# XiandaGuo/OpenStereo

Measured on AMD Instinct MI355X. Metric: stereo-pairs/s at 540x960 D=192 (GwcNet fwd), higher is better.
Workload: dtype f32 via f16x3 split-MFMA (hi/lo fp16 operands, f32 accumulate; HBM tensors f32); 1 GPU; GwcNet-gc inference, SceneFlow-shaped 540x960 padded to 544x960, D=192, G=40 + 12ch concat (BASELINE configs[1]); weights=deterministic synthetic (sharpened), random-init architecture, sub_batch_streams=3, parallelism=independent pairs x1, precision=f16x3, launch=hipGraph replay

## Files before the change

### include/openstereo_amd.h

```cpp
#ifndef OPENSTEREO_AMD_H
#define OPENSTEREO_AMD_H

#include <stddef.h>

#ifdef __cplusplus
extern "C" {
#endif

#define OSA_ABI_VERSION 17
#define OSA_META_FLOATS 128

enum { OSA_NCDHW = 0, OSA_NDHWC = 1 };
enum { OSA_ACT_NONE = 0, OSA_ACT_RELU = 1, OSA_ACT_LEAKY = 2, OSA_ACT_RELU6 = 3, OSA_ACT_SIGMOID = 4, OSA_ACT_TANH = 5 };
enum { OSA_GATE_RAW = 16 };
#define OSA_GATE_CHANNELS(n) ((int)((unsigned)(n) << 16))
enum { OSA_IN_SPLIT = 32, OSA_OUT_SPLIT = 64, OSA_RES_SPLIT = 128, OSA_REDIR_SPLIT = 256 };
enum { OSA_RES_AFTER_ACT = 512 };

int         osa_abi_version(void);
const char* osa_last_error(void);
const char* osa_target_arch(void);

int osa_build_volume_f32(const float* left_gwc, const float* right_gwc, int C, int num_groups,
                         const float* left_cat, const float* right_cat, int Cc,
                         float* vol, int layout, int vol_channels, int c_off,
                         int B, int H, int W, int maxdisp, int mask_left_concat,
                         float* vol_meta, void* stream);

int osa_build_volume_nhwc_f32(const float* left_gwc, const float* right_gwc, int C, int num_groups, int gwc_stride,
                              const float* left_cat, const float* right_cat, int Cc, int cat_stride,
                              float* vol, int vol_channels, int c_off,
                              int B, int H, int W, int maxdisp, int mask_left_concat, float* vol_meta, void* stream);
int osa_cat_fms_f32(const float* reference_fm, const float* target_fm, float* out, const int* disp_index,
                    int B, int C, int H, int W, int n_samples, void* stream);
int osa_pair_volume_f32(const float* left, const float* right, float* out,
                        int B, int C, int groups, int H, int W, int planes, int mode, void* stream);

int osa_corr_volume_f32(const float* left, const float* right, float* vol,
                        int B, int C, int H, int W, int maxdisp, void* stream);

int osa_ncdhw_to_ndhwc_f32(const float* x, float* y, int B, int C, long long S,
                           int yCs, int c_off, void* stream);
int osa_ndhwc_to_ncdhw_f32(const float* x, float* y, int B, int C, long long S,
                           int xCs, int c_off, void* stream);

size_t osa_conv3d_packed_floats(int Ci, int Co, int kd, int kh, int kw);
int    osa_conv3d_pack_f32(const float* w_ref, float* w_packed,
                           int Ci, int Co, int kd, int kh, int kw, void* stream);
size_t osa_deconv3d_packed_floats(int Ci, int Co, int k);
int    osa_deconv3d_pack_f32(const float* w_ref, float* w_packed,
                             int Ci, int Co, int k, int pad, void* stream);

int osa_conv3d_ndhwc_f32(const float* x, const float* w_packed,
                         const float* scale, const float* shift, const float* residual,
                         float* y,
                         int B, int Di, int Hi, int Wi, int Ci, int xCs,
                         int Co, int yCs, int rCs,
                         int kd, int kh, int kw, int stride,
                         int pad_d, int pad_h, int pad_w,
                         int dil_d, int dil_h, int dil_w,
                         const float* gate_logits, int gCs,
                         int act, float slope, void* stream);

int osa_conv3d_supported(int B, int Di, int Hi, int Wi, int Ci, int Co, int kd, int kh, int kw, int stride,
                         int pad_d, int pad_h, int pad_w, int dil_d, int dil_h, int dil_w, int precision);

int osa_deconv3d_ndhwc_f32(const float* x, const float* w_packed,
                           const float* scale, const float* shift, const float* residual,
                           float* y,
                           int B, int Di, int Hi, int Wi, int Ci, int xCs,
                           int Co, int yCs, int rCs,
                           int k, int pad, int opad,
                           const float* gate_logits, int gCs,
                           int act, float slope, void* stream);

typedef struct osa_f16x3_ranges {
    const float* x_meta;
    const float* residual_meta;
    const float* redir_meta;
    float*       y_meta;
    const float* bound_coef;
    const float* redir_bound_coef;
    const float* weight_scale;
} osa_f16x3_ranges;

int osa_conv3d_pack_ex_auto(const float* w_ref, float* w_packed, int Ci, int Co, int kd, int kh, int kw,
                            int src_transposed, int flip, const float* w_amax, float* scale_out, void* stream);
int osa_deconv3d_pack_f16x3_auto(const float* w_ref, float* w_packed, int Ci, int Co, int k, int pad,
                                 const float* w_amax, float* scale_out, void* stream);
int osa_deconv2d_pack_f16x3_auto(const float* w_ref, float* w_packed, int Ci, int Co, int k, int pad,
                                 const float* w_amax, float* scale_out, void* stream);

int osa_conv3d_pack_f16x3(const float* w_ref, float* w_packed,
                          int Ci, int Co, int kd, int kh, int kw, float wscale, void* stream);
int osa_deconv3d_pack_f16x3(const float* w_ref, float* w_packed,
                            int Ci, int Co, int k, int pad, float wscale, void* stream);
int osa_conv3d_ndhwc_f16x3(const float* x, const float* w_packed,
                           const float* scale, const float* shift, const float* residual,
                           float* y,
                           int B, int Di, int Hi, int Wi, int Ci, int xCs,
                           int Co, int yCs, int rCs,
                           int kd, int kh, int kw, int stride,
                           int pad_d, int pad_h, int pad_w,
                           int dil_d, int dil_h, int dil_w,
                           const float* gate_logits, int gCs,
                           int act, float slope, float out_scale, const osa_f16x3_ranges* ranges, void* stream);
int osa_deconv3d_ndhwc_f16x3(const float* x, const float* w_packed,
                             const float* scale, const float* shift, const float* residual,
                             float* y,
                             int B, int Di, int Hi, int Wi, int Ci, int xCs,
                             int Co, int yCs, int rCs,
                             int k, int pad, int opad,
                             const float* gate_logits, int gCs,
                             int act, float slope, float out_scale, const osa_f16x3_ranges* ranges, void* stream);

int osa_deconv3d_redir_ndhwc_f32(const float* x, const float* w_packed, const float* scale, const float* shift, float* y,
                                 int B, int Di, int Hi, int Wi, int Ci, int xCs, int Co, int yCs,
                                 int k, int pad, int opad,
                                 const float* rx, int rxCs, int rCi, const float* rw_packed,
                                 const float* rscale, const float* rshift,
                                 int act, float slope, void* stream);
int osa_deconv3d_redir_ndhwc_f16x3(const float* x, const float* w_packed, const float* scale, const float* shift, float* y,
                                   int B, int Di, int Hi, int Wi, int Ci, int xCs, int Co, int yCs,
                                   int k, int pad, int opad,
                                   const float* rx, int rxCs, int rCi, const float* rw_packed,
                                   const float* rscale, const float* rshift, float r_out_scale,
                                   int act, float slope, float out_scale, const osa_f16x3_ranges* ranges, void* stream);

size_t osa_deconv2d_packed_floats(int Ci, int Co, int k);
int    osa_deconv2d_pack_f32(const float* w_ref, float* w_packed, int Ci, int Co, int k, int pad, void* stream);
int    osa_deconv2d_pack_f16x3(const float* w_ref, float* w_packed, int Ci, int Co, int k, int pad,
                               float wscale, void* stream);
int osa_deconv2d_nhwc_f32(const float* x, const float* w_packed,
                          const float* scale, const float* shift, const float* residual,
                          float* y,
                          int B, int Hi, int Wi, int Ci, int xCs,
                          int Co, int yCs, int rCs,
                          int k, int pad, int opad,
                          const float* gate_logits, int gCs,
                          int act, float slope, void* stream);
int osa_deconv2d_nhwc_f16x3(const float* x, const float* w_packed,
                            const float* scale, const float* shift, const float* residual,
                            float* y,
                            int B, int Hi, int Wi, int Ci, int xCs,
                            int Co, int yCs, int rCs,
                            int k, int pad, int opad,
                            const float* gate_logits, int gCs,
                            int act, float slope, float out_scale, const osa_f16x3_ranges* ranges, void* stream);

int osa_dwconv2d_pack_f32(const float* w_ref, float* w_packed, int C, int kh, int kw, void* stream);
int osa_dwconv2d_nhwc_f32(const float* x, const float* w_packed,
                          const float* scale, const float* shift, const float* add, float* y,
                          int B, int Hi, int Wi, int C, int xCs, int yCs, int aCs,
                          int kh, int kw, int stride, int pad_h, int pad_w, int dil_h, int dil_w,
                          int act, float* y_meta, void* stream);
int osa_dwconv2d_nhwc_f16io(const void* x, int x_f16, const float* w_packed,
                            const float* scale, const float* shift, void* y, int y_f16,
                            int B, int Hi, int Wi, int C, int xCs, int yCs,
                            int kh, int kw, int stride, int pad_h, int pad_w,
                            int act, float* y_meta, void* stream);

int osa_gru_combine_f32(const float* z, const float* q, const float* h, float* out,
                        long long npix, int C, int zCs, int qCs, int hCs, int oCs, float* out_meta, void* stream);

typedef struct osa_nhwc_ref { void* ptr; int cs; int f16; } osa_nhwc_ref;
int osa_gru_gates_rz_fwd(const osa_nhwc_ref* pre, const float* bias_z, const float* bias_r, const osa_nhwc_ref* cz, const osa_nhwc_ref* cr,
                         const osa_nhwc_ref* h, const osa_nhwc_ref* z_out, const osa_nhwc_ref* rh_out, long long npix, int C, void* stream);
int osa_gru_gates_rz_bwd(const osa_nhwc_ref* pre, const float* bias_z, const float* bias_r, const osa_nhwc_ref* cz, const osa_nhwc_ref* cr,
                         const osa_nhwc_ref* h, const osa_nhwc_ref* dz, const osa_nhwc_ref* drh, const osa_nhwc_ref* dpre_out,
                         const osa_nhwc_ref* dh_out, long long npix, int C, void* stream);
int osa_gru_gates_q_fwd(const osa_nhwc_ref* z, const osa_nhwc_ref* qpre, const float* bias_q, const osa_nhwc_ref* cq, const osa_nhwc_ref* h,
                        const osa_nhwc_ref* out, long long npix, int C, void* stream);
int osa_gru_gates_q_bwd(const osa_nhwc_ref* z, const osa_nhwc_ref* qpre, const float* bias_q, const osa_nhwc_ref* cq, const osa_nhwc_ref* h,
                        const osa_nhwc_ref* dout, const osa_nhwc_ref* dz_out, const osa_nhwc_ref* dqpre_out, const osa_nhwc_ref* dh_out,
                        long long npix, int C, void* stream);

int osa_disp_update_f32(float* disp, const float* delta, int delta_cs, float* disp_nhwc4, float* slot, int slot_cs,
                        long long npix, float* disp4_meta, float* slot_meta, void* stream);

int osa_pool2x_nhwc_f32(const float* x, float* y, int B, int H, int W, int C, int xCs, int yCs,
                        const float* x_meta, float* y_meta, void* stream);
int osa_resize_bilinear_nhwc_f32(const float* x, float* y, int B, int Hi, int Wi, int Ho, int Wo, int C, int xCs, int yCs,
                                 const float* x_meta, float* y_meta, void* stream);

int osa_conv3d_pack_ex(const float* w_ref, float* w_packed, int Ci, int Co,
                       int kd, int kh, int kw, int src_transposed, int flip,
                       int f16x3, float wscale, void* stream);
int osa_conv3d_wgrad_f32(const float* x, const float* dy, float* dw,
                         int B, int Di, int Hi, int Wi, int Ci, int xCs,
                         int Do, int Ho, int Wo, int Co, int dyCs,
                         int kd, int kh, int kw, int stride,
                         int pad_d, int pad_h, int pad_w, int dil_d, int dil_h, int dil_w,
                         int transposed, void* stream);
size_t osa_conv3d_wgrad_workspace_bytes(int B, int Di, int Hi, int Wi, int Ci, int Do, int Ho, int Wo, int Co,
                                        int kd, int kh, int kw, int stride, int pad_d, int pad_h, int pad_w,
                                        int dil_d, int dil_h, int dil_w, int transposed);
int osa_conv3d_wgrad_ws_f32(const float* x, const float* dy, float* dw,
                            int B, int Di, int Hi, int Wi, int Ci, int xCs,
                            int Do, int Ho, int Wo, int Co, int dyCs,
                            int kd, int kh, int kw, int stride,
                            int pad_d, int pad_h, int pad_w, int dil_d, int dil_h, int dil_w,
                            int transposed, float* workspace, size_t workspace_bytes, void* stream);
size_t osa_conv3d_wgrad_f16x3_workspace_bytes(int B, int Di, int Hi, int Wi, int Ci, int Do, int Ho, int Wo, int Co,
                                              int kd, int kh, int kw, int stride, int pad_d, int pad_h, int pad_w,
                                              int dil_d, int dil_h, int dil_w, int transposed);
int osa_conv3d_wgrad_ws_f16x3(const float* x, const float* dy, float* dw,
                              int B, int Di, int Hi, int Wi, int Ci, int xCs,
                              int Do, int Ho, int Wo, int Co, int dyCs,
                              int kd, int kh, int kw, int stride,
                              int pad_d, int pad_h, int pad_w, int dil_d, int dil_h, int dil_w,
                              int transposed, const float* x_meta, const float* dy_meta,
                              float* workspace, size_t workspace_bytes, void* stream);
int osa_conv3d_wgrad_ws_f16(const void* x, const void* dy, float* dw,
                            int B, int Di, int Hi, int Wi, int Ci, int xCs,
                            int Do, int Ho, int Wo, int Co, int dyCs,
                            int kd, int kh, int kw, int stride,
                            int pad_d, int pad_h, int pad_w, int dil_d, int dil_h, int dil_w,
                            int transposed, const float* x_meta, const float* dy_meta, int x_f16, int dy_f16,
                            float* workspace, size_t workspace_bytes, void* stream);

int osa_conv3d_wgrad_ws_multi(int form, const void* const* xs, const void* const* dys, int n_items, float* dw,
                              int B, int Di, int Hi, int Wi, int Ci, int xCs,
                              int Do, int Ho, int Wo, int Co, int dyCs,
                              int kd, int kh, int kw, int stride,
                              int pad_d, int pad_h, int pad_w, int dil_d, int dil_h, int dil_w,
                              int transposed, const float* x_meta, const float* dy_meta, int x_f16, int dy_f16,
                              float* workspace, size_t workspace_bytes, void* stream);


int osa_conv3d_small_co_ndhwc_f32(const float* x, const float* w_ref, const float* bias,
                                  const float* residual, float* y,
                                  int B, int D, int H, int W, int Ci, int xCs, int Co, int yCs,
                                  int kd, int kh, int kw, int pad_d, int pad_h, int pad_w,
                                  void* stream);

size_t osa_conv3d_small_co_packed_floats(int Ci, int Co, int kd, int kh, int kw);
int    osa_conv3d_small_co_pack_f32(const float* w_ref, float* w_packed, int Ci, int Co,
                                    int kd, int kh, int kw, void* stream);
int    osa_conv3d_small_co_packed_ndhwc_f32(const float* x, const float* w_packed, const float* bias,
                                            const float* residual, float* y,
                                            int B, int D, int H, int W, int Ci, int xCs, int Co, int yCs,
                                            int kd, int kh, int kw, int pad_d, int pad_h, int pad_w,
                                            void* stream);

int osa_softargmin_f32(const float* prob, float* out, int B, int D, int H, int W, void* stream);
int osa_softmax_softargmin_f32(const float* cost, float* prob, float* out,
                               int B, int D, int H, int W, void* stream);
int osa_upsample_softargmin_f32(const float* cost_lowres, float* out,
                                int B, int Dl, int Hl, int Wl, int D, int H, int W,
                                int align_corners, void* stream);

int osa_softargmin_var_f32(const float* prob, const float* disparity, float* out, float* var,
                           int B, int D, int H, int W, void* stream);
int osa_softmax_softargmin_var_f32(const float* cost, float* out, float* var,
                                   int B, int D, int H, int W, void* stream);
int osa_upsample_softargmin_var_f32(const float* cost_lowres, float* out, float* var,
                                    int B, int Dl, int Hl, int Wl, int D, int H, int W,
                                    int align_corners, void* stream);

int osa_build_volume_bwd_f32(const float* dvol, const float* left, const float* right,
                             float* dleft, float* dright,
                             int B, int C, int H, int W, int maxdisp, int num_groups,
                             int concat, int mask_left_concat, int vol_channels, int c_off,
                             void* stream);
int osa_mr_volume_f32(const float* left, const float* right, const float* patch0, const float* patch1,
                      float* v0, float* v1, float* v2, int layout,
                      int B, int C, int H, int W, int num_groups, int out_channels, int maxdisp, int s_range, int m_range, int k0, int k1,
                      void* stream);
size_t osa_mr_volume_bwd_workspace_bytes(int B, int H, int W, int maxdisp);
int osa_mr_volume_bwd_ws_f32(const float* dv0, const float* dv1, const float* dv2, int layout,
                             const float* left, const float* right, const float* patch0, const float* patch1,
                             float* dleft, float* dright, float* dpatch0, float* dpatch1,
                             int B, int C, int H, int W, int num_groups, int out_channels, int maxdisp, int s_range, int m_range, int k0, int k1,
                             void* workspace, size_t workspace_bytes, void* stream);
int osa_softargmin_bwd_f32(const float* dout, float* dprob, int B, int D, int H, int W, void* stream);
int osa_softmax_softargmin_bwd_f32(const float* cost, const float* dout, float* dcost,
                                   int B, int D, int H, int W, void* stream);
int osa_upsample_softargmin_bwd_f32(const float* cost_lowres, const float* dout, float* dcost_lowres,
                                    int B, int Dl, int Hl, int Wl, int D, int H, int W,
                                    int align_corners, void* stream);
size_t osa_upsample_softargmin_bwd_workspace_bytes(int B, int Dl, int H, int W);
int osa_upsample_softargmin_bwd_ws_f32(const float* cost_lowres, const float* dout, float* dcost_lowres,
                                       int B, int Dl, int Hl, int Wl, int D, int H, int W,
                                       int align_corners, void* workspace, size_t workspace_bytes, void* stream);
int osa_softargmin_var_bwd_f32(const float* prob, const float* disparity, const float* dout, const float* dvar,
                               float* dprob, float* ddisparity, int B, int D, int H, int W, void* stream);
int osa_softmax_softargmin_var_bwd_f32(const float* cost, const float* dout, const float* dvar, float* dcost,
                                       int B, int D, int H, int W, void* stream);
int osa_upsample_softargmin_var_bwd_ws_f32(const float* cost_lowres, const float* dout, const float* dvar, float* dcost_lowres,
                                           int B, int Dl, int Hl, int Wl, int D, int H, int W,
                                           int align_corners, void* workspace, size_t workspace_bytes, void* stream);

int osa_amax_f32(const float* x, long long n, float* meta, void* stream);

int osa_context_upsample_f32(const float* disp_low, const float* weights, float* out,
                             int B, int h, int w, int scale, int softmax_weights, float gain,
                             void* stream);
int osa_context_upsample_logits_f32(const float* disp_low, const void* logits, int logits_f16, const long long* logits_strides,
                                    float* out, int B, int h, int w, int scale, float gain, void* stream);
int osa_context_upsample_logits_bwd_f32(const float* disp_low, const void* logits, int logits_f16, const long long* logits_strides,
                                        const float* dout, float* ddisp_low, void* dlogits, const long long* dlogits_strides, float* scratch,
                                        int B, int h, int w, int scale, float gain, void* stream);

int osa_allpairs_corr_f32(const float* fmap1, const float* fmap2, float* corr,
                          int B, int C, int H, int W1, int W2, void* stream);
int osa_geo_rows_f32(const float* vol_ndhwc, float* rows, int B, int D, int H, int W, int C, int Cs, void* stream);
int osa_avgpool_rows_f32(const float* x, float* y, long long rows, int n, void* stream);
int osa_geo_lookup_f32(const float* const* geo_levels, const float* const* corr_levels,
                       const int* geo_len, const int* corr_len, int levels,
                       const float* disp, const float* coords_x, float* out,
                       int B, int H, int W, int C, int radius, void* stream);
int osa_geo_lookup_nhwc_f32(const float* const* geo_levels, const float* const* corr_levels,
                            const int* geo_len, const int* corr_len, int levels,
                            const float* disp, const float* coords_x, float* out, int out_cs,
                            int B, int H, int W, int C, int radius, void* stream);
int osa_geo_lookup_bwd_f32(float* const* dgeo_levels, float* const* dcorr_levels,
                           const int* geo_len, const int* corr_len, int levels,
                           const float* disp, const float* coords_x, const float* dout,
                           int B, int H, int W, int C, int radius, void* stream);
int osa_geo_lookup_bwd_acc_f32(float* const* dgeo_levels, float* const* dcorr_levels,
                               const int* geo_len, const int* corr_len, int levels,
                               const float* disp, const float* coords_x, const float* dout,
                               int B, int H, int W, int C, int radius, void* stream);

int osa_geo_lookup_mr_f32(const float* const* geo0_levels, const float* const* corr_levels,
                          const int* geo0_len, const int* corr_len, int levels,
                          const float* geo1, int geo1_len, const float* geo2, int geo2_len,
                          const float* disp, const float* coords_x,
                          float* geo_feat0, float* geo_feat1, float* geo_feat2, float* init_corr,
                          int B, int H, int W, int C, int radius, void* stream);
int osa_geo_lookup_mr_nhwc_f32(const float* const* geo0_levels, const float* const* corr_levels,
                               const int* geo0_len, const int* corr_len, int levels,
                               const float* geo1, int geo1_len, const float* geo2, int geo2_len,
                               const float* disp, const float* coords_x,
                               float* geo_feat0, float* geo_feat1, float* geo_feat2, float* init_corr,
                               int cs0, int cs1, int cs2, int cs_corr,
                               int B, int H, int W, int C, int radius, void* stream);
int osa_geo_lookup_mr_bwd_acc_f32(float* const* dgeo0_levels, float* const* dcorr_levels,
                                  const int* geo0_len, const int* corr_len, int levels,
                                  float* dgeo1, int geo1_len, float* dgeo2, int geo2_len,
                                  const float* disp, const float* coords_x,
                                  const float* dfeat0, const float* dfeat1, const float* dfeat2, const float* dcorr_out,
                                  int B, int H, int W, int C, int radius, void* stream);

size_t osa_mv2_block3d_packed_floats(int Ci, int Ch, int Co);
int osa_mv2_block3d_pack_f32(const float* w_expand, const float* w_dw, const float* w_project, const float* scale1, const float* shift1,
                             const float* scale2, const float* shift2, const float* scale3, const float* shift3, float* packed,
                             int Ci, int Ch, int Co, void* stream);
int osa_mv2_block3d_f32(const float* x, const float* packed, float* y, int B, int D, int H, int W, int Ci, int Ch, int Co, int stride, int residual,
                        void* stream);

size_t osa_mv2_block2d_packed_floats(int Ci, int Ch, int Co);
int osa_mv2_block2d_pack_f32(const float* w_expand, const float* w_dw, const float* w_project, const float* scale1, const float* shift1,
                             const float* scale2, const float* shift2, const float* scale3, const float* shift3, float* packed,
                             int Ci, int Ch, int Co, void* stream);
int osa_mv2_block2d_f32(const float* x, const float* packed, const float* addend, float* y, int B, int H, int W, int Ci, int Ch, int Co, int stride,
                        int residual, int relu, void* stream);

size_t osa_interlaced_volume_packed_floats(int C, int k2, int k3, int F);
int osa_interlaced_volume_pack_f32(const float* w1, const float* w2, const float* w3, const float* w4, const float* scale1, const float* shift1,
                                   const float* scale2, const float* shift2, const float* scale3, const float* shift3, const float* scale4,
                                   const float* shift4, float* packed, int C, int k2, int k3, int F, void* stream);
int osa_interlaced_volume_f32(const float* featL, const float* featR, const float* packed, float* out, int B, int C, int H, int W, int D, int k2, int k3,
                              int F, void* stream);

size_t osa_disparity_attention_packed_floats(int C, int nhead, int ff, int layers);
int osa_disparity_attention_pack_f32(const float* w_attn, const float* b_attn, const float* w1, const float* b1, const float* w2, const float* b2,
                                     const float* ln, float* packed, int C, int nhead, int ff, int layers, void* stream);
int osa_disparity_attention_f32(const float* cv, const float* pe, const float* packed, float* out, int layout, int B, int C, int L, int H, int W,
                                int nhead, int ff, int layers, void* stream);

int osa_preprocess_pair_f32(const void* left_hwc, const void* right_hwc, int is_u8,
                            int H, int W, int Hp, int Wp,
                            const float* mean3, const float* std3,
                            float* out, int layout, void* stream);

enum { OSA_IN_F16 = 32, OSA_OUT_F16 = 64, OSA_RES_F16 = 128 };
int osa_conv3d_pack_f16(const float* w_ref, float* w_packed, int Ci, int Co, int kd, int kh, int kw, void* stream);
int osa_deconv3d_pack_f16(const float* w_ref, float* w_packed, int Ci, int Co, int k, int pad, void* stream);
int osa_deconv2d_pack_f16(const float* w_ref, float* w_packed, int Ci, int Co, int k, int pad, void* stream);
int osa_conv3d_ndhwc_f16(const void* x, const float* w_packed, const float* scale, const float* shift, const void* residual, void* y,
                         int B, int Di, int Hi, int Wi, int Ci, int xCs, int Co, int yCs, int rCs, int kd, int kh, int kw, int stride,
                         int pad_d, int pad_h, int pad_w, int dil_d, int dil_h, int dil_w, const float* gate_logits, int gCs,
                         int act, float slope, void* stream);
int osa_deconv3d_ndhwc_f16(const void* x, const float* w_packed, const float* scale, const float* shift, const void* residual, void* y,
                           int B, int Di, int Hi, int Wi, int Ci, int xCs, int Co, int yCs, int rCs, int k, int pad, int opad,
                           const float* gate_logits, int gCs, int act, float slope, void* stream);
int osa_deconv2d_nhwc_f16(const void* x, const float* w_packed, const float* scale, const float* shift, const void* residual, void* y,
                          int B, int Hi, int Wi, int Ci, int xCs, int Co, int yCs, int rCs, int k, int pad, int opad,
                          const float* gate_logits, int gCs, int act, float slope, void* stream);

size_t osa_channel_sums_workspace_bytes(long long P, int C);
int osa_channel_sums(const void* dy, int dy_f16, int dy_cs, const void* x, int x_f16, int x_cs, const float* x_shift,
                     const float* dx_scale, void* dx, int dx_cs, long long P, int C,
                     float* out, float* workspace, size_t workspace_bytes, void* stream);
int osa_channel_sums_multi(const void* const* dys, int n_items, int dy_f16, int dy_cs, long long P, int C,
// ... 37 lines not shown
```

### openstereo_amd/_lib.py

```python
from __future__ import annotations

import ctypes as C
import os
import threading

_HERE = os.path.dirname(os.path.abspath(__file__))
LIB_PATH = os.environ.get("OSA_LIB_PATH") or os.path.join(_HERE, "lib", "libopenstereo_amd.so")

_lock = threading.Lock()
_lib = None

c_fp = C.c_void_p
c_i = C.c_int
c_f = C.c_float
c_st = C.c_void_p
c_ll = C.c_longlong


class F16x3Ranges(C.Structure):
    _fields_ = [("x_meta", C.c_void_p), ("residual_meta", C.c_void_p), ("redir_meta", C.c_void_p),
                ("y_meta", C.c_void_p), ("bound_coef", C.c_void_p), ("redir_bound_coef", C.c_void_p), ("weight_scale", C.c_void_p)]


c_rng = C.POINTER(F16x3Ranges)


class NhwcRef(C.Structure):
    _fields_ = [("ptr", C.c_void_p), ("cs", C.c_int), ("f16", C.c_int)]


c_ref = C.POINTER(NhwcRef)

_LEVELS = [C.POINTER(C.c_void_p), C.POINTER(C.c_void_p), C.POINTER(c_i), C.POINTER(c_i), c_i]
SIGNATURES = {
    "osa_abi_version": (c_i, []),
    **dict.fromkeys(("osa_last_error", "osa_target_arch"), (C.c_char_p, [])),
    "osa_build_volume_f32": (c_i, [c_fp, c_fp, c_i, c_i, c_fp, c_fp, c_i, c_fp] + [c_i] * 8 + [c_fp, c_st]),
    "osa_build_volume_nhwc_f32": (c_i, [c_fp, c_fp, c_i, c_i, c_i, c_fp, c_fp, c_i, c_i, c_fp] + [c_i] * 7 + [c_fp, c_st]),
    **dict.fromkeys(("osa_corr_volume_f32", "osa_allpairs_corr_f32"), (c_i, [c_fp, c_fp, c_fp, c_i, c_i, c_i, c_i, c_i, c_st])),
    **dict.fromkeys(("osa_ncdhw_to_ndhwc_f32", "osa_ndhwc_to_ncdhw_f32"), (c_i, [c_fp, c_fp, c_i, c_i, c_ll, c_i, c_i, c_st])),
    **dict.fromkeys(("osa_conv3d_packed_floats", "osa_conv3d_small_co_packed_floats"), (C.c_size_t, [c_i, c_i, c_i, c_i, c_i])),
    **dict.fromkeys(("osa_conv3d_pack_f32", "osa_conv3d_small_co_pack_f32", "osa_conv3d_pack_f16"), (c_i, [c_fp, c_fp, c_i, c_i, c_i, c_i, c_i, c_st])),
    **dict.fromkeys(("osa_deconv3d_packed_floats", "osa_deconv2d_packed_floats"), (C.c_size_t, [c_i, c_i, c_i])),
    **dict.fromkeys(("osa_deconv3d_pack_f32", "osa_softargmin_bwd_f32", "osa_deconv2d_pack_f32", "osa_deconv3d_pack_f16", "osa_deconv2d_pack_f16", "osa_softargmin_f32"), (c_i, [c_fp, c_fp, c_i, c_i, c_i, c_i, c_st])),
    **dict.fromkeys(("osa_conv3d_ndhwc_f32", "osa_conv3d_ndhwc_f16"), (c_i, [c_fp] * 6 + [c_i] * 19 + [c_fp, c_i, c_i, c_f, c_st])),
    **dict.fromkeys(("osa_deconv3d_ndhwc_f32", "osa_deconv3d_ndhwc_f16"), (c_i, [c_fp] * 6 + [c_i] * 12 + [c_fp, c_i, c_i, c_f, c_st])),
    "osa_conv3d_supported": (c_i, [c_i] * 17),
    "osa_conv3d_pack_f16x3": (c_i, [c_fp, c_fp, c_i, c_i, c_i, c_i, c_i, c_f, c_st]),
    **dict.fromkeys(("osa_deconv3d_pack_f16x3", "osa_deconv2d_pack_f16x3"), (c_i, [c_fp, c_fp, c_i, c_i, c_i, c_i, c_f, c_st])),
    "osa_conv3d_ndhwc_f16x3": (c_i, [c_fp] * 6 + [c_i] * 19 + [c_fp, c_i, c_i, c_f, c_f, c_rng, c_st]),
    "osa_deconv3d_ndhwc_f16x3": (c_i, [c_fp] * 6 + [c_i] * 12 + [c_fp, c_i, c_i, c_f, c_f, c_rng, c_st]),
    "osa_conv3d_pack_ex": (c_i, [c_fp, c_fp, c_i, c_i, c_i, c_i, c_i, c_i, c_i, c_i, c_f, c_st]),
    "osa_pair_volume_f32": (c_i, [c_fp, c_fp, c_fp, c_i, c_i, c_i, c_i, c_i, c_i, c_i, c_st]),
    "osa_conv3d_wgrad_f32": (c_i, [c_fp, c_fp, c_fp] + [c_i] * 22 + [c_st]),
    **dict.fromkeys(("osa_conv3d_wgrad_workspace_bytes", "osa_conv3d_wgrad_f16x3_workspace_bytes"), (C.c_size_t, [c_i] * 20)),
    "osa_conv3d_wgrad_ws_f32": (c_i, [c_fp, c_fp, c_fp] + [c_i] * 22 + [c_fp, C.c_size_t, c_st]),
    "osa_conv3d_wgrad_ws_f16x3": (c_i, [c_fp, c_fp, c_fp] + [c_i] * 22 + [c_fp, c_fp, c_fp, C.c_size_t, c_st]),
    "osa_conv3d_wgrad_ws_f16": (c_i, [c_fp, c_fp, c_fp] + [c_i] * 22 + [c_fp, c_fp, c_i, c_i, c_fp, C.c_size_t, c_st]),
    **dict.fromkeys(("osa_conv3d_small_co_ndhwc_f32", "osa_conv3d_small_co_packed_ndhwc_f32"), (c_i, [c_fp] * 5 + [c_i] * 14 + [c_st])),
    "osa_build_volume_bwd_f32": (c_i, [c_fp, c_fp, c_fp, c_fp, c_fp, c_i, c_i, c_i, c_i, c_i, c_i, c_i, c_i, c_i, c_i, c_st]),
    **dict.fromkeys(("osa_softmax_softargmin_bwd_f32", "osa_softmax_softargmin_f32", "osa_softmax_softargmin_var_f32"), (c_i, [c_fp, c_fp, c_fp, c_i, c_i, c_i, c_i, c_st])),
    **dict.fromkeys(("osa_upsample_softargmin_bwd_f32", "osa_upsample_softargmin_var_f32"), (c_i, [c_fp, c_fp, c_fp, c_i, c_i, c_i, c_i, c_i, c_i, c_i, c_i, c_st])),
    "osa_amax_f32": (c_i, [c_fp, C.c_longlong, c_fp, c_st]),
    **dict.fromkeys(("osa_upsample_softargmin_bwd_workspace_bytes", "osa_mr_volume_bwd_workspace_bytes", "osa_interlaced_volume_packed_floats", "osa_disparity_attention_packed_floats"), (C.c_size_t, [c_i] * 4)),
    "osa_upsample_softargmin_bwd_ws_f32": (c_i, [c_fp, c_fp, c_fp, c_i, c_i, c_i, c_i, c_i, c_i, c_i, c_i, c_fp, C.c_size_t, c_st]),
    "osa_deconv3d_redir_ndhwc_f32": (c_i, [c_fp] * 5 + [c_i] * 11 + [c_fp, c_i, c_i, c_fp, c_fp, c_fp, c_i, c_f, c_st]),
    "osa_deconv3d_redir_ndhwc_f16x3": (c_i, [c_fp] * 5 + [c_i] * 11 + [c_fp, c_i, c_i, c_fp, c_fp, c_fp, c_f, c_i, c_f, c_f, c_rng, c_st]),
    **dict.fromkeys(("osa_deconv2d_nhwc_f32", "osa_deconv2d_nhwc_f16"), (c_i, [c_fp] * 6 + [c_i] * 11 + [c_fp, c_i, c_i, c_f, c_st])),
    "osa_deconv2d_nhwc_f16x3": (c_i, [c_fp] * 6 + [c_i] * 11 + [c_fp, c_i, c_i, c_f, c_f, c_rng, c_st]),
    "osa_dwconv2d_pack_f32": (c_i, [c_fp, c_fp, c_i, c_i, c_i, c_st]),
    "osa_dwconv2d_nhwc_f32": (c_i, [c_fp] * 6 + [c_i] * 15 + [c_fp, c_st]),
    "osa_dwconv2d_nhwc_f16io": (c_i, [c_fp, c_i, c_fp, c_fp, c_fp, c_fp, c_i] + [c_i] * 11 + [c_i, c_fp, c_st]),
    "osa_gru_combine_f32": (c_i, [c_fp, c_fp, c_fp, c_fp, c_ll, c_i, c_i, c_i, c_i, c_i, c_fp, c_st]),
    "osa_gru_gates_rz_fwd": (c_i, [c_ref, c_fp, c_fp, c_ref, c_ref, c_ref, c_ref, c_ref, c_ll, c_i, c_st]),
    "osa_gru_gates_rz_bwd": (c_i, [c_ref, c_fp, c_fp, c_ref, c_ref, c_ref, c_ref, c_ref, c_ref, c_ref, c_ll, c_i, c_st]),
    "osa_gru_gates_q_fwd": (c_i, [c_ref, c_ref, c_fp, c_ref, c_ref, c_ref, c_ll, c_i, c_st]),
    "osa_gru_gates_q_bwd": (c_i, [c_ref, c_ref, c_fp, c_ref, c_ref, c_ref, c_ref, c_ref, c_ref, c_ll, c_i, c_st]),
    "osa_disp_update_f32": (c_i, [c_fp, c_fp, c_i, c_fp, c_fp, c_i, c_ll, c_fp, c_fp, c_st]),
    "osa_conv3d_pack_ex_auto": (c_i, [c_fp, c_fp, c_i, c_i, c_i, c_i, c_i, c_i, c_i, c_fp, c_fp, c_st]),
    **dict.fromkeys(("osa_deconv3d_pack_f16x3_auto", "osa_deconv2d_pack_f16x3_auto"), (c_i, [c_fp, c_fp, c_i, c_i, c_i, c_i, c_fp, c_fp, c_st])),
    "osa_cat_fms_f32": (c_i, [c_fp, c_fp, c_fp, c_fp, c_i, c_i, c_i, c_i, c_i, c_st]),
    "osa_pool2x_nhwc_f32": (c_i, [c_fp, c_fp, c_i, c_i, c_i, c_i, c_i, c_i, c_fp, c_fp, c_st]),
    "osa_resize_bilinear_nhwc_f32": (c_i, [c_fp, c_fp, c_i, c_i, c_i, c_i, c_i, c_i, c_i, c_i, c_fp, c_fp, c_st]),
    "osa_context_upsample_logits_f32": (c_i, [c_fp, c_fp, c_i, C.POINTER(c_ll), c_fp, c_i, c_i, c_i, c_i, c_f, c_st]),
    "osa_context_upsample_logits_bwd_f32": (c_i, [c_fp, c_fp, c_i, C.POINTER(c_ll), c_fp, c_fp, c_fp, C.POINTER(c_ll), c_fp, c_i, c_i, c_i, c_i, c_f, c_st]),
    "osa_context_upsample_f32": (c_i, [c_fp, c_fp, c_fp, c_i, c_i, c_i, c_i, c_i, c_f, c_st]),
    "osa_geo_rows_f32": (c_i, [c_fp, c_fp, c_i, c_i, c_i, c_i, c_i, c_i, c_st]),
    "osa_avgpool_rows_f32": (c_i, [c_fp, c_fp, c_ll, c_i, c_st]),
    **dict.fromkeys(("osa_geo_lookup_f32", "osa_geo_lookup_bwd_acc_f32", "osa_geo_lookup_bwd_f32"), (c_i, _LEVELS + [c_fp, c_fp, c_fp, c_i, c_i, c_i, c_i, c_i, c_st])),
    "osa_geo_lookup_nhwc_f32": (c_i, _LEVELS + [c_fp, c_fp, c_fp, c_i, c_i, c_i, c_i, c_i, c_i, c_st]),
    **dict.fromkeys(("osa_geo_lookup_mr_f32", "osa_geo_lookup_mr_bwd_acc_f32"), (c_i, _LEVELS + [c_fp, c_i, c_fp, c_i, c_fp, c_fp, c_fp, c_fp, c_fp, c_fp, c_i, c_i, c_i, c_i, c_i, c_st])),
    "osa_geo_lookup_mr_nhwc_f32": (c_i, _LEVELS + [c_fp, c_i, c_fp, c_i, c_fp, c_fp, c_fp, c_fp, c_fp, c_fp, c_i, c_i, c_i, c_i, c_i, c_i, c_i, c_i, c_i, c_st]),
    "osa_preprocess_pair_f32": (c_i, [c_fp, c_fp, c_i, c_i, c_i, c_i, c_i, C.POINTER(c_f), C.POINTER(c_f), c_fp, c_i, c_st]),
    "osa_instnorm_workspace_floats": (C.c_size_t, [c_i, c_ll, c_i]),
    "osa_instnorm_nhwc_f32": (c_i, [c_fp, c_fp, c_i, c_ll, c_i, c_i, c_i, c_f, c_i, c_f, c_fp, c_fp, c_st]),
    "osa_conv3d_wgrad_ws_multi": (c_i, [c_i, c_fp, c_fp, c_i, c_fp] + [c_i] * 22 + [c_fp, c_fp, c_i, c_i, c_fp, C.c_size_t, c_st]),
    "osa_channel_sums_workspace_bytes": (C.c_size_t, [c_ll, c_i]),
    "osa_channel_affine": (c_i, [c_fp, c_i, c_i, c_fp, c_i, c_i, c_fp, c_fp, c_fp, c_fp, c_i, c_ll, c_i, c_i, c_st]),
    "osa_channel_sums_multi": (c_i, [c_fp, c_i, c_i, c_i, c_ll, c_i, c_fp, c_fp, C.c_size_t, c_st]),
    "osa_channel_sums": (c_i, [c_fp, c_i, c_i, c_fp, c_i, c_i, c_fp, c_fp, c_fp, c_i, c_ll, c_i, c_fp, c_fp, C.c_size_t, c_st]),
    **dict.fromkeys(("osa_conv3d_march_launches", "osa_conv3d_march_s2_launches", "osa_deconv3d_walk_launches", "osa_conv_b_ring_launches", "osa_volume_walk_launches"), (c_ll, [])),
    **dict.fromkeys(("osa_deconv_walk", "osa_deconv_walk_segment_planes", "osa_conv_march_s2_segment_planes", "osa_conv_b_ring_mask", "osa_volume_walk_step"), (c_i, [c_i])),
    "osa_build_volume_nhwc_split_eligible": (c_i, [c_fp, c_fp, c_fp, c_i, c_i, c_i, c_i, c_i, c_i, c_i, c_i, c_i]),
    "osa_build_volume_nhwc_split_f16x3": (c_i, [c_fp, c_fp, c_i, c_i, c_i, c_fp, c_fp, c_i, c_i, c_fp] + [c_i] * 7 + [c_fp, c_fp, c_fp, c_st]),
    "osa_upsample_softargmin_f32": (c_i, [c_fp, c_fp, c_i, c_i, c_i, c_i, c_i, c_i, c_i, c_i, c_st]),
    **dict.fromkeys(("osa_softargmin_var_f32", "osa_softmax_softargmin_var_bwd_f32"), (c_i, [c_fp, c_fp, c_fp, c_fp, c_i, c_i, c_i, c_i, c_st])),
    "osa_softargmin_var_bwd_f32": (c_i, [c_fp, c_fp, c_fp, c_fp, c_fp, c_fp, c_i, c_i, c_i, c_i, c_st]),
    "osa_upsample_softargmin_var_bwd_ws_f32": (c_i, [c_fp, c_fp, c_fp, c_fp, c_i, c_i, c_i, c_i, c_i, c_i, c_i, c_i, c_fp, C.c_size_t, c_st]),
    "osa_mr_volume_f32": (c_i, [c_fp] * 7 + [c_i] * 12 + [c_st]),
    "osa_mr_volume_bwd_ws_f32": (c_i, [c_fp] * 3 + [c_i] + [c_fp] * 8 + [c_i] * 11 + [c_fp, C.c_size_t, c_st]),
    **dict.fromkeys(("osa_mv2_block3d_packed_floats", "osa_mv2_block2d_packed_floats"), (C.c_size_t, [c_i] * 3)),
    **dict.fromkeys(("osa_mv2_block3d_pack_f32", "osa_mv2_block2d_pack_f32"), (c_i, [c_fp] * 10 + [c_i] * 3 + [c_st])),
    "osa_mv2_block3d_f32": (c_i, [c_fp] * 3 + [c_i] * 9 + [c_st]),
    **dict.fromkeys(("osa_mv2_block2d_f32", "osa_disparity_attention_f32"), (c_i, [c_fp] * 4 + [c_i] * 9 + [c_st])),
    "osa_disparity_attention_pack_f32": (c_i, [c_fp] * 8 + [c_i] * 4 + [c_st]),
    "osa_interlaced_volume_pack_f32": (c_i, [c_fp] * 13 + [c_i] * 4 + [c_st]),
    "osa_interlaced_volume_f32": (c_i, [c_fp] * 4 + [c_i] * 8 + [c_st]),
}


class EngineError(RuntimeError):
    pass


def load():
    global _lib
    if _lib is not None:
        return _lib
    with _lock:
        if _lib is not None:
            return _lib
        if not os.path.exists(LIB_PATH):
            raise EngineError(f"{LIB_PATH} is missing: build it with `python -m openstereo_amd.build` (hipcc, gfx950). There is no CPU fallback.")
        lib = C.CDLL(LIB_PATH)
        for name, (res, args) in SIGNATURES.items():
            fn = getattr(lib, name)
            fn.restype = res
            fn.argtypes = args
        if lib.osa_abi_version() != abi_version(lib):
            raise EngineError(f"ABI version mismatch: library reports {lib.osa_abi_version()}, include/openstereo_amd.h declares {abi_version(lib)}")
        if os.environ.get("OSA_B_RING_MASK"):
            lib.osa_conv_b_ring_mask(int(os.environ["OSA_B_RING_MASK"], 0))
        if os.environ.get("OSA_DECONV_WALK"):
            lib.osa_deconv_walk(int(os.environ["OSA_DECONV_WALK"], 0))
        if os.environ.get("OSA_VOL_WALK"):
            lib.osa_volume_walk_step(int(os.environ["OSA_VOL_WALK"]))
        _lib = lib
    return _lib


_abi = None


def abi_version(lib=None) -> int:
    global _abi
    if _abi is None:
        import re
        hdr = os.path.join(os.path.dirname(os.path.abspath(__file__)), "..", "include", "openstereo_amd.h")
        try:
            with open(hdr) as f:
                _abi = int(re.search(r"#define\s+OSA_ABI_VERSION\s+(\d+)", f.read()).group(1))
        except (OSError, AttributeError):
            h = lib if lib is not None else _lib
            if h is None:
                return -1
            _abi = int(h.osa_abi_version())
    return _abi


CALLS = {}


def call(name: str, *args):
    lib = load()
    CALLS[name] = CALLS.get(name, 0) + 1
    rc = getattr(lib, name)(*args)
    if rc != 0:
        msg = lib.osa_last_error()
        raise EngineError(f"{name} failed ({rc}): {msg.decode() if msg else '?'}")
    return rc
```

### openstereo_amd/csrc/conv3d.hip

```cpp
#include "conv_kernel.h"
#include "conv_inst.h"

namespace osa {

struct KernelCfg {
    const char* name;
    int M, N;
    int TD, TH, TW, threads;
    int ks;
    int table, idx;
};

static const KernelCfg g_cfgs[] = {
#define OSA_CFG_X(RING, MT, NT, WM, WN, TH, TW)                                                                  \
    { #MT "x" #NT "_" #WM "x" #WN "_" #TH "x" #TW, WM * MT * 32, WN * NT * 32, WM * MT * 32 / (TH * TW), TH, TW, WM * WN * 64, 0, 0, -1 },
#define OSA_KS_X(MT, NT, WM, WN, TH, TW, KS)
#include "conv_cfgs.def"
#undef OSA_CFG_X
#undef OSA_KS_X
};
constexpr int N_CFGS = sizeof(g_cfgs) / sizeof(g_cfgs[0]);

static const KernelCfg g_ks_cfgs[] = {
#define OSA_CFG_X(RING, MT, NT, WM, WN, TH, TW)
#define OSA_KS_X(MT, NT, WM, WN, TH, TW, KS)                                                                     \
    { #MT "x" #NT "_" #WM "x" #WN "_" #TH "x" #TW "_ks" #KS, WM * MT * 32, WN * NT * 32, WM * MT * 32 / (TH * TW), TH, TW, WM * WN * KS * 64, KS, 1, -1 },
#include "conv_cfgs.def"
#undef OSA_CFG_X
#undef OSA_KS_X
};

static const KernelCfg g_deconv_redir_cfg = { "deconv8_redir_1x1_4x1_4x8", 128, 32, 4, 4, 8, 256, 0, 2, 0 };
static const KernelCfg g_deconv_redir64_cfg = { "deconv8_redir64_1x1_4x1_4x8", 128, 32, 4, 4, 8, 256, 0, 2, 1 };
static const KernelCfg g_deconv_cfg = { "deconv8_1x1_4x1_4x8", 128, 32, 4, 4, 8, 256, 0, 2, 2 };
static const KernelCfg g_deconv_flat_cfg = { "deconv4_1x1_4x1_8x16", 128, 32, 1, 8, 16, 256, 0, 2, 3 };

static const KernelFns& fns_of(const KernelCfg& k, int prec) {
    const ConvFnTables& t = (prec == PREC_F32) ? conv_tables_f32() : ((prec == PREC_F16X3) ? conv_tables_f16x3() : conv_tables_f16());
    if (k.table == 0) return t.cfgs[&k - g_cfgs];
    if (k.table == 1) return t.ks[&k - g_ks_cfgs];
    return t.deconv[k.idx];
}

static int g_b_ring_mask_value();
static int pick_cfg(const ConvArgs& a, int stride, int prec = PREC_F32) {
    {
        const int v = exp_int("OSA_CONV_CFG", -1);
        if (v >= 0 && v < N_CFGS && a.CoP % g_cfgs[v].N == 0) return v;
    }
    const bool flat = (a.Ad == 1);
    const long long vox = (long long)a.B * a.Ad * a.Ah * a.Aw;
    if (flat) {
        if (stride == 2) return (a.CoP % 64 == 0) ? 14 : 12;
        const long long tiles128 = (vox + 127) / 128;
        if (a.CoP % 128 == 0) return (tiles128 * (a.CoP / 128) < 768) ? 11 : 9;
        if (a.CoP % 64 == 0) return (tiles128 * (a.CoP / 64) < 128) ? 14 : 13;
        return 12;
    }
    if (stride == 2) return (a.CoP % 128 == 0) ? 6 : ((a.CoP % 64 == 0) ? 5 : 15);
    if (a.T <= 8) return (a.CoP % 64 == 0) ? 4 : 3;
    if (prec != PREC_F32 && a.CoP % 64 == 0 && ((g_b_ring_mask_value() >> 4) & 1)) return 4;
    if (a.CoP % 128 == 0) return 2;
    if (vox < (1ll << 20)) return (a.CoP % 64 == 0) ? 4 : 3;
    return (a.CoP % 64 == 0) ? 1 : 0;
}

static void finish_geometry(ConvArgs& a, int TW, bool compact) {
    if (exp_set("OSA_NOCOMPACT")) compact = false;
    int rowq;
    if (compact) {
        a.VQ = 4;
        rowq = a.LW * 4 + 1;
    } else {
        a.VQ = 5;
        const int want = (TW == 8) ? 8 : 0;
        rowq = a.LW * 5;
        while ((rowq & 15) != want) ++rowq;
        if (exp_set("OSA_NOPAD")) rowq = a.LW * 5;
    }
    a.RowQ = rowq; a.PlaneQ = a.LH * a.RowQ;
    for (int t = 0; t < a.T; ++t)
        a.toff[t] = (a.td[t] - a.dmin) * a.PlaneQ + (a.th[t] - a.hmin) * a.RowQ + (a.tw[t] - a.wmin) * a.VQ;
    a.magicW = (unsigned)((0x100000000ull + a.LW - 1) / a.LW);
    a.magicH = (unsigned)((0x100000000ull + a.LH - 1) / a.LH);
    a.magicHW = (unsigned)((0x100000000ull + (unsigned long long)a.LH * a.LW - 1) / ((unsigned long long)a.LH * a.LW));
    a.dbg = exp_int("OSA_DBG", 0);
}

static size_t brick_bytes(ConvArgs& a, const KernelCfg& k) {
    int dmax = -128, hmax = -128, wmax = -128;
    a.dmin = a.hmin = a.wmin = 127;
    for (int t = 0; t < a.T; ++t) {
        a.dmin = a.td[t] < a.dmin ? a.td[t] : a.dmin; dmax = a.td[t] > dmax ? a.td[t] : dmax;
        a.hmin = a.th[t] < a.hmin ? a.th[t] : a.hmin; hmax = a.th[t] > hmax ? a.th[t] : hmax;
        a.wmin = a.tw[t] < a.wmin ? a.tw[t] : a.wmin; wmax = a.tw[t] > wmax ? a.tw[t] : wmax;
    }
    a.LD = (k.TD - 1) * a.isd + (dmax - a.dmin) + 1;
    a.LH = (k.TH - 1) * a.ish + (hmax - a.hmin) + 1;
    a.LW = (k.TW - 1) * a.isw + (wmax - a.wmin) + 1;
    return (size_t)a.LD * a.LH * (a.LW * VS + 64) * sizeof(float);
}

int launch_conv_march(ConvArgs& a, hipStream_t st, const char* what);
int launch_conv_march_s2(ConvArgs& a, hipStream_t st, const char* what);
int launch_conv_deconv_walk(ConvArgs& a, hipStream_t st, const char* what);
void wgrad_set_multi_tile(int on);

static int g_b_ring_mask = (1 << 1) | (1 << 2) | (1 << 3) | (1 << 4) | (1 << 13) | (1 << 29) | (1 << 27);
static long long g_b_ring_launches = 0;
static int g_b_ring_mask_value() { return g_b_ring_mask; }

static int plan_conv(ConvArgs& a, int stride, int prec, const char* what, const KernelCfg* forced, const KernelCfg*& kp) {
    int ci = forced ? 0 : pick_cfg(a, stride, prec);
    if (!forced && brick_bytes(a, g_cfgs[ci]) > 160 * 1024) {
        static const int fallback[] = {5, 15, 3, 11};
        for (int f : fallback)
            if (a.CoP % g_cfgs[f].N == 0 && brick_bytes(a, g_cfgs[f]) <= 160 * 1024) { ci = f; break; }
    }
    kp = forced ? forced : &g_cfgs[ci];
    if (!forced && (ci == 11 || ci == 14) && a.Ad == 1 && !(a.act & OSA_OUT_SPLIT)) {
        const int want = exp_int("OSA_KS", -1);
        const long long items = (prec == PREC_F32) ? 1 : a.B;
        const long long nwg = ((items * a.Ad * a.Ah * a.Aw + g_cfgs[ci].M - 1) / g_cfgs[ci].M) * (a.CoP / g_cfgs[ci].N);
        int ks = (a.nchunks % 4 == 0 && a.nchunks >= 16) ? 4 : ((a.nchunks % 2 == 0 && a.nchunks >= 8) ? 2 : 1);
        if (nwg >= 192) ks = 1;
        else if (nwg >= 96 && ks == 4) ks = 2;
        if (want >= 0) ks = (want > 1 && a.nchunks % want == 0) ? want : 1;
        const KernelCfg* split = (ks == 4) ? &g_ks_cfgs[ci == 11 ? 0 : 1] : ((ks == 2) ? &g_ks_cfgs[ci == 11 ? 2 : 3] : nullptr);
        if (split && brick_bytes(a, *split) * ks <= 160 * 1024) kp = split;
    }
    const KernelCfg& k = *kp;
    a.tilesD = cdiv(a.Ad, k.TD); a.tilesH = cdiv(a.Ah, k.TH); a.tilesW = cdiv(a.Aw, k.TW);
    (void)brick_bytes(a, k);
    OSA_REQUIRE((long long)a.LD * a.LH * a.LW < 65536, "%s: LDS brick too large", what);
    finish_geometry(a, k.TW, k.TW == 8 && a.isw == 1);
    const size_t brick = (size_t)a.LD * a.PlaneQ * sizeof(float4);
    OSA_REQUIRE(brick <= 160 * 1024, "%s: LDS brick %dx%dx%d needs %zu B (> 160 KiB)", what, a.LD, a.LH, a.LW, brick);
    return 0;
}

static int launch_conv(ConvArgs& a, int stride, int prec, hipStream_t st, const char* what,
                       const KernelCfg* forced = nullptr) {
    const KernelCfg* kp = nullptr;
    if (plan_conv(a, stride, prec, what, forced, kp)) return -1;
    const KernelCfg& k = *kp;
    const size_t brick = (size_t)a.LD * a.PlaneQ * sizeof(float4);
    a.cps = 1;
    {
        const int want = exp_int("OSA_CPS", 4);
        const size_t cap = (size_t)exp_int("OSA_CPS_LDS", 40 * 1024);
        while (a.cps < want && a.cps < a.nchunks && (size_t)(a.cps + 1) * brick <= cap) ++a.cps;
    }
// ... 123 lines not shown
        v = p.transposed ? p.src[((size_t)ci * p.Co + co) * kvol + kidx] : p.src[((size_t)co * p.Ci + ci) * kvol + kidx];
    }
    reinterpret_cast<_Float16*>(p.dst)[i] = (_Float16)v;
}

__device__ __forceinline__ float auto_wscale(float amax) {
    const unsigned b = __builtin_bit_cast(unsigned, amax);
    const int eb = (int)((b >> 23) & 0xffu);
    if (eb == 0 || eb == 255) return 1.f;
    int k = 14 - (eb - 127) - ((b & 0x7fffffu) ? 1 : 0);
    k = k < -14 ? -14 : (k > 40 ? 40 : k);
    return __builtin_bit_cast(float, (unsigned)(127 + k) << 23);
}
__global__ __launch_bounds__(256) void pack_weights_f16x3_auto_kernel(const PackArgs p, const float* __restrict__ amax, float* __restrict__ scale_out) {
    const float wscale = auto_wscale(*amax);
    if (blockIdx.x == 0 && threadIdx.x == 0) { scale_out[0] = wscale; scale_out[1] = 1.0f / wscale; }
    const size_t total = (size_t)p.nchunks * p.T * 2 * 2 * p.CoP * 8;
    size_t i = (size_t)blockIdx.x * 256 + threadIdx.x;
    if (i >= total) return;
    const int e = i & 7; size_t r = i >> 3;
    const int co = r % p.CoP; r /= p.CoP;
    const int kg = r & 1; r >>= 1;
    const int hl = r & 1; r >>= 1;
    const int t = r % p.T; const int ch = r / p.T;
    const int ci = ch * CC + 8 * kg + e;
    float v = 0.f;
    if (ci < p.Ci && co < p.Co) {
        const size_t kvol = (size_t)p.kd * p.kh * p.kw;
        const size_t kidx = ((size_t)p.kz[t] * p.kh + p.ky[t]) * p.kw + p.kx[t];
        v = wscale * (p.transposed ? p.src[((size_t)ci * p.Co + co) * kvol + kidx]
                                   : p.src[((size_t)co * p.Ci + ci) * kvol + kidx]);
    }
    const _Float16 hi = (_Float16)v;
    reinterpret_cast<_Float16*>(p.dst)[i] = hl ? (_Float16)(v - (float)hi) : hi;
}

static inline int pad32(int c) { return (c + 31) / 32 * 32; }
static inline int nchunks_of(int ci) { return (ci + CC - 1) / CC; }
static inline size_t packed_floats(int Ci, int Co, int T) {
    return (size_t)nchunks_of(Ci) * T * JO * 2 * pad32(Co) * 4;
}
static inline size_t slack_floats(int Co) { return (size_t)4 * JO * 2 * pad32(Co) * 4; }

static int deconv_dim_taps(int k, int pad, int par, int* delta, int* kk) {
    int n = 0;
    for (int t = 0; t < k; ++t) {
        const int num = par + pad - t;
        if (((num % 2) + 2) % 2 != 0) continue;
        delta[n] = (num >= 0) ? num / 2 : -((-num) / 2);
        kk[n] = t;
        ++n;
    }
    return n;
}

template <int CO, bool WG>
__global__ __launch_bounds__(256) void conv_small_co_tiled_kernel(const ConvArgs p, const float* __restrict__ wref,
                                                                  const float* __restrict__ bias) {
    constexpr int TD = 4, TH = 8, TW = 8;
    extern __shared__ __attribute__((aligned(16))) float4 smem[];
    const int tid = threadIdx.x;
    float4* wl4 = smem + (size_t)p.LD * p.PlaneQ;
    float* wl = reinterpret_cast<float*>(wl4);

    unsigned bid = xcd_remap(blockIdx.x, gridDim.x);
    const int twi = bid % p.tilesW; bid /= p.tilesW;
    const int thi = bid % p.tilesH; bid /= p.tilesH;
    const int tdi = bid % p.tilesD;
    const int b = bid / p.tilesD;
    const int a0d = tdi * TD, a0h = thi * TH, a0w = twi * TW;
    const int g0d = a0d + p.dmin, g0h = a0h + p.hmin, g0w = a0w + p.wmin;

    const int nw = WG ? 0 : p.nchunks * p.T * CO * 16;
    for (int i = tid; i < nw; i += 256) {
        const int e = i & 15; int r = i >> 4;
        const int co = r % CO; r /= CO;
        const int t = r % p.T; const int ch = r / p.T;
        const int ci = ch * CC + e;
        wl[i] = (ci < p.Ci) ? wref[((size_t)co * p.Ci + ci) * p.T + t] : 0.f;
    }
    const int tw_ = tid % TW, th_ = (tid / TW) % TH, td_ = tid / (TW * TH);
    const int abase = td_ * p.PlaneQ + th_ * p.RowQ + tw_ * p.VQ;
    float acc[CO];
#pragma unroll
    for (int o = 0; o < CO; ++o) acc[o] = bias ? bias[o] : 0.f;

    for (int ch = 0; ch < p.nchunks; ++ch) {
        if (ch) __syncthreads();
        stage_brick<256, PREC_F32, 1>(p, smem, 0, b, ch * CC, g0d, g0h, g0w, tid);
        __syncthreads();
        for (int t = 0; t < p.T; ++t) {
            const float4* xp = smem + abase + p.toff[t];
            const float4* wq = WG ? reinterpret_cast<const float4*>(wref) + (size_t)(ch * p.T + t) * CO * 4
                                  : wl4 + (size_t)(ch * p.T + t) * CO * 4;
#pragma unroll
            for (int q = 0; q < 4; ++q) {
                const float4 xv = xp[q];
#pragma unroll
                for (int o = 0; o < CO; ++o) {
                    const float4 wv = wq[o * 4 + q];
                    acc[o] = fmaf(xv.x, wv.x, acc[o]); acc[o] = fmaf(xv.y, wv.y, acc[o]);
                    acc[o] = fmaf(xv.z, wv.z, acc[o]); acc[o] = fmaf(xv.w, wv.w, acc[o]);
                }
            }
        }
    }
    const int ad = a0d + td_, ah = a0h + th_, aw = a0w + tw_;
    if (ad < p.Ad && ah < p.Ah && aw < p.Aw) {
        const size_t vox = (((size_t)b * p.Do + ad) * p.Ho + ah) * p.Wo + aw;
#pragma unroll
        for (int o = 0; o < CO; ++o)
            p.y[vox * p.yCs + o] = acc[o] + (p.res ? p.res[vox * p.yCs + o] : 0.f);
    }
}


constexpr int CM_TH = 16, CM_TW = 16, CM_LH = 18, CM_LW = 18, CM_PXQ = 9, CM_ROWQ = 176, CM_ITEMS = CM_LH * CM_LW * 8, CM_PER = (CM_ITEMS + 255) / 256;
__global__ __launch_bounds__(256) void classifier_march_kernel(const ConvArgs p, const float* __restrict__ wpk, const float* __restrict__ bias,
                                                               int dseg, int nseg) {
    extern __shared__ __attribute__((aligned(16))) float4 smem[];
    const int tid = threadIdx.x;
    unsigned bid = xcd_remap(blockIdx.x, gridDim.x);
    const int twi = bid % p.tilesW; bid /= p.tilesW;
    const int thi = bid % p.tilesH; bid /= p.tilesH;
    const int seg = bid % nseg;
    const int b = bid / nseg;
    const int d0 = seg * dseg, d1 = (d0 + dseg < p.Di) ? d0 + dseg : p.Di;
    const int h0 = thi * CM_TH, w0 = twi * CM_TW;
    const size_t plane = (size_t)p.Hi * p.Wi * p.xCs;
    const float* xb = p.x + (size_t)b * p.Di * plane;

    int goff[CM_PER], loff[CM_PER];
#pragma unroll
    for (int j = 0; j < CM_PER; ++j) {
        const int i = tid + 256 * j;
        const int px = i >> 3, q = i & 7;
        const int lh = px / CM_LW, lw = px - lh * CM_LW;
        const int gh = h0 - 1 + lh, gw = w0 - 1 + lw;
        const bool in = i < CM_ITEMS && gh >= 0 && gh < p.Hi && gw >= 0 && gw < p.Wi;
        goff[j] = in ? (gh * p.Wi + gw) * p.xCs + q * 4 : -1;
        loff[j] = (i < CM_ITEMS) ? lh * CM_ROWQ + lw * CM_PXQ + q : -1;
    }
    float4 pre[CM_PER];
    auto issue = [&](int pd) {
        const float* xp = xb + (size_t)pd * plane;
#pragma unroll
        for (int j = 0; j < CM_PER; ++j)
            pre[j] = (goff[j] >= 0) ? *reinterpret_cast<const float4*>(xp + goff[j]) : make_float4(0.f, 0.f, 0.f, 0.f);
    };
    const int tw_ = tid % CM_TW, th_ = tid / CM_TW;
    const float4* xt = smem + th_ * CM_ROWQ + tw_ * CM_PXQ;
    const float4* w4 = reinterpret_cast<const float4*>(wpk);
    float a0 = 0.f, a1 = 0.f, a2 = 0.f;
    issue(d0 > 0 ? d0 - 1 : 0);
    for (int pd = d0 - 1; pd <= d1; ++pd) {
        if (pd >= 0 && pd < p.Di) {
            __syncthreads();
#pragma unroll
            for (int j = 0; j < CM_PER; ++j)
                if (loff[j] >= 0) smem[loff[j]] = pre[j];
            __syncthreads();
            if (pd + 1 <= d1 && pd + 1 < p.Di) issue(pd + 1);
#pragma unroll
            for (int kh = 0; kh < 3; ++kh)
#pragma unroll
                for (int kw = 0; kw < 3; ++kw)
#pragma unroll
                    for (int q = 0; q < 8; ++q) {
                        const float4 xv = xt[kh * CM_ROWQ + kw * CM_PXQ + q];
                        const int wi = ((q >> 2) * 27 + kh * 3 + kw) * 4 + (q & 3);
                        const float4 wk0 = w4[wi], wk1 = w4[wi + 9 * 4], wk2 = w4[wi + 18 * 4];
                        a0 = fmaf(xv.x, wk2.x, a0); a0 = fmaf(xv.y, wk2.y, a0); a0 = fmaf(xv.z, wk2.z, a0); a0 = fmaf(xv.w, wk2.w, a0);
                        a1 = fmaf(xv.x, wk1.x, a1); a1 = fmaf(xv.y, wk1.y, a1); a1 = fmaf(xv.z, wk1.z, a1); a1 = fmaf(xv.w, wk1.w, a1);
                        a2 = fmaf(xv.x, wk0.x, a2); a2 = fmaf(xv.y, wk0.y, a2); a2 = fmaf(xv.z, wk0.z, a2); a2 = fmaf(xv.w, wk0.w, a2);
                    }
        }
        const int od = pd - 1, oh = h0 + th_, ow = w0 + tw_;
        if (od >= d0 && od < d1 && oh < p.Hi && ow < p.Wi) {
            const size_t vox = (((size_t)b * p.Do + od) * p.Ho + oh) * p.Wo + ow;
            p.y[vox * p.yCs] = a0 + (bias ? bias[0] : 0.f) + (p.res ? p.res[vox * p.yCs] : 0.f);
        }
        a0 = a1; a1 = a2; a2 = 0.f;
    }
}

}

using namespace osa;

extern "C" size_t osa_conv3d_packed_floats(int Ci, int Co, int kd, int kh, int kw) {
    return packed_floats(Ci, Co, kd * kh * kw) + slack_floats(Co);
}

static void launch_pack(const PackArgs& p, int prec, float wscale, hipStream_t st, const float* amax_dev = nullptr, float* scale_out = nullptr) {
    if (amax_dev) {
        const size_t total = (size_t)p.nchunks * p.T * 2 * 2 * p.CoP * 8;
        hipLaunchKernelGGL(pack_weights_f16x3_auto_kernel, dim3(total ? cdiv((long long)total, 256) : 1), dim3(256), 0, st, p, amax_dev, scale_out);
        return;
    }
    if (prec == PREC_F32) {
        const size_t total = (size_t)p.nchunks * p.T * JO * 2 * p.CoP * 4;
        if (total) hipLaunchKernelGGL(pack_weights_kernel, dim3(cdiv((long long)total, 256)), dim3(256), 0, st, p);
    } else if (prec == PREC_F16) {
        const size_t total = (size_t)p.nchunks * p.T * 2 * 2 * p.CoP * 8;
        if (total) hipLaunchKernelGGL(pack_weights_f16_kernel, dim3(cdiv((long long)total, 256)), dim3(256), 0, st, p);
    } else {
        const size_t total = (size_t)p.nchunks * p.T * 2 * 2 * p.CoP * 8;
        if (total) hipLaunchKernelGGL(pack_weights_f16x3_kernel, dim3(cdiv((long long)total, 256)), dim3(256), 0, st, p, wscale);
    }
}

static int conv3d_pack_impl(const float* w_ref, float* w_packed, int Ci, int Co,
                            int kd, int kh, int kw, int prec, float wscale, void* stream,
                            int src_transposed = 0, int flip = 0, const float* amax_dev = nullptr, float* scale_out = nullptr) {
    OSA_REQUIRE(w_ref && w_packed, "conv3d_pack: NULL pointer");
    const int T = kd * kh * kw;
    OSA_REQUIRE(T >= 1 && T <= MAX_TAPS, "conv3d_pack: %dx%dx%d kernel has %d taps (max %d)", kd, kh, kw, T, MAX_TAPS);
    OSA_REQUIRE(Ci > 0 && Co > 0, "conv3d_pack: bad channels %d->%d", Ci, Co);
    PackArgs p;
    p.src = w_ref; p.dst = w_packed; p.Ci = Ci; p.Co = Co; p.CoP = pad32(Co);
    p.kd = kd; p.kh = kh; p.kw = kw; p.T = T; p.nchunks = (prec == PREC_F16) ? cdiv(Ci, 32) : nchunks_of(Ci); p.transposed = src_transposed ? 1 : 0;
    int t = 0;
    for (int z = 0; z < kd; ++z) for (int y = 0; y < kh; ++y) for (int x = 0; x < kw; ++x, ++t) {
        p.kz[t] = (signed char)(flip ? kd - 1 - z : z); p.ky[t] = (signed char)(flip ? kh - 1 - y : y);
        p.kx[t] = (signed char)(flip ? kw - 1 - x : x);
    }
    launch_pack(p, prec, wscale, (hipStream_t)stream, amax_dev, scale_out);
    OSA_LAUNCH_CHECK("conv3d_pack");
    return 0;
}

extern "C" int osa_conv3d_pack_ex_auto(const float* w_ref, float* w_packed, int Ci, int Co, int kd, int kh, int kw,
                                       int src_transposed, int flip, const float* w_amax, float* scale_out, void* stream) {
    OSA_REQUIRE(w_amax && scale_out, "conv3d_pack_ex_auto: NULL scale pointers");
    return conv3d_pack_impl(w_ref, w_packed, Ci, Co, kd, kh, kw, PREC_F16X3, 1.f, stream, src_transposed, flip, w_amax, scale_out);
}

extern "C" int osa_conv3d_pack_f32(const float* w_ref, float* w_packed, int Ci, int Co,
                                   int kd, int kh, int kw, void* stream) {
    return conv3d_pack_impl(w_ref, w_packed, Ci, Co, kd, kh, kw, PREC_F32, 1.f, stream);
}

extern "C" int osa_conv3d_pack_ex(const float* w_ref, float* w_packed, int Ci, int Co,
                                  int kd, int kh, int kw, int src_transposed, int flip,
                                  int f16x3, float wscale, void* stream) {
    OSA_REQUIRE(wscale > 0.f, "conv3d_pack_ex: wscale must be a positive power of two");
    return conv3d_pack_impl(w_ref, w_packed, Ci, Co, kd, kh, kw, (f16x3 == 2) ? PREC_F16 : (f16x3 ? PREC_F16X3 : PREC_F32), wscale, stream,
                            src_transposed, flip);
}

extern "C" int osa_conv3d_pack_f16x3(const float* w_ref, float* w_packed, int Ci, int Co,
                                     int kd, int kh, int kw, float wscale, void* stream) {
    OSA_REQUIRE(wscale > 0.f, "conv3d_pack_f16x3: wscale must be a positive power of two");
    return conv3d_pack_impl(w_ref, w_packed, Ci, Co, kd, kh, kw, PREC_F16X3, wscale, stream);
}

extern "C" int osa_conv3d_pack_f16(const float* w_ref, float* w_packed, int Ci, int Co, int kd, int kh, int kw, void* stream) {
    return conv3d_pack_impl(w_ref, w_packed, Ci, Co, kd, kh, kw, PREC_F16, 1.f, stream);
}

extern "C" size_t osa_deconv3d_packed_floats(int Ci, int Co, int k) {
    return packed_floats(Ci, Co, k * k * k) + slack_floats(Co);
}

struct DeconvTaps {
    int T; int cls_end[8];
    signed char kz[MAX_TAPS], ky[MAX_TAPS], kx[MAX_TAPS], dz[MAX_TAPS], dy[MAX_TAPS], dx[MAX_TAPS];
};
static void deconv_taps(int k, int pad, DeconvTaps& d, bool flat = false) {
    int t = 0;
    for (int cls = 0; cls < 8; ++cls) {
        int dd[4], kd_[4], dh[4], kh_[4], dw[4], kw_[4];
        int nd = flat ? (((cls >> 2) & 1) ? 0 : 1) : deconv_dim_taps(k, pad, (cls >> 2) & 1, dd, kd_);
        if (flat) { dd[0] = 0; kd_[0] = 0; }
        const int nh = deconv_dim_taps(k, pad, (cls >> 1) & 1, dh, kh_);
        const int nw = deconv_dim_taps(k, pad, cls & 1, dw, kw_);
        for (int a = 0; a < nd; ++a) for (int b = 0; b < nh; ++b) for (int c = 0; c < nw; ++c, ++t) {
            d.kz[t] = (signed char)kd_[a]; d.ky[t] = (signed char)kh_[b]; d.kx[t] = (signed char)kw_[c];
            d.dz[t] = (signed char)dd[a]; d.dy[t] = (signed char)dh[b]; d.dx[t] = (signed char)dw[c];
        }
        d.cls_end[cls] = t;
    }
    d.T = t;
}

static int deconv3d_pack_impl(const float* w_ref, float* w_packed, int Ci, int Co,
                              int k, int pad, int prec, float wscale, void* stream, bool flat = false,
                              const float* amax_dev = nullptr, float* scale_out = nullptr) {
    OSA_REQUIRE(w_ref && w_packed, "deconv3d_pack: NULL pointer");
    OSA_REQUIRE(k == 3 || k == 4, "deconv3d_pack: kernel %d unsupported (3 or 4)", k);
    DeconvTaps d;
    deconv_taps(k, pad, d, flat);
    PackArgs p;
    p.src = w_ref; p.dst = w_packed; p.Ci = Ci; p.Co = Co; p.CoP = pad32(Co);
    p.kd = flat ? 1 : k; p.kh = k; p.kw = k; p.T = d.T; p.nchunks = (prec == PREC_F16) ? cdiv(Ci, 32) : nchunks_of(Ci); p.transposed = 1;
    for (int t = 0; t < d.T; ++t) { p.kz[t] = d.kz[t]; p.ky[t] = d.ky[t]; p.kx[t] = d.kx[t]; }
    launch_pack(p, prec, wscale, (hipStream_t)stream, amax_dev, scale_out);
    OSA_LAUNCH_CHECK("deconv3d_pack");
    return 0;
}

extern "C" int osa_deconv3d_pack_f16x3_auto(const float* w_ref, float* w_packed, int Ci, int Co, int k, int pad,
                                            const float* w_amax, float* scale_out, void* stream) {
    OSA_REQUIRE(w_amax && scale_out, "deconv3d_pack_f16x3_auto: NULL scale pointers");
    return deconv3d_pack_impl(w_ref, w_packed, Ci, Co, k, pad, PREC_F16X3, 1.f, stream, false, w_amax, scale_out);
}

extern "C" int osa_deconv2d_pack_f16x3_auto(const float* w_ref, float* w_packed, int Ci, int Co, int k, int pad,
                                            const float* w_amax, float* scale_out, void* stream) {
    OSA_REQUIRE(w_amax && scale_out, "deconv2d_pack_f16x3_auto: NULL scale pointers");
    return deconv3d_pack_impl(w_ref, w_packed, Ci, Co, k, pad, PREC_F16X3, 1.f, stream, true, w_amax, scale_out);
}

extern "C" int osa_deconv3d_pack_f32(const float* w_ref, float* w_packed, int Ci, int Co,
                                     int k, int pad, void* stream) {
    return deconv3d_pack_impl(w_ref, w_packed, Ci, Co, k, pad, PREC_F32, 1.f, stream);
}

extern "C" int osa_deconv3d_pack_f16x3(const float* w_ref, float* w_packed, int Ci, int Co,
                                       int k, int pad, float wscale, void* stream) {
    OSA_REQUIRE(wscale > 0.f, "deconv3d_pack_f16x3: wscale must be a positive power of two");
    return deconv3d_pack_impl(w_ref, w_packed, Ci, Co, k, pad, PREC_F16X3, wscale, stream);
}

extern "C" int osa_deconv3d_pack_f16(const float* w_ref, float* w_packed, int Ci, int Co, int k, int pad, void* stream) {
    return deconv3d_pack_impl(w_ref, w_packed, Ci, Co, k, pad, PREC_F16, 1.f, stream);
}
extern "C" int osa_deconv2d_pack_f16(const float* w_ref, float* w_packed, int Ci, int Co, int k, int pad, void* stream) {
// ... 163 lines not shown
                                    int pad_d, int pad_h, int pad_w, int dil_d, int dil_h, int dil_w, const float* gate_logits, int gCs,
                                    int act, float slope, void* stream) {
    const float* x = static_cast<const float*>(x_); const float* residual = static_cast<const float*>(residual_); float* y = static_cast<float*>(y_);
    return conv3d_impl(OSA_CONV_ARGS, PREC_F16, 1.f, stream);
}

static int deconv3d_impl(const float* x, const float* w_packed,
                         const float* scale, const float* shift, const float* residual,
                         float* y,
                         int B, int Di, int Hi, int Wi, int Ci, int xCs,
                         int Co, int yCs, int rCs,
                         int k, int pad, int opad,
                         const float* gate_logits, int gCs,
                         int act, float slope, int prec, float oscale, void* stream, bool flat = false,
                         const float* rx = nullptr, int rxCs = 0, int rCi = 0, const float* rw_packed = nullptr,
                         const float* rscale = nullptr, const float* rshift = nullptr, float roscale = 1.f,
                         const osa_f16x3_ranges* rng = nullptr) {
    if (gate_logits) OSA_REQUIRE(gCs >= Co, "deconv3d: gate stride %d < Co %d", gCs, Co);
    if (check_common("deconv3d", x, w_packed, y, B, Di, Hi, Wi, Ci, xCs, Co, yCs, rCs, residual)) return -1;
    if (flat) OSA_REQUIRE(Di == 1, "deconv2d: the tensor must have D == 1 (got %d)", Di);
    OSA_REQUIRE((k == 3 && pad == 1 && opad == 1) || (k == 4 && pad == 1 && opad == 0),
                "deconv3d: only (k=3,p=1,op=1) and (k=4,p=1,op=0) with stride 2 are supported (got k=%d p=%d op=%d)", k, pad, opad);
    DeconvTaps d;
    deconv_taps(k, pad, d, flat);
    ConvArgs a;
    memset(&a, 0, sizeof(a));
    a.x = x; a.w = reinterpret_cast<const float4*>(w_packed);
    a.scale = scale; a.shift = shift; a.res = residual; a.y = y;
    a.gate = gate_logits; a.gCs = gCs;
    a.B = B; a.Di = Di; a.Hi = Hi; a.Wi = Wi; a.Ci = Ci; a.xCs = xCs;
    a.Do = flat ? 1 : (Di - 1) * 2 - 2 * pad + k + opad; a.Ho = (Hi - 1) * 2 - 2 * pad + k + opad; a.Wo = (Wi - 1) * 2 - 2 * pad + k + opad;
    a.Co = Co; a.yCs = yCs; a.rCs = rCs;
    a.Ad = (a.Do + 1) / 2; a.Ah = (a.Ho + 1) / 2; a.Aw = (a.Wo + 1) / 2;
    a.isd = a.ish = a.isw = 1;
    a.os = 2;
    a.T = d.T;
    for (int t = 0; t < d.T; ++t) { a.td[t] = d.dz[t]; a.th[t] = d.dy[t]; a.tw[t] = d.dx[t]; }
    for (int c = 0; c < 8; ++c) a.cls_end[c] = d.cls_end[c];
    a.nchunks = nchunks_of(Ci); a.CoP = pad32(Co);
    a.act = act; a.slope = slope; a.oscale = oscale;
    if (prec == PREC_F16 && f16_units(a, flat ? "deconv2d" : "deconv3d")) return -1;
    if (rx) {
        OSA_REQUIRE(!flat && !residual && !gate_logits, "deconv3d_redir: residual / gate cannot be combined with the fused redir branch");
        OSA_REQUIRE(rw_packed && rCi > 0 && rCi <= 64 && rCi % 4 == 0 && rxCs >= rCi && rxCs % 4 == 0 && ((size_t)rx & 15) == 0,
                    "deconv3d_redir: redir input needs <= 64 channels (multiple of 4), stride >= channels, 16-byte alignment (Ci=%d stride=%d)", rCi, rxCs);
        OSA_REQUIRE((long long)a.Do * a.Ho * a.Wo * rxCs < (1ll << 31), "deconv3d_redir: redir input too large");
        a.rx = rx; a.rxCs = rxCs; a.rCi = rCi; a.rw = reinterpret_cast<const float4*>(rw_packed);
        a.rscale = rscale; a.rshift = rshift; a.roscale = roscale;
    }
    set_ranges(a, rng);
    if (check_split_ranges(a, prec, flat ? "deconv2d" : "deconv3d")) return -1;
    if (prec == PREC_F16X3 && !flat && k == 3 && rx) {
        const int r = launch_conv_deconv_walk(a, (hipStream_t)stream, "deconv3d (walk)");
        if (r != 0) return r < 0 ? r : 0;
    }
    return launch_conv(a, 1, prec, (hipStream_t)stream, flat ? "deconv2d" : "deconv3d",
                       flat ? &g_deconv_flat_cfg : (rx ? (rCi > 32 ? &g_deconv_redir64_cfg : &g_deconv_redir_cfg) : &g_deconv_cfg));
}

#define OSA_DECONV_PARAMS                                                                       \
    const float* x, const float* w_packed, const float* scale, const float* shift,             \
    const float* residual, float* y, int B, int Di, int Hi, int Wi, int Ci, int xCs,           \
    int Co, int yCs, int rCs, int k, int pad, int opad, const float* gate_logits, int gCs, int act, float slope
#define OSA_DECONV_ARGS                                                                         \
    x, w_packed, scale, shift, residual, y, B, Di, Hi, Wi, Ci, xCs, Co, yCs, rCs, k, pad, opad, \
    gate_logits, gCs, act, slope

extern "C" int osa_deconv3d_ndhwc_f32(OSA_DECONV_PARAMS, void* stream) {
    return deconv3d_impl(OSA_DECONV_ARGS, PREC_F32, 1.f, stream);
}

extern "C" int osa_deconv3d_ndhwc_f16x3(OSA_DECONV_PARAMS, float out_scale, const osa_f16x3_ranges* ranges, void* stream) {
    return deconv3d_impl(OSA_DECONV_ARGS, PREC_F16X3, out_scale, stream, false, nullptr, 0, 0, nullptr, nullptr, nullptr, 1.f, ranges);
}

extern "C" int osa_deconv3d_ndhwc_f16(const void* x_, const float* w_packed, const float* scale, const float* shift, const void* residual_, void* y_,
                                      int B, int Di, int Hi, int Wi, int Ci, int xCs, int Co, int yCs, int rCs, int k, int pad, int opad,
                                      const float* gate_logits, int gCs, int act, float slope, void* stream) {
    const float* x = static_cast<const float*>(x_); const float* residual = static_cast<const float*>(residual_); float* y = static_cast<float*>(y_);
    return deconv3d_impl(OSA_DECONV_ARGS, PREC_F16, 1.f, stream);
}

#define OSA_REDIR_PARAMS const float* rx, int rxCs, int rCi, const float* rw_packed, const float* rscale, const float* rshift
extern "C" int osa_deconv3d_redir_ndhwc_f32(const float* x, const float* w_packed, const float* scale, const float* shift, float* y,
                                            int B, int Di, int Hi, int Wi, int Ci, int xCs, int Co, int yCs,
                                            int k, int pad, int opad, OSA_REDIR_PARAMS, int act, float slope, void* stream) {
    return deconv3d_impl(x, w_packed, scale, shift, nullptr, y, B, Di, Hi, Wi, Ci, xCs, Co, yCs, 0, k, pad, opad, nullptr, 0,
                         act, slope, PREC_F32, 1.f, stream, false, rx, rxCs, rCi, rw_packed, rscale, rshift, 1.f);
}

extern "C" int osa_deconv3d_redir_ndhwc_f16x3(const float* x, const float* w_packed, const float* scale, const float* shift, float* y,
                                              int B, int Di, int Hi, int Wi, int Ci, int xCs, int Co, int yCs,
                                              int k, int pad, int opad, OSA_REDIR_PARAMS, float r_out_scale,
                                              int act, float slope, float out_scale, const osa_f16x3_ranges* ranges, void* stream) {
    return deconv3d_impl(x, w_packed, scale, shift, nullptr, y, B, Di, Hi, Wi, Ci, xCs, Co, yCs, 0, k, pad, opad, nullptr, 0,
                         act, slope, PREC_F16X3, out_scale, stream, false, rx, rxCs, rCi, rw_packed, rscale, rshift, r_out_scale, ranges);
}

#define OSA_DECONV2D_PARAMS                                                                     \
    const float* x, const float* w_packed, const float* scale, const float* shift,             \
    const float* residual, float* y, int B, int Hi, int Wi, int Ci, int xCs,                   \
    int Co, int yCs, int rCs, int k, int pad, int opad, const float* gate_logits, int gCs, int act, float slope
#define OSA_DECONV2D_ARGS                                                                       \
    x, w_packed, scale, shift, residual, y, B, 1, Hi, Wi, Ci, xCs, Co, yCs, rCs, k, pad, opad, \
    gate_logits, gCs, act, slope

extern "C" int osa_deconv2d_nhwc_f32(OSA_DECONV2D_PARAMS, void* stream) {
    return deconv3d_impl(OSA_DECONV2D_ARGS, PREC_F32, 1.f, stream, true);
}

extern "C" int osa_deconv2d_nhwc_f16x3(OSA_DECONV2D_PARAMS, float out_scale, const osa_f16x3_ranges* ranges, void* stream) {
    return deconv3d_impl(OSA_DECONV2D_ARGS, PREC_F16X3, out_scale, stream, true, nullptr, 0, 0, nullptr, nullptr, nullptr, 1.f, ranges);
}

extern "C" int osa_deconv2d_nhwc_f16(const void* x_, const float* w_packed, const float* scale, const float* shift, const void* residual_, void* y_,
                                     int B, int Hi, int Wi, int Ci, int xCs, int Co, int yCs, int rCs, int k, int pad, int opad,
                                     const float* gate_logits, int gCs, int act, float slope, void* stream) {
    const float* x = static_cast<const float*>(x_); const float* residual = static_cast<const float*>(residual_); float* y = static_cast<float*>(y_);
    return deconv3d_impl(OSA_DECONV2D_ARGS, PREC_F16, 1.f, stream, true);
}

__global__ __launch_bounds__(256) void small_co_pack_kernel(const float* __restrict__ src, float* __restrict__ dst,
                                                            int Ci, int Co, int T, int nchunks) {
    const int i = blockIdx.x * 256 + threadIdx.x;
    if (i >= nchunks * T * Co * 16) return;
    const int e = i & 15; int r = i >> 4;
    const int co = r % Co; r /= Co;
    const int t = r % T; const int ch = r / T;
    const int ci = ch * CC + e;
    dst[i] = (ci < Ci) ? src[((size_t)co * Ci + ci) * T + t] : 0.f;
}

extern "C" size_t osa_conv3d_small_co_packed_floats(int Ci, int Co, int kd, int kh, int kw) {
    return (size_t)nchunks_of(Ci) * kd * kh * kw * Co * 16;
}

extern "C" int osa_conv3d_small_co_pack_f32(const float* w_ref, float* w_packed, int Ci, int Co,
                                            int kd, int kh, int kw, void* stream) {
    OSA_REQUIRE(w_ref && w_packed, "conv3d_small_co_pack: NULL pointer");
    OSA_REQUIRE(Ci > 0 && Co >= 1 && Co <= 4 && kd > 0 && kh > 0 && kw > 0, "conv3d_small_co_pack: bad dims");
    const int n = (int)osa_conv3d_small_co_packed_floats(Ci, Co, kd, kh, kw);
    hipLaunchKernelGGL(small_co_pack_kernel, dim3(cdiv(n, 256)), dim3(256), 0, (hipStream_t)stream,
                       w_ref, w_packed, Ci, Co, kd * kh * kw, nchunks_of(Ci));
    OSA_LAUNCH_CHECK("conv3d_small_co_pack");
    return 0;
}

static int small_co_impl(const float* x, const float* w, bool packed, const float* bias,
                         const float* residual, float* y,
                         int B, int D, int H, int W, int Ci, int xCs, int Co, int yCs,
                         int kd, int kh, int kw, int pad_d, int pad_h, int pad_w,
                         void* stream);

extern "C" int osa_conv3d_small_co_ndhwc_f32(const float* x, const float* w_ref, const float* bias,
                                             const float* residual, float* y,
                                             int B, int D, int H, int W, int Ci, int xCs, int Co, int yCs,
                                             int kd, int kh, int kw, int pad_d, int pad_h, int pad_w,
                                             void* stream) {
    return small_co_impl(x, w_ref, false, bias, residual, y, B, D, H, W, Ci, xCs, Co, yCs, kd, kh, kw, pad_d, pad_h, pad_w, stream);
}

extern "C" int osa_conv3d_small_co_packed_ndhwc_f32(const float* x, const float* w_packed, const float* bias,
                                                    const float* residual, float* y,
                                                    int B, int D, int H, int W, int Ci, int xCs, int Co, int yCs,
                                                    int kd, int kh, int kw, int pad_d, int pad_h, int pad_w,
                                                    void* stream) {
    OSA_REQUIRE(((size_t)w_packed & 63) == 0, "conv3d_small_co_packed: packed weights must be 64-byte aligned");
    return small_co_impl(x, w_packed, true, bias, residual, y, B, D, H, W, Ci, xCs, Co, yCs, kd, kh, kw, pad_d, pad_h, pad_w, stream);
}

static int small_co_impl(const float* x, const float* w_ref, bool packed, const float* bias,
                         const float* residual, float* y,
                         int B, int D, int H, int W, int Ci, int xCs, int Co, int yCs,
                         int kd, int kh, int kw, int pad_d, int pad_h, int pad_w,
                         void* stream) {
    OSA_REQUIRE(x && w_ref && y, "conv3d_small_co: NULL pointer");
    OSA_REQUIRE(Co >= 1 && Co <= 4, "conv3d_small_co: Co=%d unsupported (1..4)", Co);
    OSA_REQUIRE(xCs % 4 == 0 && xCs >= Ci && ((size_t)x & 15) == 0, "conv3d_small_co: x must be 16-byte aligned, xCs %% 4 == 0");
    OSA_REQUIRE(kd == 2 * pad_d + 1 && kh == 2 * pad_h + 1 && kw == 2 * pad_w + 1, "conv3d_small_co: only 'same' convolutions");
    OSA_REQUIRE(kd * kh * kw <= MAX_TAPS, "conv3d_small_co: too many taps");
    OSA_REQUIRE(yCs >= Co, "conv3d_small_co: yCs < Co");
    ConvArgs a;
    memset(&a, 0, sizeof(a));
    a.x = x; a.y = y; a.res = residual; a.oscale = 1.f;
    a.B = B; a.Di = D; a.Hi = H; a.Wi = W; a.Ci = Ci; a.xCs = xCs;
    a.Do = D; a.Ho = H; a.Wo = W; a.Co = Co; a.yCs = yCs;
    a.Ad = D; a.Ah = H; a.Aw = W;
    a.isd = a.ish = a.isw = 1; a.os = 1;
    a.T = kd * kh * kw;
    int t = 0;
    for (int z = 0; z < kd; ++z) for (int yy = 0; yy < kh; ++yy) for (int xx = 0; xx < kw; ++xx, ++t) {
        a.td[t] = (signed char)(z - pad_d); a.th[t] = (signed char)(yy - pad_h); a.tw[t] = (signed char)(xx - pad_w);
    }
    a.nchunks = nchunks_of(Ci); a.CoP = Co;
    a.dmin = -pad_d; a.hmin = -pad_h; a.wmin = -pad_w;
    a.LD = 4 + 2 * pad_d; a.LH = 8 + 2 * pad_h; a.LW = 8 + 2 * pad_w;
    a.tilesD = cdiv(D, 4); a.tilesH = cdiv(H, 8); a.tilesW = cdiv(W, 8);
    finish_geometry(a, 8, true);
    hipStream_t st = (hipStream_t)stream;
    if (packed && Co == 1 && Ci == 32 && xCs == 32 && kd == 3 && kh == 3 && kw == 3 && !exp_set("OSA_NO_MARCH")) {
        a.tilesH = cdiv(H, CM_TH); a.tilesW = cdiv(W, CM_TW);
        const long long cols = (long long)B * a.tilesH * a.tilesW;
        int nseg = (int)((2048 + cols - 1) / cols);
        { const int o = exp_int("OSA_MARCH_NSEG", 0); if (o) nseg = o; }
        if (nseg > D / 8) nseg = D / 8;
        if (nseg < 1) nseg = 1;
        const int dseg = cdiv(D, nseg);
        nseg = cdiv(D, dseg);
        OSA_REQUIRE(cols * nseg < (1ll << 31), "conv3d_small_co: grid too large");
        OSA_REQUIRE((long long)H * W * xCs < (1ll << 31), "conv3d_small_co: plane too large");
        const size_t mlds = (size_t)CM_LH * CM_ROWQ * sizeof(float4);
        hipLaunchKernelGGL(classifier_march_kernel, dim3((unsigned)(cols * nseg)), dim3(256), mlds, st, a, w_ref, bias, dseg, nseg);
        OSA_LAUNCH_CHECK("conv3d_small_co (march)");
        return 0;
    }
    const size_t lds = ((size_t)a.LD * a.PlaneQ * 4 + (packed ? 0 : (size_t)a.nchunks * a.T * Co * 16)) * sizeof(float);
    OSA_REQUIRE(lds <= 160 * 1024, "conv3d_small_co: %zu B of LDS needed", lds);
    const long long nblk = (long long)B * a.tilesD * a.tilesH * a.tilesW;
    OSA_REQUIRE(nblk < (1ll << 31), "conv3d_small_co: grid too large");
    dim3 grid((unsigned)nblk), block(256);
#define OSA_SC_LAUNCH1(CO, WG)                                                                              \
    do {                                                                                                    \
        if (lds > 64 * 1024)                                                                                \
            (void)hipFuncSetAttribute((const void*)conv_small_co_tiled_kernel<CO, WG>,                      \
                                      hipFuncAttributeMaxDynamicSharedMemorySize, (int)lds);                \
        hipLaunchKernelGGL((conv_small_co_tiled_kernel<CO, WG>), grid, block, lds, st, a, w_ref, bias);     \
    } while (0)
#define OSA_SC_LAUNCH(CO) do { if (packed) OSA_SC_LAUNCH1(CO, true); else OSA_SC_LAUNCH1(CO, false); } while (0)
    switch (Co) {
        case 1: OSA_SC_LAUNCH(1); break;
        case 2: OSA_SC_LAUNCH(2); break;
        case 3: OSA_SC_LAUNCH(3); break;
        default: OSA_SC_LAUNCH(4); break;
    }
#undef OSA_SC_LAUNCH
    OSA_LAUNCH_CHECK("conv3d_small_co");
    return 0;
}

extern "C" int osa_conv_b_ring_mask(int mask) { const int prev = osa::g_b_ring_mask; osa::g_b_ring_mask = mask; osa::wgrad_set_multi_tile((mask >> 27) & 1); return prev; }
extern "C" long long osa_conv_b_ring_launches(void) { return osa::g_b_ring_launches; }
```

### openstereo_amd/csrc/layout.hip

```cpp
#include "osa_common.h"

namespace osa {

__global__ __launch_bounds__(256) void to_ndhwc_kernel(const float* __restrict__ x, float* __restrict__ y,
                                                       int C, long long S, int yCs, int c_off) {
    __shared__ float tile[32][33];
    const int b = blockIdx.z;
    const long long s0 = (long long)blockIdx.x * 32;
    const int c0 = blockIdx.y * 32;
    const int tx = threadIdx.x & 31, ty = threadIdx.x >> 5;
    for (int r = ty; r < 32; r += 8) {
        const int c = c0 + r; const long long s = s0 + tx;
        tile[r][tx] = (c < C && s < S) ? x[((size_t)b * C + c) * S + s] : 0.f;
    }
    __syncthreads();
    for (int r = ty; r < 32; r += 8) {
        const long long s = s0 + r; const int c = c0 + tx;
        if (c < C && s < S) y[((size_t)b * S + s) * yCs + c_off + c] = tile[tx][r];
    }
}

__global__ __launch_bounds__(256) void to_ncdhw_kernel(const float* __restrict__ x, float* __restrict__ y,
                                                       int C, long long S, int xCs, int c_off) {
    __shared__ float tile[32][33];
    const int b = blockIdx.z;
    const long long s0 = (long long)blockIdx.x * 32;
    const int c0 = blockIdx.y * 32;
    const int tx = threadIdx.x & 31, ty = threadIdx.x >> 5;
    for (int r = ty; r < 32; r += 8) {
        const long long s = s0 + r; const int c = c0 + tx;
        tile[r][tx] = (c < C && s < S) ? x[((size_t)b * S + s) * xCs + c_off + c] : 0.f;
    }
    __syncthreads();
    for (int r = ty; r < 32; r += 8) {
        const int c = c0 + r; const long long s = s0 + tx;
        if (c < C && s < S) y[((size_t)b * C + c) * S + s] = tile[tx][r];
    }
}

__global__ void amax_clear_kernel(float* meta) {
    if (threadIdx.x < OSA_AMAX_SLOTS) atomicExch(reinterpret_cast<unsigned*>(meta) + threadIdx.x * OSA_AMAX_STRIDE, 0u);
}

__global__ __launch_bounds__(256) void amax_kernel(const float* __restrict__ x, long long n, float* meta) {
    __shared__ float red[4];
    float am = 0.f;
    const long long n4 = n >> 2, stride = (long long)gridDim.x * 256;
    const float4* x4 = reinterpret_cast<const float4*>(x);
    for (long long i = (long long)blockIdx.x * 256 + threadIdx.x; i < n4; i += stride) {
        const float4 v = x4[i];
        am = fmaxf(am, fmaxf(fmaxf(fabsf(v.x), fabsf(v.y)), fmaxf(fabsf(v.z), fabsf(v.w))));
    }
    if (blockIdx.x == 0 && threadIdx.x < (n & 3)) am = fmaxf(am, fabsf(x[(n4 << 2) + threadIdx.x]));
    publish_amax(meta, am, 0u, red);
}

}

using namespace osa;

extern "C" int osa_amax_f32(const float* x, long long n, float* meta, void* stream) {
    OSA_REQUIRE(x && meta && n > 0, "amax: NULL pointer or empty tensor");
    OSA_REQUIRE(((size_t)x & 15) == 0, "amax: x must be 16-byte aligned");
    long long blocks = (n / 4 + 255) / 256;
    if (blocks > 2048) blocks = 2048;
    if (blocks < 1) blocks = 1;
    hipLaunchKernelGGL(amax_clear_kernel, dim3(1), dim3(64), 0, (hipStream_t)stream, meta);
    hipLaunchKernelGGL(amax_kernel, dim3((unsigned)blocks), dim3(256), 0, (hipStream_t)stream, x, n, meta);
    OSA_LAUNCH_CHECK("amax");
    return 0;
}

extern "C" int osa_ncdhw_to_ndhwc_f32(const float* x, float* y, int B, int C, long long S,
                                      int yCs, int c_off, void* stream) {
    OSA_REQUIRE(x && y, "ncdhw_to_ndhwc: NULL pointer");
    OSA_REQUIRE(B > 0 && C > 0 && S > 0 && c_off >= 0 && c_off + C <= yCs, "ncdhw_to_ndhwc: bad dims");
    OSA_REQUIRE(B <= 65535 && cdiv(C, 32) <= 65535, "ncdhw_to_ndhwc: grid too large");
    dim3 grid(cdiv(S, 32), cdiv(C, 32), B);
    hipLaunchKernelGGL(to_ndhwc_kernel, grid, dim3(256), 0, (hipStream_t)stream, x, y, C, S, yCs, c_off);
    OSA_LAUNCH_CHECK("ncdhw_to_ndhwc");
    return 0;
}

extern "C" int osa_ndhwc_to_ncdhw_f32(const float* x, float* y, int B, int C, long long S,
                                      int xCs, int c_off, void* stream) {
    OSA_REQUIRE(x && y, "ndhwc_to_ncdhw: NULL pointer");
    OSA_REQUIRE(B > 0 && C > 0 && S > 0 && c_off >= 0 && c_off + C <= xCs, "ndhwc_to_ncdhw: bad dims");
    OSA_REQUIRE(B <= 65535 && cdiv(C, 32) <= 65535, "ndhwc_to_ncdhw: grid too large");
    dim3 grid(cdiv(S, 32), cdiv(C, 32), B);
    hipLaunchKernelGGL(to_ncdhw_kernel, grid, dim3(256), 0, (hipStream_t)stream, x, y, C, S, xCs, c_off);
    OSA_LAUNCH_CHECK("ndhwc_to_ncdhw");
    return 0;
}
```

### openstereo_amd/csrc/torch_ext.cpp

```cpp
#include <ATen/ATen.h>
#include <c10/hip/HIPStream.h>
#include <torch/library.h>
#include <torch/csrc/autograd/custom_function.h>

#include "../../include/openstereo_amd.h"

namespace {

inline void* cur_stream() { return static_cast<void*>(c10::hip::getCurrentHIPStream().stream()); }

#define OSA_CALL(expr)                                                                     \
    do {                                                                                   \
        const int rc__ = (expr);                                                           \
        TORCH_CHECK(rc__ == 0, "openstereo_amd: ", #expr, " failed (", rc__, "): ", osa_last_error()); \
    } while (0)

inline const at::Tensor& gpu_f32(const at::Tensor& t, const char* name) {
    TORCH_CHECK(t.is_cuda(), "openstereo_amd: ", name, " is on ", t.device(), " -- the gfx950 engine has no CPU path");
    TORCH_CHECK(t.scalar_type() == at::kFloat, "openstereo_amd: ", name, " must be float32");
    return t;
}
inline const float* fp(const at::Tensor& t) { return t.data_ptr<float>(); }
inline const float* fpo(const c10::optional<at::Tensor>& t) { return (t.has_value() && t->defined()) ? t->data_ptr<float>() : nullptr; }
inline void* vp(const at::Tensor& t, int64_t off) { return static_cast<char*>(t.data_ptr()) + off * t.element_size(); }
// ... 433 lines not shown

at::Tensor softmax_softargmin_bwd(const at::Tensor& cost, const at::Tensor& dout) {
    gpu_f32(cost, "cost"); gpu_f32(dout, "dout");
    TORCH_CHECK(cost.dim() == 4 && dout.dim() == 3, "softmax_softargmin_bwd: cost [B,D,H,W], dout [B,H,W]");
    const auto c = cost.contiguous(), g = dout.contiguous();
    auto dc = at::empty_like(c);
    OSA_CALL(osa_softmax_softargmin_bwd_f32(fp(c), fp(g), dc.data_ptr<float>(), (int)c.size(0), (int)c.size(1), (int)c.size(2), (int)c.size(3), cur_stream()));
    return dc;
}

at::Tensor upsample_softargmin_bwd(const at::Tensor& cost_lowres, const at::Tensor& dout, int64_t maxdisp, int64_t h, int64_t w, bool align_corners) {
    gpu_f32(cost_lowres, "cost_lowres"); gpu_f32(dout, "dout");
    TORCH_CHECK(cost_lowres.dim() == 4 && dout.dim() == 3, "upsample_softargmin_bwd: cost [B,Dl,Hl,Wl], dout [B,h,w]");
    const auto c = cost_lowres.contiguous(), g = dout.contiguous();
    auto dc = at::empty_like(c);
    const size_t need = osa_upsample_softargmin_bwd_workspace_bytes((int)c.size(0), (int)c.size(1), (int)h, (int)w);
    auto ws = at::empty({(int64_t)((need + 3) / 4)}, c.options());
    OSA_CALL(osa_upsample_softargmin_bwd_ws_f32(fp(c), fp(g), dc.data_ptr<float>(), (int)c.size(0), (int)c.size(1), (int)c.size(2), (int)c.size(3), (int)maxdisp,
                                                (int)h, (int)w, align_corners ? 1 : 0, ws.data_ptr<float>(), need, cur_stream()));
    return dc;
}

std::tuple<at::Tensor, at::Tensor> softargmin_var_bwd(const at::Tensor& prob, const at::Tensor& disparity, const at::Tensor& dout, const at::Tensor& dvar) {
    gpu_f32(prob, "prob"); gpu_f32(disparity, "disparity"); gpu_f32(dout, "dout"); gpu_f32(dvar, "dvar");
    TORCH_CHECK(prob.dim() == 4 && dout.dim() == 3 && dvar.sizes() == dout.sizes(), "softargmin_var_bwd: prob [B,D,H,W], dout / dvar [B,H,W]");
    const auto p = prob.contiguous(), d = disparity.contiguous(), g = dout.contiguous(), gv = dvar.contiguous();
    TORCH_CHECK(d.numel() == g.numel() && g.size(0) == p.size(0) && g.size(1) == p.size(2) && g.size(2) == p.size(3), "softargmin_var_bwd: shapes disagree");
    auto dp = at::empty_like(p), dd = at::empty(d.sizes(), d.options());
    OSA_CALL(osa_softargmin_var_bwd_f32(fp(p), fp(d), fp(g), fp(gv), dp.data_ptr<float>(), dd.data_ptr<float>(), (int)p.size(0), (int)p.size(1), (int)p.size(2),
                                        (int)p.size(3), cur_stream()));
    return {dp, dd};
}

at::Tensor softmax_softargmin_var_bwd(const at::Tensor& cost, const at::Tensor& dout, const at::Tensor& dvar) {
    gpu_f32(cost, "cost"); gpu_f32(dout, "dout"); gpu_f32(dvar, "dvar");
    TORCH_CHECK(cost.dim() == 4 && dout.dim() == 3 && dvar.sizes() == dout.sizes(), "softmax_softargmin_var_bwd: cost [B,D,H,W], dout / dvar [B,H,W]");
    const auto c = cost.contiguous(), g = dout.contiguous(), gv = dvar.contiguous();
    TORCH_CHECK(g.size(0) == c.size(0) && g.size(1) == c.size(2) && g.size(2) == c.size(3), "softmax_softargmin_var_bwd: shapes disagree");
    auto dc = at::empty_like(c);
    OSA_CALL(osa_softmax_softargmin_var_bwd_f32(fp(c), fp(g), fp(gv), dc.data_ptr<float>(), (int)c.size(0), (int)c.size(1), (int)c.size(2), (int)c.size(3), cur_stream()));
    return dc;
}

at::Tensor upsample_softargmin_var_bwd(const at::Tensor& cost_lowres, const at::Tensor& dout, const at::Tensor& dvar, int64_t maxdisp, int64_t h, int64_t w,
                                       bool align_corners) {
    gpu_f32(cost_lowres, "cost_lowres"); gpu_f32(dout, "dout"); gpu_f32(dvar, "dvar");
    TORCH_CHECK(cost_lowres.dim() == 4 && dout.dim() == 3 && dvar.sizes() == dout.sizes(), "upsample_softargmin_var_bwd: cost [B,Dl,Hl,Wl], dout / dvar [B,h,w]");
    const auto c = cost_lowres.contiguous(), g = dout.contiguous(), gv = dvar.contiguous();
    TORCH_CHECK(g.size(0) == c.size(0) && g.size(1) == h && g.size(2) == w, "upsample_softargmin_var_bwd: shapes disagree");
    auto dc = at::empty_like(c);
    const size_t need = osa_upsample_softargmin_bwd_workspace_bytes((int)c.size(0), (int)c.size(1), (int)h, (int)w);
    auto ws = at::empty({(int64_t)((need + 3) / 4)}, c.options());
    OSA_CALL(osa_upsample_softargmin_var_bwd_ws_f32(fp(c), fp(g), fp(gv), dc.data_ptr<float>(), (int)c.size(0), (int)c.size(1), (int)c.size(2), (int)c.size(3),
                                                    (int)maxdisp, (int)h, (int)w, align_corners ? 1 : 0, ws.data_ptr<float>(), need, cur_stream()));
    return dc;
}

std::tuple<at::Tensor, bool> cost_volume_cl(const at::Tensor& gwc_feat, const c10::optional<at::Tensor>& cat_feat, int64_t B, int64_t num_groups, int64_t maxdisp,
                                            int64_t gwc_channels, int64_t cat_channels, int64_t gwc_off, bool mask_left, bool out_split,
                                            const c10::optional<at::Tensor>& gwc_meta, const c10::optional<at::Tensor>& cat_meta, const at::Tensor& out_meta) {
    gpu_f32(gwc_feat, "gwc_feat"); gpu_f32(out_meta, "out_meta");
    TORCH_CHECK(gwc_feat.dim() == 5 && gwc_feat.size(0) == 2 * B && gwc_feat.size(2) == 1 && gwc_feat.stride(1) == 1, "cost_volume_cl: gwc_feat must be NHWC [2B, Cs, 1, H, W]");
    const int64_t Gs = gwc_feat.size(1), H = gwc_feat.size(3), W = gwc_feat.size(4);
    const int64_t C = gwc_channels >= 0 ? gwc_channels : Gs - gwc_off;
    const float* lg = fp(gwc_feat) + gwc_off;
    const float* rg = lg + B * H * W * Gs;
    const float *lc = nullptr, *rc = nullptr;
    int64_t Cc = 0, cs = 0;
    if (cat_feat.has_value() && cat_feat->defined()) {
        gpu_f32(*cat_feat, "cat_feat");
        TORCH_CHECK(cat_feat->dim() == 5 && cat_feat->size(0) == 2 * B && cat_feat->size(3) == H && cat_feat->size(4) == W && cat_feat->stride(1) == 1,
                    "cost_volume_cl: cat_feat must be NHWC [2B, cs, 1, H, W] at the gwc features' resolution");
        cs = cat_feat->size(1); Cc = cat_channels >= 0 ? cat_channels : cs;
        lc = fp(*cat_feat); rc = lc + B * H * W * cs;
    }
    const int64_t nch = num_groups + 2 * Cc, VC = (nch + 3) / 4 * 4;
    auto out = at::empty({B, maxdisp, H, W, VC}, gwc_feat.options()).permute({0, 4, 1, 2, 3});
    if (VC != nch) out.zero_();
    const float* gm = fpo(gwc_meta); const float* cm = fpo(cat_meta);
    const bool split = out_split && VC == nch && (C == 0 || gm) && (Cc == 0 || cm) &&
        osa_build_volume_nhwc_split_eligible(lc, rc, out.data_ptr<float>(), (int)C, (int)num_groups, (int)Gs, (int)Cc, (int)cs, (int)VC, 0, (int)W, (int)maxdisp) == 1;
    if (split)
        OSA_CALL(osa_build_volume_nhwc_split_f16x3(lg, rg, (int)C, (int)num_groups, (int)Gs, lc, rc, (int)Cc, (int)cs, out.data_ptr<float>(), (int)VC, 0, (int)B, (int)H, (int)W,
                                                   (int)maxdisp, mask_left ? 1 : 0, gm, cm, out_meta.data_ptr<float>(), cur_stream()));
    else
        OSA_CALL(osa_build_volume_nhwc_f32(lg, rg, (int)C, (int)num_groups, (int)Gs, lc, rc, (int)Cc, (int)cs, out.data_ptr<float>(), (int)VC, 0, (int)B, (int)H, (int)W,
                                           (int)maxdisp, mask_left ? 1 : 0, out_meta.data_ptr<float>(), cur_stream()));
    return {out, split};
}

static size_t wgrad_workspace(at::IntArrayRef dims, int64_t prec, const char* who, const char* batch, int (&d)[22]) {
    TORCH_CHECK(dims.size() == 22, who, ": dims = [", batch, ", D, H, W, Ci, xCs, Do, Ho, Wo, Co, dyCs, kd, kh, kw, stride, pad x3, dil x3, transposed]");
    for (int i = 0; i < 22; ++i) d[i] = (int)dims[i];
    const auto query = prec == 0 ? osa_conv3d_wgrad_workspace_bytes : osa_conv3d_wgrad_f16x3_workspace_bytes;
    return query(d[0], d[1], d[2], d[3], d[4], d[6], d[7], d[8], d[9], d[11], d[12], d[13], d[14], d[15], d[16], d[17], d[18], d[19], d[20], d[21]);
}
struct WgradOperands {
    std::vector<const void*> x, dy;
    bool list, xh, dyh;
};
static bool wgrad_run(const char* who, const char* batch, const WgradOperands& t, at::Tensor& dw, at::IntArrayRef dims, int64_t prec,
                      const c10::optional<at::Tensor>& x_meta, const c10::optional<at::Tensor>& dy_meta) {
    TORCH_CHECK(prec == 2 || (!t.xh && !t.dyh), who, ": fp16 tensors exist in the native f16 form only (prec 2)");
    int d[22];
    const size_t need = wgrad_workspace(dims, prec, who, batch, d);
    if (need == 0) {
        TORCH_CHECK(prec != 0, who, ": unsupported layer");
        return false;
    }
    auto ws = at::empty({(int64_t)((need + 3) / 4)}, dw.options());
    void* st = cur_stream();
    const float* const x = static_cast<const float*>(t.x[0]); const float* const dy = static_cast<const float*>(t.dy[0]);
#define OSA_WG_DIMS d[0], d[1], d[2], d[3], d[4], d[5], d[6], d[7], d[8], d[9], d[10], d[11], d[12], d[13], d[14], d[15], d[16], d[17], d[18], d[19], d[20], d[21]
    if (t.list) OSA_CALL(osa_conv3d_wgrad_ws_multi((int)prec, t.x.data(), t.dy.data(), (int)t.x.size(), dw.data_ptr<float>(), OSA_WG_DIMS, fpo(x_meta), fpo(dy_meta),
                                                   t.xh ? 1 : 0, t.dyh ? 1 : 0, ws.data_ptr<float>(), need, st));
    else if (prec == 0) OSA_CALL(osa_conv3d_wgrad_ws_f32(x, dy, dw.data_ptr<float>(), OSA_WG_DIMS, ws.data_ptr<float>(), need, st));
    else if (prec == 1) OSA_CALL(osa_conv3d_wgrad_ws_f16x3(x, dy, dw.data_ptr<float>(), OSA_WG_DIMS, fpo(x_meta), fpo(dy_meta), ws.data_ptr<float>(), need, st));
    else OSA_CALL(osa_conv3d_wgrad_ws_f16(x, dy, dw.data_ptr<float>(), OSA_WG_DIMS, fpo(x_meta), fpo(dy_meta), t.xh ? 1 : 0, t.dyh ? 1 : 0, ws.data_ptr<float>(), need, st));
#undef OSA_WG_DIMS
    return true;
}
bool conv_wgrad(const at::Tensor& x, const at::Tensor& dy, at::Tensor dw, at::IntArrayRef dims, int64_t prec, const c10::optional<at::Tensor>& x_meta,
                const c10::optional<at::Tensor>& dy_meta) {
    gpu_f32(dw, "dw");
    const bool xh = x.scalar_type() == at::kHalf, dyh = dy.scalar_type() == at::kHalf;
    TORCH_CHECK(x.is_cuda() && dy.is_cuda() && (xh || x.scalar_type() == at::kFloat) && (dyh || dy.scalar_type() == at::kFloat), "conv_wgrad: x / dy must be CUDA fp32 or fp16 tensors");
    return wgrad_run("conv_wgrad", "B", {{x.data_ptr()}, {dy.data_ptr()}, false, xh, dyh}, dw, dims, prec, x_meta, dy_meta);
}

bool conv_wgrad_multi(at::TensorList xs, at::TensorList dys, at::Tensor dw, at::IntArrayRef dims, int64_t prec, const c10::optional<at::Tensor>& x_meta,
                      const c10::optional<at::Tensor>& dy_meta) {
    gpu_f32(dw, "dw");
    TORCH_CHECK(xs.size() >= 1 && xs.size() <= 24 && xs.size() == dys.size(), "conv_wgrad_multi: 1..24 (x, dy) pairs");
    WgradOperands t{{}, {}, true, xs[0].scalar_type() == at::kHalf, dys[0].scalar_type() == at::kHalf};
    for (size_t i = 0; i < xs.size(); ++i) {
        TORCH_CHECK(xs[i].is_cuda() && dys[i].is_cuda() && xs[i].scalar_type() == xs[0].scalar_type() && dys[i].scalar_type() == dys[0].scalar_type() &&
                    xs[i].sizes() == xs[0].sizes() && xs[i].strides() == xs[0].strides() && dys[i].sizes() == dys[0].sizes() && dys[i].strides() == dys[0].strides(),
                    "conv_wgrad_multi: the items must agree in device, dtype, shape and strides");
        t.x.push_back(xs[i].data_ptr()); t.dy.push_back(dys[i].data_ptr());
    }
    TORCH_CHECK((t.xh || xs[0].scalar_type() == at::kFloat) && (t.dyh || dys[0].scalar_type() == at::kFloat), "conv_wgrad_multi: fp32 or fp16 tensors");
    return wgrad_run("conv_wgrad_multi", "B total", t, dw, dims, prec, x_meta, dy_meta);
}

void to_cl(const at::Tensor& x, at::Tensor y, int64_t C, int64_t S, int64_t c_off) {
    gpu_f32(x, "x"); gpu_f32(y, "y");
    TORCH_CHECK(x.is_contiguous() && y.dim() == 5 && y.stride(1) == 1, "to_cl: x contiguous NCDHW, y NDHWC");
    OSA_CALL(osa_ncdhw_to_ndhwc_f32(fp(x), y.data_ptr<float>(), (int)x.size(0), (int)C, (long long)S, (int)y.size(1), (int)c_off, cur_stream()));
}
void to_ncdhw(const at::Tensor& x, at::Tensor y, int64_t C, int64_t S, int64_t c_off) {
    gpu_f32(x, "x"); gpu_f32(y, "y");
    TORCH_CHECK(y.is_contiguous() && x.dim() == 5 && x.stride(1) == 1, "to_ncdhw: x NDHWC, y contiguous NCDHW");
    OSA_CALL(osa_ndhwc_to_ncdhw_f32(fp(x), y.data_ptr<float>(), (int)x.size(0), (int)C, (long long)S, (int)x.size(1), (int)c_off, cur_stream()));
}

void conv_pack(const at::Tensor& w, at::Tensor packed, at::IntArrayRef geom, int64_t prec, const c10::optional<at::Tensor>& w_amax, const c10::optional<at::Tensor>& scale_out) {
    gpu_f32(w, "w"); gpu_f32(packed, "packed");
    TORCH_CHECK(geom.size() == 7 && w.is_contiguous(), "conv_pack: geom = [Ci, Co, kd, kh, kw, src_transposed, flip], w contiguous");
    const int g[7] = {(int)geom[0], (int)geom[1], (int)geom[2], (int)geom[3], (int)geom[4], (int)geom[5], (int)geom[6]};
    if (prec == 1) {
        TORCH_CHECK(w_amax.has_value() && scale_out.has_value(), "conv_pack: the f16x3 mode needs w_amax and scale_out (device tensors)");
        OSA_CALL(osa_conv3d_pack_ex_auto(fp(w), packed.data_ptr<float>(), g[0], g[1], g[2], g[3], g[4], g[5], g[6], fpo(w_amax), const_cast<float*>(fpo(scale_out)), cur_stream()));
    } else OSA_CALL(osa_conv3d_pack_ex(fp(w), packed.data_ptr<float>(), g[0], g[1], g[2], g[3], g[4], g[5], g[6], prec == 2 ? 2 : 0, 1.0f, cur_stream()));
}
void deconv_pack(const at::Tensor& w, at::Tensor packed, at::IntArrayRef geom, int64_t prec, const c10::optional<at::Tensor>& w_amax, const c10::optional<at::Tensor>& scale_out) {
    gpu_f32(w, "w"); gpu_f32(packed, "packed");
    TORCH_CHECK(geom.size() == 5 && w.is_contiguous(), "deconv_pack: geom = [Ci, Co, k, pad, flat], w contiguous");
    const int Ci = (int)geom[0], Co = (int)geom[1], k = (int)geom[2], pad = (int)geom[3];
    const bool flat = geom[4] != 0;
    float* dst = packed.data_ptr<float>();
    void* st = cur_stream();
    if (prec == 1) {
        TORCH_CHECK(w_amax.has_value() && scale_out.has_value(), "deconv_pack: the f16x3 mode needs w_amax and scale_out (device tensors)");
        float* so = const_cast<float*>(fpo(scale_out));
        if (flat) OSA_CALL(osa_deconv2d_pack_f16x3_auto(fp(w), dst, Ci, Co, k, pad, fpo(w_amax), so, st));
        else OSA_CALL(osa_deconv3d_pack_f16x3_auto(fp(w), dst, Ci, Co, k, pad, fpo(w_amax), so, st));
    } else if (prec == 2) {
        if (flat) OSA_CALL(osa_deconv2d_pack_f16(fp(w), dst, Ci, Co, k, pad, st));
        else OSA_CALL(osa_deconv3d_pack_f16(fp(w), dst, Ci, Co, k, pad, st));
    } else {
        if (flat) OSA_CALL(osa_deconv2d_pack_f32(fp(w), dst, Ci, Co, k, pad, st));
        else OSA_CALL(osa_deconv3d_pack_f32(fp(w), dst, Ci, Co, k, pad, st));
    }
}

inline osa_nhwc_ref nref(const at::Tensor& t, const char* name) {
    TORCH_CHECK(t.is_cuda() && t.dim() == 4 && t.stride(1) == 1 && (t.scalar_type() == at::kFloat || t.scalar_type() == at::kHalf),
                "openstereo_amd: ", name, " must be a CUDA fp32 / fp16 tensor [B,C,H,W] in NHWC memory order");
    TORCH_CHECK(t.stride(2) == t.size(3) * t.stride(3) && t.stride(0) == t.size(2) * t.stride(2), "openstereo_amd: ", name, " is not dense over its pixels");
    osa_nhwc_ref r;
    r.ptr = t.data_ptr(); r.cs = (int)t.stride(3); r.f16 = t.scalar_type() == at::kHalf ? 1 : 0;
    return r;
}
void gru_gates_rz_fwd(const at::Tensor& pre, const c10::optional<at::Tensor>& bz, const c10::optional<at::Tensor>& br, const at::Tensor& cz, const at::Tensor& cr,
                      const at::Tensor& h, at::Tensor z, at::Tensor rh) {
    const auto a = nref(pre, "pre"), b = nref(cz, "cz"), c = nref(cr, "cr"), d = nref(h, "h"), e = nref(z, "z"), f = nref(rh, "rh");
    OSA_CALL(osa_gru_gates_rz_fwd(&a, fpo(bz), fpo(br), &b, &c, &d, &e, &f, (long long)h.size(0) * h.size(2) * h.size(3), (int)h.size(1), cur_stream()));
}
void gru_gates_rz_bwd(const at::Tensor& pre, const c10::optional<at::Tensor>& bz, const c10::optional<at::Tensor>& br, const at::Tensor& cz, const at::Tensor& cr,
                      const at::Tensor& h, const at::Tensor& dz, const at::Tensor& drh, at::Tensor dpre, at::Tensor dh) {
    const auto a = nref(pre, "pre"), b = nref(cz, "cz"), c = nref(cr, "cr"), d = nref(h, "h"), e = nref(dz, "dz"), f = nref(drh, "drh"), g = nref(dpre, "dpre"), i = nref(dh, "dh");
    OSA_CALL(osa_gru_gates_rz_bwd(&a, fpo(bz), fpo(br), &b, &c, &d, &e, &f, &g, &i, (long long)h.size(0) * h.size(2) * h.size(3), (int)h.size(1), cur_stream()));
}
void gru_gates_q_fwd(const at::Tensor& z, const at::Tensor& qpre, const c10::optional<at::Tensor>& bq, const at::Tensor& cq, const at::Tensor& h, at::Tensor out) {
    const auto a = nref(z, "z"), b = nref(qpre, "qpre"), c = nref(cq, "cq"), d = nref(h, "h"), e = nref(out, "out");
    OSA_CALL(osa_gru_gates_q_fwd(&a, &b, fpo(bq), &c, &d, &e, (long long)h.size(0) * h.size(2) * h.size(3), (int)h.size(1), cur_stream()));
}
void gru_gates_q_bwd(const at::Tensor& z, const at::Tensor& qpre, const c10::optional<at::Tensor>& bq, const at::Tensor& cq, const at::Tensor& h, const at::Tensor& dout,
                     at::Tensor dz, at::Tensor dqpre, at::Tensor dh) {
    const auto a = nref(z, "z"), b = nref(qpre, "qpre"), c = nref(cq, "cq"), d = nref(h, "h"), e = nref(dout, "dout"), f = nref(dz, "dz"), g = nref(dqpre, "dqpre"), i = nref(dh, "dh");
    OSA_CALL(osa_gru_gates_q_bwd(&a, &b, fpo(bq), &c, &d, &e, &f, &g, &i, (long long)h.size(0) * h.size(2) * h.size(3), (int)h.size(1), cur_stream()));
}

struct RowList { float* ptr[10]; int len[10]; };
inline RowList row_list(at::TensorList ts, size_t split, const char* first, const char* rest) {
    RowList v;
    TORCH_CHECK(ts.size() <= 10, "row_list: ", ts.size(), " row tensors, at most 10");
    for (size_t q = 0; q < ts.size(); ++q) { v.ptr[q] = gpu_f32(ts[q], q < split ? first : rest).data_ptr<float>(); v.len[q] = (int)ts[q].size(-1); }
    return v;
}

void geo_lookup(at::TensorList levels, const at::Tensor& disp, const at::Tensor& coords_x, at::Tensor out, int64_t C, int64_t radius) {
    const size_t L = levels.size() / 2;
    TORCH_CHECK(L >= 1 && L <= 4 && levels.size() == 2 * L, "geo_lookup: levels = geo pyramid + corr pyramid, 1..4 levels each");
    gpu_f32(disp, "disp"); gpu_f32(coords_x, "coords_x"); gpu_f32(out, "out");
    const RowList v = row_list(levels, L, "geo level", "corr level");
    OSA_CALL(osa_geo_lookup_f32(v.ptr, v.ptr + L, v.len, v.len + L, (int)L, fp(disp), fp(coords_x), out.data_ptr<float>(), (int)disp.size(0), (int)disp.size(1), (int)disp.size(2), (int)C, (int)radius, cur_stream()));
}
static void geo_lookup_bwd_any(bool acc, at::TensorList dlevels, const at::Tensor& disp, const at::Tensor& coords_x, const at::Tensor& dout, int64_t C, int64_t radius) {
    const size_t L = dlevels.size() / 2;
    TORCH_CHECK(L >= 1 && L <= 4 && dlevels.size() == 2 * L, "geo_lookup_bwd: dlevels = gradients of the geo pyramid + of the corr pyramid");
    gpu_f32(disp, "disp"); gpu_f32(coords_x, "coords_x"); gpu_f32(dout, "dout");
    const RowList v = row_list(dlevels, L, "dgeo level", "dcorr level");
    if (acc) OSA_CALL(osa_geo_lookup_bwd_acc_f32(v.ptr, v.ptr + L, v.len, v.len + L, (int)L, fp(disp), fp(coords_x), fp(dout), (int)disp.size(0), (int)disp.size(1), (int)disp.size(2), (int)C, (int)radius, cur_stream()));
    else OSA_CALL(osa_geo_lookup_bwd_f32(v.ptr, v.ptr + L, v.len, v.len + L, (int)L, fp(disp), fp(coords_x), fp(dout), (int)disp.size(0), (int)disp.size(1), (int)disp.size(2), (int)C, (int)radius, cur_stream()));
}
void geo_lookup_bwd(at::TensorList dlevels, const at::Tensor& disp, const at::Tensor& coords_x, const at::Tensor& dout, int64_t C, int64_t radius) {
    geo_lookup_bwd_any(false, dlevels, disp, coords_x, dout, C, radius);
}
void geo_lookup_bwd_acc(at::TensorList dlevels, const at::Tensor& disp, const at::Tensor& coords_x, const at::Tensor& dout, int64_t C, int64_t radius) {
    geo_lookup_bwd_any(true, dlevels, disp, coords_x, dout, C, radius);
}

inline float* mfp(const c10::optional<at::Tensor>& t) { return (t.has_value() && t->defined() && t->numel()) ? t->data_ptr<float>() : nullptr; }
inline const at::Tensor* opt(const c10::optional<at::Tensor>& t) { return (t.has_value() && t->defined()) ? &*t : nullptr; }

void build_volume(const c10::optional<at::Tensor>& lg, const c10::optional<at::Tensor>& rg, int64_t G, const c10::optional<at::Tensor>& lc,
                  const c10::optional<at::Tensor>& rc, at::Tensor out, int64_t layout, int64_t VC, int64_t c_off, int64_t maxdisp, bool mask_left,
                  const c10::optional<at::Tensor>& meta) {
    const at::Tensor* g0 = opt(lg); const at::Tensor* c0 = opt(lc);
    TORCH_CHECK(g0 || c0, "build_volume: no features");
    const at::Tensor& ref = g0 ? *g0 : *c0;
    gpu_f32(ref, "features"); gpu_f32(out, "out");
    TORCH_CHECK(ref.dim() == 4, "build_volume: features are [B,C,H,W]");
    for (const auto* t : {opt(lg), opt(rg), opt(lc), opt(rc)})
        if (t) TORCH_CHECK(gpu_f32(*t, "features").is_contiguous() && t->size(0) == ref.size(0) && t->size(2) == ref.size(2) && t->size(3) == ref.size(3),
                           "build_volume: contiguous fp32 feature maps of one spatial shape");
    TORCH_CHECK((g0 != nullptr) == (opt(rg) != nullptr) && (c0 != nullptr) == (opt(rc) != nullptr), "build_volume: left and right maps come in pairs");
    OSA_CALL(osa_build_volume_f32(fpo(lg), fpo(rg), g0 ? (int)g0->size(1) : 0, (int)G, fpo(lc), fpo(rc), c0 ? (int)c0->size(1) : 0, out.data_ptr<float>(),
                                  (int)layout, (int)VC, (int)c_off, (int)ref.size(0), (int)ref.size(2), (int)ref.size(3), (int)maxdisp, mask_left ? 1 : 0, mfp(meta),
                                  cur_stream()));
}

void deconv_redir(const at::Tensor& x, int64_t x_off, const at::Tensor& packed, const c10::optional<at::Tensor>& scale, const c10::optional<at::Tensor>& shift,
                  at::Tensor out, int64_t out_off, at::IntArrayRef dims, at::IntArrayRef geom, const at::Tensor& rx, at::IntArrayRef rdims, const at::Tensor& rpacked,
                  const c10::optional<at::Tensor>& rscale, const c10::optional<at::Tensor>& rshift, double r_out_scale, int64_t prec, int64_t act, double slope,
                  double out_scale, at::TensorList metas) {
    gpu_f32(x, "x"); gpu_f32(out, "out"); gpu_f32(rx, "redir input"); gpu_f32(packed, "packed"); gpu_f32(rpacked, "redir packed");
    TORCH_CHECK(dims.size() == 8 && geom.size() == 3 && rdims.size() == 2, "deconv_redir: dims = [B, D, H, W, Ci, xCs, Co, yCs], geom = [k, pad, opad], rdims = [rxCs, rCi]");
    TORCH_CHECK(prec == 0 || prec == 1, "deconv_redir: f32 and f16x3 only (the f16 mode runs the 1x1x1 layer separately)");
    const int d[8] = {(int)dims[0], (int)dims[1], (int)dims[2], (int)dims[3], (int)dims[4], (int)dims[5], (int)dims[6], (int)dims[7]};
    const float* xp = (const float*)vp(x, x_off);
    float* yp = (float*)vp(out, out_off);
    if (prec == 0) {
        OSA_CALL(osa_deconv3d_redir_ndhwc_f32(xp, fp(packed), fpo(scale), fpo(shift), yp, d[0], d[1], d[2], d[3], d[4], d[5], d[6], d[7], (int)geom[0], (int)geom[1], (int)geom[2],
                                              fp(rx), (int)rdims[0], (int)rdims[1], fp(rpacked), fpo(rscale), fpo(rshift), (int)act, (float)slope, cur_stream()));
        return;
    }
    TORCH_CHECK(metas.size() == 7, "deconv_redir: the f16x3 mode takes the 7 range blocks of conv_ndhwc");
    auto mp = [&](size_t i) -> float* { return metas[i].defined() && metas[i].numel() ? metas[i].data_ptr<float>() : nullptr; };
    osa_f16x3_ranges rng{};
    rng.x_meta = mp(0); rng.residual_meta = mp(1); rng.redir_meta = mp(2); rng.y_meta = mp(3); rng.bound_coef = mp(4); rng.redir_bound_coef = mp(5); rng.weight_scale = mp(6);
    OSA_CALL(osa_deconv3d_redir_ndhwc_f16x3(xp, fp(packed), fpo(scale), fpo(shift), yp, d[0], d[1], d[2], d[3], d[4], d[5], d[6], d[7], (int)geom[0], (int)geom[1], (int)geom[2],
                                            fp(rx), (int)rdims[0], (int)rdims[1], fp(rpacked), fpo(rscale), fpo(rshift), (float)r_out_scale, (int)act, (float)slope,
                                            (float)out_scale, &rng, cur_stream()));
}

void small_co_conv(const at::Tensor& x, const at::Tensor& packed, const c10::optional<at::Tensor>& bias, const c10::optional<at::Tensor>& residual, at::Tensor y,
                   at::IntArrayRef dims, at::IntArrayRef geom) {
    gpu_f32(x, "x"); gpu_f32(packed, "packed"); gpu_f32(y, "y");
    TORCH_CHECK(dims.size() == 8 && geom.size() == 6, "small_co_conv: dims = [B, D, H, W, Ci, xCs, Co, yCs], geom = [kd, kh, kw, pd, ph, pw]");
    OSA_CALL(osa_conv3d_small_co_packed_ndhwc_f32(fp(x), fp(packed), fpo(bias), fpo(residual), y.data_ptr<float>(), (int)dims[0], (int)dims[1], (int)dims[2], (int)dims[3],
                                                  (int)dims[4], (int)dims[5], (int)dims[6], (int)dims[7], (int)geom[0], (int)geom[1], (int)geom[2], (int)geom[3], (int)geom[4],
                                                  (int)geom[5], cur_stream()));
}

void dwconv2d(const at::Tensor& x, const at::Tensor& packed, const c10::optional<at::Tensor>& scale, const c10::optional<at::Tensor>& shift,
              const c10::optional<at::Tensor>& add, at::Tensor y, at::IntArrayRef dims, at::IntArrayRef geom, int64_t act, const c10::optional<at::Tensor>& y_meta) {
    gpu_f32(x, "x"); gpu_f32(packed, "packed"); gpu_f32(y, "y");
    TORCH_CHECK(dims.size() == 7 && geom.size() == 7, "dwconv2d: dims = [B, Hi, Wi, C, xCs, yCs, aCs], geom = [kh, kw, stride, pad_h, pad_w, dil_h, dil_w]");
    OSA_CALL(osa_dwconv2d_nhwc_f32(fp(x), fp(packed), fpo(scale), fpo(shift), fpo(add), y.data_ptr<float>(), (int)dims[0], (int)dims[1], (int)dims[2], (int)dims[3], (int)dims[4],
                                   (int)dims[5], (int)dims[6], (int)geom[0], (int)geom[1], (int)geom[2], (int)geom[3], (int)geom[4], (int)geom[5], (int)geom[6], (int)act,
                                   mfp(y_meta), cur_stream()));
}

void dwconv2d_f16io(const at::Tensor& x, const at::Tensor& packed, const c10::optional<at::Tensor>& scale, const c10::optional<at::Tensor>& shift,
// ... 429 lines not shown
        static auto op = c10::Dispatcher::singleton().findSchemaOrThrow("osa_native::upsample_softargmin_bwd", "")
            .typed<at::Tensor(const at::Tensor&, const at::Tensor&, int64_t, int64_t, int64_t, bool)>();
        auto dc = op.call(c.to(at::kFloat), gy[0].to(at::kFloat), ctx->saved_data["maxdisp"].toInt(), ctx->saved_data["h"].toInt(), ctx->saved_data["w"].toInt(),
                          ctx->saved_data["align"].toBool());
        return {dc.to(c.scalar_type()), at::Tensor(), at::Tensor(), at::Tensor(), at::Tensor()};
    }
};
at::Tensor upsample_softargmin_autograd(const at::Tensor& c, int64_t maxdisp, int64_t h, int64_t w, bool align) { return UpsampleSoftargminFn::apply(c, maxdisp, h, w, align); }

using tensor_pair = std::tuple<at::Tensor, at::Tensor>;
struct SoftargminVarFn : torch::autograd::Function<SoftargminVarFn> {
    static variable_list forward(AutogradContext* ctx, const at::Tensor& p, const at::Tensor& d) {
        at::AutoDispatchBelowADInplaceOrView g;
        ctx->save_for_backward({p, d});
        static auto op = c10::Dispatcher::singleton().findSchemaOrThrow("osa_native::softargmin_var", "").typed<tensor_pair(const at::Tensor&, const at::Tensor&)>();
        auto [out, var] = op.call(p, d);
        return {out, var};
    }
    static variable_list backward(AutogradContext* ctx, variable_list gy) {
        const auto sv = ctx->get_saved_variables();
        static auto op = c10::Dispatcher::singleton().findSchemaOrThrow("osa_native::softargmin_var_bwd", "")
            .typed<tensor_pair(const at::Tensor&, const at::Tensor&, const at::Tensor&, const at::Tensor&)>();
        auto [dp, dd] = op.call(sv[0].to(at::kFloat), sv[1].to(at::kFloat), gy[0].to(at::kFloat), gy[1].to(at::kFloat));
        return {dp.to(sv[0].scalar_type()), dd.to(sv[1].scalar_type())};
    }
};
tensor_pair softargmin_var_autograd(const at::Tensor& p, const at::Tensor& d) {
    auto r = SoftargminVarFn::apply(p, d);
    return {r[0], r[1]};
}

struct SoftmaxSoftargminVarFn : torch::autograd::Function<SoftmaxSoftargminVarFn> {
    static variable_list forward(AutogradContext* ctx, const at::Tensor& c) {
        at::AutoDispatchBelowADInplaceOrView g;
        ctx->save_for_backward({c});
        static auto op = c10::Dispatcher::singleton().findSchemaOrThrow("osa_native::softmax_softargmin_var", "").typed<tensor_pair(const at::Tensor&)>();
        auto [out, var] = op.call(c);
        return {out, var};
    }
    static variable_list backward(AutogradContext* ctx, variable_list gy) {
        const auto c = ctx->get_saved_variables()[0];
        static auto op = c10::Dispatcher::singleton().findSchemaOrThrow("osa_native::softmax_softargmin_var_bwd", "")
            .typed<at::Tensor(const at::Tensor&, const at::Tensor&, const at::Tensor&)>();
        return {op.call(c.to(at::kFloat), gy[0].to(at::kFloat), gy[1].to(at::kFloat)).to(c.scalar_type())};
    }
};
tensor_pair softmax_softargmin_var_autograd(const at::Tensor& c) {
    auto r = SoftmaxSoftargminVarFn::apply(c);
    return {r[0], r[1]};
}

struct UpsampleSoftargminVarFn : torch::autograd::Function<UpsampleSoftargminVarFn> {
    static variable_list forward(AutogradContext* ctx, const at::Tensor& c, int64_t maxdisp, int64_t h, int64_t w, bool align) {
        at::AutoDispatchBelowADInplaceOrView g;
        ctx->save_for_backward({c});
        ctx->saved_data["maxdisp"] = maxdisp; ctx->saved_data["h"] = h; ctx->saved_data["w"] = w; ctx->saved_data["align"] = align;
        static auto op = c10::Dispatcher::singleton().findSchemaOrThrow("osa_native::upsample_softargmin_var", "")
            .typed<tensor_pair(const at::Tensor&, int64_t, int64_t, int64_t, bool)>();
        auto [out, var] = op.call(c, maxdisp, h, w, align);
        return {out, var};
    }
    static variable_list backward(AutogradContext* ctx, variable_list gy) {
        const auto c = ctx->get_saved_variables()[0];
        static auto op = c10::Dispatcher::singleton().findSchemaOrThrow("osa_native::upsample_softargmin_var_bwd", "")
            .typed<at::Tensor(const at::Tensor&, const at::Tensor&, const at::Tensor&, int64_t, int64_t, int64_t, bool)>();
        auto dc = op.call(c.to(at::kFloat), gy[0].to(at::kFloat), gy[1].to(at::kFloat), ctx->saved_data["maxdisp"].toInt(), ctx->saved_data["h"].toInt(),
                          ctx->saved_data["w"].toInt(), ctx->saved_data["align"].toBool());
        return {dc.to(c.scalar_type()), at::Tensor(), at::Tensor(), at::Tensor(), at::Tensor()};
    }
};
tensor_pair upsample_softargmin_var_autograd(const at::Tensor& c, int64_t maxdisp, int64_t h, int64_t w, bool align) {
    auto r = UpsampleSoftargminVarFn::apply(c, maxdisp, h, w, align);
    return {r[0], r[1]};
}

int64_t abi_version() { return osa_abi_version(); }

void noop_boxed(const c10::OperatorHandle& op, torch::jit::Stack* stack) {
    TORCH_INTERNAL_ASSERT(op.schema().returns().empty(), "noop_boxed serves ops without results only: ", op.schema().name());
    torch::jit::drop(*stack, op.schema().arguments().size());
}
std::tuple<at::Tensor, bool> cost_volume_cl_meta(const at::Tensor& gwc_feat, const c10::optional<at::Tensor>& cat_feat, int64_t B, int64_t num_groups, int64_t maxdisp,
                                                 int64_t gwc_channels, int64_t cat_channels, int64_t gwc_off, bool mask_left, bool out_split,
                                                 const c10::optional<at::Tensor>& gwc_meta, const c10::optional<at::Tensor>& cat_meta, const at::Tensor& out_meta) {
    TORCH_CHECK(gwc_feat.dim() == 5 && gwc_feat.size(0) == 2 * B && gwc_feat.size(2) == 1, "cost_volume_cl: gwc_feat must be NHWC [2B, Cs, 1, H, W]");
    const int64_t Gs = gwc_feat.size(1), H = gwc_feat.size(3), W = gwc_feat.size(4);
    const int64_t C = gwc_channels >= 0 ? gwc_channels : Gs - gwc_off;
    int64_t Cc = 0, cs = 0;
    const bool has_cat = cat_feat.has_value() && cat_feat->defined();
    if (has_cat) { cs = cat_feat->size(1); Cc = cat_channels >= 0 ? cat_channels : cs; }
    const int64_t nch = num_groups + 2 * Cc, VC = (nch + 3) / 4 * 4;
    auto out = at::empty({B, maxdisp, H, W, VC}, gwc_feat.options()).permute({0, 4, 1, 2, 3});
    const float* al = reinterpret_cast<const float*>(static_cast<uintptr_t>(4096));
    float* ao = reinterpret_cast<float*>(static_cast<uintptr_t>(8192));
    const bool gm = gwc_meta.has_value() && gwc_meta->defined(), cm = cat_meta.has_value() && cat_meta->defined();
    const bool split = out_split && VC == nch && (C == 0 || gm) && (Cc == 0 || cm) &&
        osa_build_volume_nhwc_split_eligible(has_cat ? al : nullptr, has_cat ? al : nullptr, ao, (int)C, (int)num_groups, (int)Gs, (int)Cc, (int)cs, (int)VC, 0, (int)W, (int)maxdisp) == 1;
    (void)mask_left; (void)out_meta;
    return {out, split};
}
bool conv_wgrad_meta(const at::Tensor& x, const at::Tensor& dy, at::Tensor dw, at::IntArrayRef dims, int64_t prec, const c10::optional<at::Tensor>& x_meta,
                     const c10::optional<at::Tensor>& dy_meta) {
    int d[22];
    const size_t need = wgrad_workspace(dims, prec, "conv_wgrad", "B", d);
    TORCH_CHECK(need != 0 || prec != 0, "conv_wgrad: unsupported layer");
    (void)x; (void)dy; (void)dw; (void)x_meta; (void)dy_meta;
    return need != 0;
}
bool conv_wgrad_multi_meta(at::TensorList xs, at::TensorList dys, at::Tensor dw, at::IntArrayRef dims, int64_t prec, const c10::optional<at::Tensor>& x_meta,
                           const c10::optional<at::Tensor>& dy_meta) {
    TORCH_CHECK(dims.size() == 22 && xs.size() >= 1 && xs.size() == dys.size(), "conv_wgrad_multi: dims of 22 entries, equally long lists");
    return conv_wgrad_meta(xs[0], dys[0], dw, dims, prec, x_meta, dy_meta);
}

}

TORCH_LIBRARY(osa_native, m) {
    m.def("abi_version() -> int", &abi_version);
    m.def("gwc_volume(Tensor left, Tensor right, int maxdisp, int groups) -> Tensor");
    m.def("mr_volume(Tensor left, Tensor right, Tensor patch0, Tensor patch1, int maxdisp, int s_range, int m_range, bool channels_last=False) -> (Tensor, Tensor, Tensor)");
    m.def("mv2_block3d_pack(Tensor w_expand, Tensor w_dw, Tensor w_project, Tensor scale1, Tensor shift1, Tensor scale2, Tensor shift2, Tensor scale3, Tensor shift3) -> Tensor");
    m.def("mv2_block3d(Tensor x, Tensor packed, int hidden, int out_channels, int stride, bool residual) -> Tensor");
    m.def("mv2_block2d_pack(Tensor w_expand, Tensor w_dw, Tensor w_project, Tensor scale1, Tensor shift1, Tensor scale2, Tensor shift2, Tensor scale3, Tensor shift3) -> Tensor");
    m.def("mv2_block2d(Tensor x, Tensor packed, int hidden, int out_channels, int stride, bool residual, Tensor? addend, bool relu) -> Tensor");
    m.def("interlaced_volume_pack(Tensor w1, Tensor w2, Tensor w3, Tensor w4, Tensor scale1, Tensor shift1, Tensor scale2, Tensor shift2, Tensor scale3, Tensor shift3, Tensor scale4, Tensor shift4) -> Tensor");
    m.def("interlaced_volume(Tensor left, Tensor right, Tensor packed, int maxdisp, int k2, int k3, int features) -> Tensor");
    m.def("disparity_attention_pack(Tensor[] params, int nhead) -> Tensor");
    m.def("disparity_attention(Tensor cv, Tensor pe, Tensor packed, int C, int nhead, int ff, int layers) -> Tensor");
    m.def("mr_volume_bwd(Tensor? dv0, Tensor? dv1, Tensor? dv2, Tensor left, Tensor right, Tensor patch0, Tensor patch1, int maxdisp, int s_range, int m_range, bool channels_last) -> (Tensor, Tensor, Tensor, Tensor)");
    m.def("concat_volume(Tensor left, Tensor right, int maxdisp, bool mask_left=True) -> Tensor");
    m.def("corr_volume(Tensor left, Tensor right, int maxdisp) -> Tensor");
    m.def("softargmin(Tensor prob) -> Tensor");
    m.def("softmax_softargmin(Tensor cost, bool return_prob=False) -> (Tensor, Tensor)");
    m.def("upsample_softargmin(Tensor cost_lowres, int maxdisp, int h, int w, bool align_corners=False) -> Tensor");
    m.def("context_upsample(Tensor disp_low, Tensor up_weights, int scale=4, bool softmax_weights=False, float gain=1.0) -> Tensor");
    m.def("conv_ndhwc(Tensor x, int x_off, Tensor packed, Tensor? scale, Tensor? shift, Tensor? residual, int res_off, Tensor(a!) out, int out_off, "
          "Tensor? gate, int[] dims, int[] geom, int family, int prec, int act, float slope, float out_scale, Tensor[] metas) -> ()");
    m.def("volume_bwd(Tensor dvol, Tensor? left, Tensor? right, int[] shape, int maxdisp, int groups, bool concat, bool mask_left) -> (Tensor, Tensor)");
    m.def("softargmin_bwd(Tensor dout, int D) -> Tensor");
    m.def("softmax_softargmin_bwd(Tensor cost, Tensor dout) -> Tensor");
    m.def("upsample_softargmin_bwd(Tensor cost_lowres, Tensor dout, int maxdisp, int h, int w, bool align_corners=False) -> Tensor");
    m.def("softargmin_var(Tensor prob, Tensor disparity) -> (Tensor, Tensor)");
    m.def("softmax_softargmin_var(Tensor cost) -> (Tensor, Tensor)");
    m.def("upsample_softargmin_var(Tensor cost_lowres, int maxdisp, int h, int w, bool align_corners=False) -> (Tensor, Tensor)");
    m.def("softargmin_var_bwd(Tensor prob, Tensor disparity, Tensor dout, Tensor dvar) -> (Tensor, Tensor)");
    m.def("softmax_softargmin_var_bwd(Tensor cost, Tensor dout, Tensor dvar) -> Tensor");
    m.def("upsample_softargmin_var_bwd(Tensor cost_lowres, Tensor dout, Tensor dvar, int maxdisp, int h, int w, bool align_corners=False) -> Tensor");
    m.def("cost_volume_cl(Tensor gwc_feat, Tensor? cat_feat, int B, int num_groups, int maxdisp, int gwc_channels, int cat_channels, int gwc_off, bool mask_left, "
          "bool out_split, Tensor? gwc_meta, Tensor? cat_meta, Tensor(a!) out_meta) -> (Tensor, bool)");
    m.def("conv_wgrad(Tensor x, Tensor dy, Tensor(a!) dw, int[] dims, int prec, Tensor? x_meta, Tensor? dy_meta) -> bool");
    m.def("conv_wgrad_multi(Tensor[] xs, Tensor[] dys, Tensor(a!) dw, int[] dims, int prec, Tensor? x_meta, Tensor? dy_meta) -> bool");
    m.def("to_cl(Tensor x, Tensor(a!) y, int C, int S, int c_off) -> ()");
    m.def("to_ncdhw(Tensor x, Tensor(a!) y, int C, int S, int c_off) -> ()");
    m.def("conv_pack(Tensor w, Tensor(a!) packed, int[] geom, int prec, Tensor? w_amax, Tensor(b!)? scale_out) -> ()");
    m.def("deconv_pack(Tensor w, Tensor(a!) packed, int[] geom, int prec, Tensor? w_amax, Tensor(b!)? scale_out) -> ()");
    m.def("gru_gates_rz_fwd(Tensor pre, Tensor? bias_z, Tensor? bias_r, Tensor cz, Tensor cr, Tensor h, Tensor(a!) z, Tensor(b!) rh) -> ()");
    m.def("gru_gates_rz_bwd(Tensor pre, Tensor? bias_z, Tensor? bias_r, Tensor cz, Tensor cr, Tensor h, Tensor dz, Tensor drh, Tensor(a!) dpre, Tensor(b!) dh) -> ()");
    m.def("gru_gates_q_fwd(Tensor z, Tensor qpre, Tensor? bias_q, Tensor cq, Tensor h, Tensor(a!) out) -> ()");
    m.def("gru_gates_q_bwd(Tensor z, Tensor qpre, Tensor? bias_q, Tensor cq, Tensor h, Tensor dout, Tensor(a!) dz, Tensor(b!) dqpre, Tensor(c!) dh) -> ()");
    m.def("geo_lookup(Tensor[] levels, Tensor disp, Tensor coords_x, Tensor(a!) out, int C, int radius) -> ()");
    m.def("geo_lookup_bwd(Tensor(a!)[] dlevels, Tensor disp, Tensor coords_x, Tensor dout, int C, int radius) -> ()");
    m.def("geo_lookup_bwd_acc(Tensor(a!)[] dlevels, Tensor disp, Tensor coords_x, Tensor dout, int C, int radius) -> ()");
    m.def("build_volume(Tensor? left_gwc, Tensor? right_gwc, int groups, Tensor? left_cat, Tensor? right_cat, Tensor(a!) out, int layout, int vol_channels, int c_off, "
          "int maxdisp, bool mask_left, Tensor(b!)? meta) -> ()");
    m.def("deconv_redir(Tensor x, int x_off, Tensor packed, Tensor? scale, Tensor? shift, Tensor(a!) out, int out_off, int[] dims, int[] geom, Tensor rx, int[] rdims, "
          "Tensor rpacked, Tensor? rscale, Tensor? rshift, float r_out_scale, int prec, int act, float slope, float out_scale, Tensor[] metas) -> ()");
    m.def("small_co_conv(Tensor x, Tensor packed, Tensor? bias, Tensor? residual, Tensor(a!) y, int[] dims, int[] geom) -> ()");
    m.def("dwconv2d(Tensor x, Tensor packed, Tensor? scale, Tensor? shift, Tensor? add, Tensor(a!) y, int[] dims, int[] geom, int act, Tensor(b!)? y_meta) -> ()");
    m.def("dwconv2d_f16io(Tensor x, Tensor packed, Tensor? scale, Tensor? shift, Tensor(a!) y, int[] dims, int[] geom, int act, Tensor(b!)? y_meta) -> ()");
    m.def("gru_combine(Tensor z, int z_off, Tensor q, Tensor h, Tensor(a!) out, int[] dims, Tensor(b!)? out_meta) -> ()");
    m.def("resample_nhwc(Tensor x, Tensor(a!) y, int y_off, int kind, int[] dims, Tensor? x_meta, Tensor(b!)? y_meta) -> ()");
    m.def("disp_update(Tensor(a!) disp, Tensor? delta, int delta_cs, Tensor(b!) disp4, Tensor(c!) slot, int slot_off, int slot_cs, int npix, Tensor(d!)? disp4_meta, "
          "Tensor(e!)? slot_meta) -> ()");
    m.def("geo_lookup_nhwc(Tensor[] levels, Tensor disp, Tensor coords_x, Tensor(a!) out, int out_cs, int[] bhw, int C, int radius) -> ()");
    m.def("geo_lookup_mr(Tensor[] sources, Tensor disp, Tensor coords_x, Tensor(a!)[] outs, int C, int radius) -> ()");
    m.def("geo_lookup_mr_nhwc(Tensor[] sources, Tensor disp, Tensor coords_x, Tensor(a!)[] outs, int[] out_cs, int[] bhw, int C, int radius) -> ()");
    m.def("geo_lookup_mr_bwd_acc(Tensor(a!)[] dsources, Tensor disp, Tensor coords_x, Tensor[] douts, int C, int radius) -> ()");
    m.def("allpairs_corr(Tensor fmap1, Tensor fmap2, Tensor(a!) corr) -> ()");
    m.def("geo_rows(Tensor volume, Tensor(a!) rows, int C) -> ()");
    m.def("avgpool_rows(Tensor x, Tensor(a!) y) -> ()");
    m.def("weight_pack(Tensor w, Tensor(a!) packed, int family, int prec, int[] geom, float wscale) -> ()");
    m.def("cat_fms(Tensor reference_fm, Tensor target_fm, Tensor(a!) out, Tensor disp_index) -> ()");
    m.def("pair_volume(Tensor left, Tensor right, Tensor(a!) out, int groups, int planes, int mode) -> ()");
    m.def("channel_sums(Tensor dy, Tensor? x, Tensor? x_shift, Tensor? dx_scale, int P, int C, int dy_cs, int x_cs) -> (Tensor, Tensor)");
    m.def("context_upsample_logits(Tensor disp_low, Tensor logits, int scale, float gain) -> Tensor");
    m.def("context_upsample_logits_bwd(Tensor disp_low, Tensor logits, Tensor dout, int scale, float gain) -> (Tensor, Tensor)");
    m.def("channel_affine(Tensor u, Tensor? v, Tensor a, Tensor? b, Tensor c0, int P, int C, int u_cs, int v_cs, bool relu) -> Tensor");
    m.def("channel_sums_multi(Tensor[] dys, int P, int C, int dy_cs) -> Tensor");
    m.def("instnorm_nhwc(Tensor x, Tensor(a!) out, int out_off, int[] dims, float eps, int act, float slope, Tensor(b!) workspace, Tensor(c!)? y_meta) -> ()");
    m.def("preprocess_pair(Tensor left_hwc, Tensor right_hwc, Tensor(a!) out, int[] pad_size, float[] mean, float[] std, bool channels_last) -> ()");
    m.def("amax_into(Tensor t, Tensor(a!) meta) -> ()");
}

TORCH_LIBRARY_IMPL(osa_native, CUDA, m) {
    m.impl("gwc_volume", &gwc_volume);
    m.impl("mr_volume", &mr_volume);
    m.impl("mr_volume_bwd", &mr_volume_bwd);
    m.impl("mv2_block3d_pack", &mv2_pack<MV2_3D>);
    m.impl("mv2_block3d", &mv2_block3d);
    m.impl("mv2_block2d_pack", &mv2_pack<MV2_2D>);
    m.impl("mv2_block2d", &mv2_block2d);
    m.impl("interlaced_volume_pack", &interlaced_volume_pack);
    m.impl("interlaced_volume", &interlaced_volume);
    m.impl("disparity_attention_pack", &disparity_attention_pack);
    m.impl("disparity_attention", &disparity_attention);
    m.impl("concat_volume", &concat_volume);
    m.impl("corr_volume", &corr_volume);
    m.impl("softargmin", &softargmin);
    m.impl("softmax_softargmin", &softmax_softargmin);
    m.impl("upsample_softargmin", &upsample_softargmin);
    m.impl("context_upsample", &context_upsample);
    m.impl("conv_ndhwc", &conv_ndhwc);
    m.impl("volume_bwd", &volume_bwd);
    m.impl("softargmin_bwd", &softargmin_bwd);
    m.impl("softmax_softargmin_bwd", &softmax_softargmin_bwd);
    m.impl("upsample_softargmin_bwd", &upsample_softargmin_bwd);
    m.impl("softargmin_var", &softargmin_var);
    m.impl("softmax_softargmin_var", &softmax_softargmin_var);
    m.impl("upsample_softargmin_var", &upsample_softargmin_var);
    m.impl("softargmin_var_bwd", &softargmin_var_bwd);
    m.impl("softmax_softargmin_var_bwd", &softmax_softargmin_var_bwd);
    m.impl("upsample_softargmin_var_bwd", &upsample_softargmin_var_bwd);
    m.impl("cost_volume_cl", &cost_volume_cl);
    m.impl("conv_wgrad", &conv_wgrad);
    m.impl("conv_wgrad_multi", &conv_wgrad_multi);
    m.impl("to_cl", &to_cl);
    m.impl("to_ncdhw", &to_ncdhw);
    m.impl("conv_pack", &conv_pack);
    m.impl("deconv_pack", &deconv_pack);
    m.impl("gru_gates_rz_fwd", &gru_gates_rz_fwd);
    m.impl("gru_gates_rz_bwd", &gru_gates_rz_bwd);
    m.impl("gru_gates_q_fwd", &gru_gates_q_fwd);
    m.impl("gru_gates_q_bwd", &gru_gates_q_bwd);
    m.impl("geo_lookup", &geo_lookup);
    m.impl("geo_lookup_bwd", &geo_lookup_bwd);
    m.impl("geo_lookup_bwd_acc", &geo_lookup_bwd_acc);
    m.impl("build_volume", &build_volume);
    m.impl("deconv_redir", &deconv_redir);
    m.impl("small_co_conv", &small_co_conv);
    m.impl("dwconv2d", &dwconv2d);
    m.impl("dwconv2d_f16io", &dwconv2d_f16io);
    m.impl("gru_combine", &gru_combine);
    m.impl("resample_nhwc", &resample_nhwc);
    m.impl("disp_update", &disp_update);
    m.impl("geo_lookup_nhwc", &geo_lookup_nhwc);
    m.impl("geo_lookup_mr", &geo_lookup_mr);
    m.impl("geo_lookup_mr_nhwc", &geo_lookup_mr_nhwc);
    m.impl("geo_lookup_mr_bwd_acc", &geo_lookup_mr_bwd_acc);
    m.impl("allpairs_corr", &allpairs_corr);
    m.impl("geo_rows", &geo_rows);
    m.impl("avgpool_rows", &avgpool_rows);
    m.impl("weight_pack", &weight_pack);
    m.impl("cat_fms", &cat_fms);
    m.impl("pair_volume", &pair_volume);
    m.impl("instnorm_nhwc", &instnorm_nhwc);
    m.impl("channel_sums", &channel_sums);
    m.impl("channel_sums_multi", &channel_sums_multi);
    m.impl("channel_affine", &channel_affine);
    m.impl("context_upsample_logits", &context_upsample_logits);
    m.impl("context_upsample_logits_bwd", &context_upsample_logits_bwd);
    m.impl("preprocess_pair", &preprocess_pair);
    m.impl("amax_into", &amax_into);
}

TORCH_LIBRARY_IMPL(osa_native, Meta, m) {
    m.impl("gwc_volume", &gwc_volume_meta);
    m.impl("mr_volume", &mr_volume_meta);
    m.impl("mr_volume_bwd", &mr_volume_bwd_meta);
    m.impl("mv2_block3d_pack", &mv2_pack_meta<MV2_3D>);
    m.impl("mv2_block3d", &mv2_block3d_meta);
    m.impl("mv2_block2d_pack", &mv2_pack_meta<MV2_2D>);
    m.impl("mv2_block2d", &mv2_block2d_meta);
    m.impl("interlaced_volume_pack", &interlaced_volume_pack_meta);
    m.impl("interlaced_volume", &interlaced_volume_meta);
    m.impl("disparity_attention_pack", &disparity_attention_pack_meta);
    m.impl("disparity_attention", &disparity_attention_meta);
    m.impl("concat_volume", &concat_volume_meta);
    m.impl("corr_volume", &corr_volume_meta);
    m.impl("softargmin", &softargmin_meta);
    m.impl("softmax_softargmin", &softmax_softargmin_meta);
    m.impl("upsample_softargmin", &upsample_softargmin_meta);
    m.impl("context_upsample", &context_upsample_meta);
    m.impl("volume_bwd", &volume_bwd_meta);
    m.impl("softargmin_bwd", &softargmin_bwd_meta);
    m.impl("softmax_softargmin_bwd", &softmax_softargmin_bwd_meta);
    m.impl("upsample_softargmin_bwd", &upsample_softargmin_bwd_meta);
    m.impl("softargmin_var", &softargmin_var_meta);
    m.impl("softmax_softargmin_var", &softmax_softargmin_var_meta);
    m.impl("upsample_softargmin_var", &upsample_softargmin_var_meta);
    m.impl("softargmin_var_bwd", &softargmin_var_bwd_meta);
    m.impl("softmax_softargmin_var_bwd", &softmax_softargmin_var_bwd_meta);
    m.impl("upsample_softargmin_var_bwd", &upsample_softargmin_var_bwd_meta);
    m.impl("cost_volume_cl", &cost_volume_cl_meta);
    m.impl("conv_wgrad", &conv_wgrad_meta);
    m.impl("conv_wgrad_multi", &conv_wgrad_multi_meta);
    m.impl("channel_sums", &channel_sums_meta);
    m.impl("channel_sums_multi", &channel_sums_multi_meta);
    m.impl("channel_affine", &channel_affine_meta);
    m.impl("context_upsample_logits", &context_upsample_logits_meta);
    m.impl("context_upsample_logits_bwd", &context_upsample_logits_bwd_meta);
    for (const char* name : {"conv_ndhwc", "to_cl", "to_ncdhw", "conv_pack", "deconv_pack", "gru_gates_rz_fwd", "gru_gates_rz_bwd", "gru_gates_q_fwd", "gru_gates_q_bwd",
                             "geo_lookup", "geo_lookup_bwd", "geo_lookup_bwd_acc", "build_volume", "deconv_redir", "small_co_conv", "dwconv2d", "dwconv2d_f16io", "gru_combine", "resample_nhwc", "disp_update",
                             "geo_lookup_nhwc", "geo_lookup_mr", "geo_lookup_mr_nhwc", "geo_lookup_mr_bwd_acc", "allpairs_corr", "geo_rows", "avgpool_rows", "weight_pack", "cat_fms", "pair_volume", "instnorm_nhwc", "preprocess_pair",
                             "amax_into"})
        m.impl(name, torch::CppFunction::makeFromBoxedFunction<&noop_boxed>());
}

TORCH_LIBRARY_IMPL(osa_native, Autograd, m) {
    m.impl("gwc_volume", &gwc_volume_autograd);
    m.impl("mr_volume", &mr_volume_autograd);
    m.impl("concat_volume", &concat_volume_autograd);
    m.impl("corr_volume", &corr_volume_autograd);
    m.impl("softargmin", &softargmin_autograd);
    m.impl("softmax_softargmin", &softmax_softargmin_autograd);
    m.impl("upsample_softargmin", &upsample_softargmin_autograd);
    m.impl("softargmin_var", &softargmin_var_autograd);
    m.impl("softmax_softargmin_var", &softmax_softargmin_var_autograd);
    m.impl("upsample_softargmin_var", &upsample_softargmin_var_autograd);
}
```

### openstereo_amd/models/gwcnet.py

```python
from __future__ import annotations

import os

import torch
import torch.nn as nn

import torch.nn.functional as F

from .. import autograd as AG
from .. import amp, ops, timing
from ..engine import is_split, chains, cached_pack, PackedConv3d, SmallCoConv3d, ACT_NONE, ACT_RELU


def run_train(mod, x):
    if isinstance(mod, (nn.Conv3d, nn.ConvTranspose3d)):
        return AG.conv_module(mod, x)
    if isinstance(mod, nn.Sequential):
        for child in mod:
            x = run_train(child, x)
        return x
    if isinstance(mod, nn.modules.batchnorm._BatchNorm):
        return AG.bn_module(mod, x)
    return mod(x)


def _cb2(cin, cout, k, stride, pad, dil):
    return nn.Sequential(
        nn.Conv2d(cin, cout, k, stride, dil if dil > 1 else pad, dil, bias=False),
        nn.BatchNorm2d(cout))


TRAIN_BACKBONE_ENGINE = os.environ.get("OSA_GWC_TRAIN_BACKBONE_ENGINE", "0") == "1"
_FUSE_REDIR = os.environ.get("OSA_FUSE_REDIR", "1") != "0"
_SPLIT_ACT = os.environ.get("OSA_SPLIT_ACT", "1") != "0"
_VOL_SPLIT = os.environ.get("OSA_VOL_SPLIT", "1") != "0"

class _ResBlock(nn.Module):
    def __init__(self, cin, cout, stride, shortcut, pad, dil):
        super().__init__()
        self.conv1 = nn.Sequential(_cb2(cin, cout, 3, stride, pad, dil), nn.ReLU(inplace=True))
        self.conv2 = _cb2(cout, cout, 3, 1, pad, dil)
        self.downsample = shortcut

    def forward(self, x):
        y = self.conv2(self.conv1(x))
        return y + (x if self.downsample is None else self.downsample(x))


class _Features(nn.Module):

    def __init__(self, concat_feature=True, concat_feature_channel=12):
        super().__init__()
        self.concat_feature = concat_feature
        self.firstconv = nn.Sequential(
            _cb2(3, 32, 3, 2, 1, 1), nn.ReLU(inplace=True),
            _cb2(32, 32, 3, 1, 1, 1), nn.ReLU(inplace=True),
            _cb2(32, 32, 3, 1, 1, 1), nn.ReLU(inplace=True))
        self._cin = 32
        self.layer1 = self._stage(32, 3, 1, 1, 1)
        self.layer2 = self._stage(64, 16, 2, 1, 1)
        self.layer3 = self._stage(128, 3, 1, 1, 1)
        self.layer4 = self._stage(128, 3, 1, 1, 2)
        if concat_feature:
            self.lastconv = nn.Sequential(
                _cb2(320, 128, 3, 1, 1, 1), nn.ReLU(inplace=True),
                nn.Conv2d(128, concat_feature_channel, 1, 1, 0, bias=False))

    def _stage(self, cout, n, stride, pad, dil):
        shortcut = None
        if stride != 1 or self._cin != cout:
            shortcut = nn.Sequential(nn.Conv2d(self._cin, cout, 1, stride, bias=False), nn.BatchNorm2d(cout))
        blocks = [_ResBlock(self._cin, cout, stride, shortcut, pad, dil)]
        self._cin = cout
        blocks += [_ResBlock(cout, cout, 1, None, pad, dil) for _ in range(1, n)]
        return nn.Sequential(*blocks)

    def _pack(self):
        def build():
            P = lambda cb, act: PackedConv3d(cb[0], cb[1], act)
            fc = self.firstconv
            pk = {"first": [P(fc[0], ACT_RELU), P(fc[2], ACT_RELU), P(fc[4], ACT_RELU)], "layers": []}
            for layer in (self.layer1, self.layer2, self.layer3, self.layer4):
                pk["layers"].append([(P(b.conv1[0], ACT_RELU), P(b.conv2, ACT_NONE),
                                      None if b.downsample is None else P(b.downsample, ACT_NONE)) for b in layer])
            if self.concat_feature:
                pk["last"] = (P(self.lastconv[0], ACT_RELU), PackedConv3d(self.lastconv[2]))
            return pk
        return cached_pack(self, "_pk", build)

    def forward_cl(self, img):
        pk = self._pack()
        sp = _SPLIT_ACT and chains(pk["first"][0].precision)
        x = ops.to_cl(img.unsqueeze(2))
        for conv in pk["first"]:
            x = conv(x, out_split=sp)
        xoff, cat, slices = 0, None, {1: 0, 2: 64, 3: 192}
        for li, blocks in enumerate(pk["layers"]):
            for bi, (c1, c2, ds) in enumerate(blocks):
                last = bi == len(blocks) - 1
                y = c1(x, x_off=xoff, out_split=sp)
                if ds is not None:
                    skip, soff = ds(x, x_off=xoff, out_split=sp), 0
                else:
                    skip, soff = x, xoff
                if last and li >= 1:
                    if cat is None:
                        N_, _, _, h4, w4 = y.shape
                        cat = ops.empty_cl(N_, 320, 1, h4, w4, y.device)
                    c2(y, residual=skip, res_off=soff, out=cat, out_off=slices[li])
                    x, xoff = cat, slices[li]
                else:
                    x, xoff = c2(y, residual=skip, res_off=soff, out_split=sp and is_split(skip)), 0
        if not self.concat_feature:
            return cat, None
        l0, l2 = pk["last"]
        return cat, l2(l0(cat, out_split=sp))

    def forward(self, x):
        x = self.layer1(self.firstconv(x))
        l2 = self.layer2(x)
        l3 = self.layer3(l2)
        l4 = self.layer4(l3)
        out = {"gwc_feature": torch.cat((l2, l3, l4), dim=1)}
        if self.concat_feature:
            out["concat_feature"] = self.lastconv(out["gwc_feature"])
        return out


class GwcBackbone(nn.Module):
    use_engine = True

    def __init__(self, use_concat_volume=True, concat_channels=12):
        super().__init__()
        self.use_concat_volume = use_concat_volume
        self.concat_channels = concat_channels if use_concat_volume else 0
        self.feature_extraction = _Features(use_concat_volume, self.concat_channels)

    @amp.contract("cast")
    def forward(self, inputs):
        left, right = inputs["left"], inputs["right"]
        B = left.shape[0]
        if self.use_engine and not self.training and ops.on_engine(left):
            gwc, catf = self.forward_cl(left, right)
            f = {"gwc_feature": ops.to_ncdhw(gwc)[:, :, 0]}
            if catf is not None:
                f["concat_feature"] = ops.to_ncdhw(catf, self.concat_channels)[:, :, 0]
        elif self.training:
            with timing.span("backbone2d", left.shape[2], left.shape[3]):
                if TRAIN_BACKBONE_ENGINE and ops.on_engine(left):
                    with AG.engine_convs():
                        return {"ref_feature": self.feature_extraction(left), "tgt_feature": self.feature_extraction(right)}
                return {"ref_feature": self.feature_extraction(left), "tgt_feature": self.feature_extraction(right)}
        else:
            with timing.span("backbone2d", left.shape[2], left.shape[3]):
                f = self.feature_extraction(torch.cat((left, right), 0))
        ref = {k: v[:B] for k, v in f.items()}
        tgt = {k: v[B:] for k, v in f.items()}
        return {"ref_feature": ref, "tgt_feature": tgt}

    def forward_cl(self, left, right):
        with timing.span("backbone2d_engine", left.shape[2], left.shape[3]):
            return self.feature_extraction.forward_cl(torch.cat((left, right), 0))


class GwcVolumeCostProcessor(nn.Module):

    def __init__(self, maxdisp=192, downsample=4, num_groups=40, use_concat_volume=True, *args, **kwargs):
        super().__init__()
        self.maxdisp, self.downsample = maxdisp, downsample
        self.num_groups, self.use_concat_volume = num_groups, use_concat_volume

    def build_gwc_volume(self, refimg_fea, targetimg_fea):
        return ops.build_gwc_volume(refimg_fea, targetimg_fea, self.maxdisp // self.downsample, self.num_groups)

    def build_concat_volume(self, refimg_fea, targetimg_fea):
        return ops.build_concat_volume(refimg_fea, targetimg_fea, self.maxdisp // self.downsample)

    @amp.contract("volume")
    def forward(self, inputs):
        l, r = inputs["ref_feature"], inputs["tgt_feature"]
        cat = self.use_concat_volume
        if self.training or (torch.is_grad_enabled() and l["gwc_feature"].requires_grad):
            D4 = self.maxdisp // self.downsample
            vol = AG.build_gwc_volume(l["gwc_feature"], r["gwc_feature"], D4, self.num_groups)
            if cat:
                vol = torch.cat((vol, AG.build_concat_volume(l["concat_feature"], r["concat_feature"], D4)), 1)
            return {"cost_volume": vol}
        vol = ops.build_cost_volume_cl(
            l["gwc_feature"], r["gwc_feature"], self.num_groups,
            l["concat_feature"] if cat else None, r["concat_feature"] if cat else None,
            maxdisp=self.maxdisp // self.downsample)
        return {"cost_volume": vol}

    def input_output(self):
        return {"inputs": ["ref_feature", "tgt_feature"], "outputs": ["cost_volume"]}


def _cb3(cin, cout, k, stride, pad):
    return nn.Sequential(nn.Conv3d(cin, cout, k, stride, pad, bias=False), nn.BatchNorm3d(cout))


class Hourglass(nn.Module):

    def __init__(self, in_channels):
        super().__init__()
        c = in_channels
        self.conv1 = nn.Sequential(_cb3(c, 2 * c, 3, 2, 1), nn.ReLU(inplace=True))
        self.conv2 = nn.Sequential(_cb3(2 * c, 2 * c, 3, 1, 1), nn.ReLU(inplace=True))
        self.conv3 = nn.Sequential(_cb3(2 * c, 4 * c, 3, 2, 1), nn.ReLU(inplace=True))
        self.conv4 = nn.Sequential(_cb3(4 * c, 4 * c, 3, 1, 1), nn.ReLU(inplace=True))
        self.conv5 = nn.Sequential(
            nn.ConvTranspose3d(4 * c, 2 * c, 3, padding=1, output_padding=1, stride=2, bias=False),
            nn.BatchNorm3d(2 * c))
        self.conv6 = nn.Sequential(
            nn.ConvTranspose3d(2 * c, c, 3, padding=1, output_padding=1, stride=2, bias=False),
            nn.BatchNorm3d(c))
        self.redir1 = _cb3(c, c, 1, 1, 0)
        self.redir2 = _cb3(2 * c, 2 * c, 1, 1, 0)
        self._packed = None

    def _pack(self):
        P = PackedConv3d
        return cached_pack(self, "_packed", lambda: dict(
            c1=P(self.conv1[0][0], self.conv1[0][1], ACT_RELU), c2=P(self.conv2[0][0], self.conv2[0][1], ACT_RELU),
            c3=P(self.conv3[0][0], self.conv3[0][1], ACT_RELU), c4=P(self.conv4[0][0], self.conv4[0][1], ACT_RELU),
            c5=P(self.conv5[0], self.conv5[1], ACT_RELU), c6=P(self.conv6[0], self.conv6[1], ACT_RELU),
            r1=P(self.redir1[0], self.redir1[1], ACT_NONE), r2=P(self.redir2[0], self.redir2[1], ACT_NONE)))

    def forward_cl(self, x, split=False):
        p = self._pack()
        s = dict(out_split=True) if split else {}
        c1 = p["c1"](x, **s)
        c2 = p["c2"](c1, **s)
        c4 = p["c4"](p["c3"](c2, **s), **s)
        fuse = _FUSE_REDIR and p["c5"].precision != "f16"
        if fuse and p["r2"].Ci <= 64:
            c5 = p["c5"](c4, redir=(p["r2"], c2), **s)
        else:
            c5 = p["c5"](c4, residual=p["r2"](c2, **s), **s)
        if fuse and p["r1"].Ci <= 32:
            return p["c6"](c5, redir=(p["r1"], x), **s)
        return p["c6"](c5, residual=p["r1"](x, **s), **s)

    def forward_train(self, x):
        c1 = run_train(self.conv1, x)
        c2 = run_train(self.conv2, c1)
        c4 = run_train(self.conv4, run_train(self.conv3, c2))
        c5 = F.relu(run_train(self.conv5, c4) + run_train(self.redir2, c2))
        return F.relu(run_train(self.conv6, c5) + run_train(self.redir1, x))

    @amp.contract("cast")
    def forward(self, x):
        if self.training or (torch.is_grad_enabled() and x.requires_grad):
            return self.forward_train(x)
        return ops.to_ncdhw(self.forward_cl(ops.to_cl(x)), channels=x.shape[1])


STAGE_STASH = None


class GwcDispProcessor(nn.Module):

    def __init__(self, maxdisp=192, downsample=4, num_groups=40, use_concat_volume=True, concat_channels=12,
                 *args, **kwargs):
        super().__init__()
        self.maxdisp, self.downsample, self.num_groups = maxdisp, downsample, num_groups
        self.use_concat_volume = use_concat_volume
        self.concat_channels = concat_channels if use_concat_volume else 0
        cin = self.num_groups + self.concat_channels * 2
        relu = lambda: nn.ReLU(inplace=True)
        self.dres0 = nn.Sequential(_cb3(cin, 32, 3, 1, 1), relu(), _cb3(32, 32, 3, 1, 1), relu())
        self.dres1 = nn.Sequential(_cb3(32, 32, 3, 1, 1), relu(), _cb3(32, 32, 3, 1, 1))
        self.dres2, self.dres3, self.dres4 = Hourglass(32), Hourglass(32), Hourglass(32)
        for i in range(4):
            setattr(self, f"classif{i}", nn.Sequential(
                _cb3(32, 32, 3, 1, 1), relu(), nn.Conv3d(32, 1, kernel_size=3, padding=1, stride=1, bias=False)))
        self._packed = None

    def reset_engine(self):
        self._packed = None
        for h in (self.dres2, self.dres3, self.dres4):
            h._packed = None

    def _pack(self):
        P = PackedConv3d
        return cached_pack(self, "_packed", lambda: dict(
            d00=P(self.dres0[0][0], self.dres0[0][1], ACT_RELU), d02=P(self.dres0[2][0], self.dres0[2][1], ACT_RELU),
            d10=P(self.dres1[0][0], self.dres1[0][1], ACT_RELU), d12=P(self.dres1[2][0], self.dres1[2][1], ACT_NONE),
            k0=P(self.classif3[0][0], self.classif3[0][1], ACT_RELU), k2=SmallCoConv3d(self.classif3[2])),
            mods=(self.dres0, self.dres1, self.classif3))

    def aggregate_cl(self, volume):
        p = self._pack()
        split = _SPLIT_ACT and chains(p["d00"].precision)
        s = dict(out_split=True) if split else {}
        if STAGE_STASH is not None:
            k = lambda name, t: (STAGE_STASH.append((name, t.clone())), t)[1]
            d00 = k("dres0.0", p["d00"](k("volume", volume), **s))
            cost0 = k("dres0.2", p["d02"](d00, **s))
            cost0 = k("dres1", p["d12"](k("dres1.0", p["d10"](cost0, **s)), residual=cost0, **s))
            out1 = k("hourglass1", self.dres2.forward_cl(cost0, split))
            out2 = k("hourglass2", self.dres3.forward_cl(out1, split))
            out3 = k("hourglass3", self.dres4.forward_cl(out2, split))
            return k("classif3.2", p["k2"](k("classif3.0", p["k0"](out3))))
        cost0 = p["d02"](p["d00"](volume, **s), **s)
        cost0 = p["d12"](p["d10"](cost0, **s), residual=cost0, **s)
        out3 = self.dres4.forward_cl(self.dres3.forward_cl(self.dres2.forward_cl(cost0, split), split), split)
        return p["k2"](p["k0"](out3))

    def forward_train(self, inputs):
        volume = inputs["cost_volume"]
        h, w = inputs["left"].shape[2:]
        cost0 = run_train(self.dres0, volume)
        cost0 = run_train(self.dres1, cost0) + cost0
        out1 = self.dres2.forward_train(cost0)
        out2 = self.dres3.forward_train(out1)
        out3 = self.dres4.forward_train(out2)
        preds = []
        for head, feat in ((self.classif0, cost0), (self.classif1, out1), (self.classif2, out2), (self.classif3, out3)):
            cost = run_train(head, feat)
            preds.append(AG.upsample_softargmin(cost, self.maxdisp, h, w, align_corners=False))
        return {"training_disp": {"disp": {"disp_ests": preds}}}

    def forward(self, inputs, return_variance=False):
        if self.training:
            return self.forward_train(inputs)
        volume = inputs["cost_volume"]
        h, w = inputs["left"].shape[2:]
        if not ops.is_cl(volume) or volume.shape[1] % 4:
            volume = ops.to_cl(volume)
        cost3 = self.aggregate_cl(volume)
        if return_variance:
            pred3, var3 = ops.upsample_softargmin(cost3, self.maxdisp, h, w, align_corners=False, return_variance=True)
            return {"inference_disp": {"disp_est": pred3, "disp_var": var3}}
        pred3 = ops.upsample_softargmin(cost3, self.maxdisp, h, w, align_corners=False)
        return {"inference_disp": {"disp_est": pred3}}

    def input_output(self):
        return {"inputs": ["cost_volume", "disp_shape"],
                "outputs": ["training_disp", "inference_disp", "visual_summary"]}


class _Cfg(dict):
    __getattr__ = dict.__getitem__


GWCNET_G_SCENEFLOW = _Cfg(MAX_DISP=192, USE_CONCAT_VOLUME=True, CONCAT_CHANNELS=12, DOWNSAMPLE=4, NUM_GROUPS=40)


class GwcNet(nn.Module):

    return_variance = False

    def __init__(self, cfgs=GWCNET_G_SCENEFLOW):
        super().__init__()
        self.maxdisp = cfgs.MAX_DISP
        kw = dict(maxdisp=self.maxdisp, downsample=cfgs.DOWNSAMPLE, num_groups=cfgs.NUM_GROUPS,
                  use_concat_volume=cfgs.USE_CONCAT_VOLUME)
        self.Backbone = GwcBackbone(use_concat_volume=cfgs.USE_CONCAT_VOLUME, concat_channels=cfgs.CONCAT_CHANNELS)
        self.CostProcessor = GwcVolumeCostProcessor(**kw)
        self.DispProcessor = GwcDispProcessor(concat_channels=cfgs.CONCAT_CHANNELS, **kw)

    def reset_engine(self):
        self.Backbone.feature_extraction._pk = None
        self.DispProcessor.reset_engine()

    def forward(self, inputs):
        if self.Backbone.use_engine and not self.training and ops.on_engine(inputs["left"]):
            B = inputs["left"].shape[0]
            gwc, catf = self.Backbone.forward_cl(inputs["left"], inputs["right"])
            if STAGE_STASH is not None:
                STAGE_STASH.append(("backbone gwc", gwc.clone()))
                if catf is not None:
                    STAGE_STASH.append(("backbone concat", catf.clone()))
            cp = self.CostProcessor
            vol = ops.build_cost_volume_from_cl(gwc, cp.num_groups, catf if cp.use_concat_volume else None, B,
                                                cp.maxdisp // cp.downsample,
                                                cat_channels=self.Backbone.concat_channels or None,
                                                out_split=_SPLIT_ACT and _VOL_SPLIT and self.DispProcessor._pack()["d00"].precision == "f16x3")
            if getattr(vol, "_osa_split", False):
                dp = self.DispProcessor
                h, w = inputs["left"].shape[2:]
                if getattr(self, "return_variance", False):
                    pred, var = ops.upsample_softargmin(dp.aggregate_cl(vol), dp.maxdisp, h, w, align_corners=False, return_variance=True)
                    return {"disp_pred": pred, "disp_var": var}
                return {"disp_pred": ops.upsample_softargmin(dp.aggregate_cl(vol), dp.maxdisp, h, w, align_corners=False)}
            inputs["cost_volume"] = vol
        else:
            inputs.update(self.Backbone(inputs))
            inputs.update(self.CostProcessor(inputs))
        if not self.training and getattr(self, "return_variance", False):
            est = self.DispProcessor(inputs, return_variance=True)["inference_disp"]
            return {"disp_pred": est["disp_est"], "disp_var": est["disp_var"]}
        disp_out = self.DispProcessor(inputs)
        if self.training:
            ests = disp_out["training_disp"]["disp"]["disp_ests"]
            return {"disp_preds": ests, "disp_pred": ests[-1]}
        return {"disp_pred": disp_out["inference_disp"]["disp_est"]}

    def get_loss(self, model_preds, input_data, static=False):
        disp_gt = input_data["disp"]
        mask = (disp_gt < self.maxdisp) & (disp_gt > 0)
        loss = 0.0
        for disp_est, weight in zip(model_preds["disp_preds"], [0.5, 0.5, 0.7, 1.0]):
            if static:
                m = mask.to(disp_est.dtype)
                loss = loss + weight * (F.smooth_l1_loss(disp_est, disp_gt, reduction="none") * m).sum() / m.sum()
            else:
                loss = loss + weight * F.smooth_l1_loss(disp_est[mask], disp_gt[mask], reduction="mean")
        return loss, {"scalar/train/loss_disp": loss.detach() if static else loss.item()}
```

### openstereo_amd/ops.py

```python
from __future__ import annotations

import torch

from . import _ext, _lib, timing
from .ranges import attach_meta, new_meta

NCDHW, NDHWC = 0, 1


def on_engine(t) -> bool:
    return t.is_cuda


def _stream() -> int:
    return torch.cuda.current_stream().cuda_stream


def _chk(t: torch.Tensor, name: str, ndim: int | None = None) -> torch.Tensor:
    if not isinstance(t, torch.Tensor):
        raise TypeError(f"{name} must be a torch.Tensor")
    if not t.is_cuda:
        raise _lib.EngineError(f"{name} is on {t.device}: the gfx950 engine has no CPU path")
    if ndim is not None and t.dim() != ndim:
        raise ValueError(f"{name} must be {ndim}-D, got shape {tuple(t.shape)}")
    return t


def _f32c(t: torch.Tensor) -> torch.Tensor:
    if t.dtype != torch.float32:
        t = t.float()
    return t if t.is_contiguous() else t.contiguous()


def _sum_dtype(*ts):
    if torch.is_autocast_enabled("cuda"):
        return torch.float32
    dt = ts[0].dtype
    for t in ts[1:]:
        dt = torch.promote_types(dt, t.dtype)
    return dt


def empty_cl(B, C, D, H, W, device, dtype=torch.float32) -> torch.Tensor:
    return torch.empty((B, D, H, W, C), device=device, dtype=dtype).permute(0, 4, 1, 2, 3)


def is_cl(t: torch.Tensor) -> bool:
    return t.dim() == 5 and t.permute(0, 2, 3, 4, 1).is_contiguous()


def to_cl(x: torch.Tensor, pad_to: int = 4) -> torch.Tensor:
    _chk(x, "x", 5)
    if is_cl(x) and x.shape[1] % pad_to == 0 and x.dtype == torch.float32:
        return x
    xs = _f32c(x)
    B, Cn, D, H, W = xs.shape
    Cp = (Cn + pad_to - 1) // pad_to * pad_to
    y = empty_cl(B, Cp, D, H, W, x.device)
    if Cp != Cn:
        y.zero_()
    _ext.load().to_cl(xs, y, Cn, D * H * W, 0)
    return y


def to_ncdhw(x: torch.Tensor, channels: int | None = None) -> torch.Tensor:
    assert not getattr(x, "_osa_split", False), "split activation tensors are internal to engine layer chains"
    _chk(x, "x", 5)
    if not is_cl(x):
        return x.contiguous()
    if x.dtype != torch.float32:
        raise _lib.EngineError(f"to_ncdhw takes an fp32 NDHWC tensor, got {x.dtype} (an f16-mode chain tensor is internal to its layer chain)")
    B, Cs, D, H, W = x.shape
    Cn = Cs if channels is None else channels
    y = torch.empty((B, Cn, D, H, W), device=x.device, dtype=torch.float32)
    _ext.load().to_ncdhw(x, y, Cn, D * H * W, 0)
    return y


def _build(lg, rg, G, lc, rc, maxdisp, mask_left=True, vol_channels=None):
    ref = lg if lg is not None else lc
    B, _, H, W = ref.shape
    Cg = lg.shape[1] if lg is not None else 0
    Cc = lc.shape[1] if lc is not None else 0
    nch = (G if Cg else 0) + 2 * Cc
    VC = nch if vol_channels is None else vol_channels
    out = empty_cl(B, VC, maxdisp, H, W, ref.device)
    if VC > nch:
        out.zero_()
    meta = attach_meta(out)
    with timing.span("build_volume", Cg, G, Cc, NDHWC, maxdisp, H, W):
        _ext.load().build_volume(lg, rg, G, lc, rc, out, NDHWC, VC, 0, maxdisp, bool(mask_left), meta)
    return out


def build_gwc_volume(refimg_fea, targetimg_fea, maxdisp, num_groups):
    _chk(refimg_fea, "refimg_fea", 4); _chk(targetimg_fea, "targetimg_fea", 4)
    B, Cn, H, W = refimg_fea.shape
    assert Cn % num_groups == 0
    with timing.span("build_volume", Cn, num_groups, 0, NCDHW, maxdisp, H, W):
        v = _ext.load().gwc_volume(_f32c(refimg_fea), _f32c(targetimg_fea), int(maxdisp), int(num_groups))
    return v if refimg_fea.dtype == torch.float32 else v.to(refimg_fea.dtype)


def build_concat_volume(refimg_fea, targetimg_fea, maxdisp, mask_left=True):
    _chk(refimg_fea, "refimg_fea", 4); _chk(targetimg_fea, "targetimg_fea", 4)
    B, Cn, H, W = refimg_fea.shape
    with timing.span("build_volume", 0, 0, Cn, NCDHW, maxdisp, H, W):
        v = _ext.load().concat_volume(_f32c(refimg_fea), _f32c(targetimg_fea), int(maxdisp), bool(mask_left))
    return v if refimg_fea.dtype == torch.float32 else v.to(refimg_fea.dtype)


def build_multirange_volumes(match_left, match_right, patch0_weight, patch1_weight, maxdisp, s_range, m_range, num_groups=8, channels_last=False):
    for t, name, nd in ((match_left, "match_left", 4), (match_right, "match_right", 4), (patch0_weight, "patch0_weight", 5), (patch1_weight, "patch1_weight", 5)):
        _chk(t, name, nd)
    B, Cn, H, W = match_left.shape
    if patch0_weight.shape[1] != num_groups or patch1_weight.shape[1] != num_groups:
        raise ValueError(f"patch weights must be [Co, num_groups={num_groups}, k, 1, 1], got {tuple(patch0_weight.shape)} and {tuple(patch1_weight.shape)}")
    with timing.span("mr_volume", Cn, num_groups, int(maxdisp), int(s_range), int(m_range), H, W):
        return _ext.load().mr_volume(match_left, match_right, patch0_weight, patch1_weight, int(maxdisp), int(s_range), int(m_range), bool(channels_last))


def correlation_volume(left_feature, right_feature, max_disp):
    _chk(left_feature, "left_feature", 4); _chk(right_feature, "right_feature", 4)
    out = _ext.load().corr_volume(_f32c(left_feature), _f32c(right_feature), int(max_disp))
    return out if left_feature.dtype == torch.float32 else out.to(left_feature.dtype)


def build_corr_volume(img_left, img_right, max_disp):
    vol = correlation_volume(img_left, img_right, max_disp)
    W = img_left.shape[-1]
    if max_disp > W:
        vol[:, W:] = vol[:, :1]
    return vol


def cat_fms(reference_fm, target_fm, max_disp=192, start_disp=0, dilation=1):
    ref, tgt = _f32c(_chk(reference_fm, "reference_fm", 4)), _f32c(_chk(target_fm, "target_fm", 4))
    if start_disp == 0 and dilation == 1:
        return build_concat_volume(ref, tgt, max_disp)
    B, C, H, W = ref.shape
    n = (max_disp + dilation - 1) // dilation
    idx = torch.tensor([int(i) for i in torch.linspace(start_disp, start_disp + max_disp - 1, n)], dtype=torch.int32, device=ref.device)
    out = torch.empty((B, 2 * C, n, H, W), device=ref.device, dtype=torch.float32)
    _ext.load().cat_fms(ref, tgt, out, idx)
    return out


def _pair_volume(left, right, planes, mode, groups=1):
    l, r = _f32c(_chk(left, "left", 4)), _f32c(_chk(right, "right", 4))
    assert l.shape == r.shape, "feature maps must have the same shape"
    B, C, H, W = l.shape
    shape = (B, groups, planes, H, W) if mode == 0 else ((B, planes, H, W) if mode == 3 else (B, C, planes, H, W))
    out = torch.empty(shape, device=l.device, dtype=torch.float32)
    _ext.load().pair_volume(l, r, out, groups, planes, mode)
    return out if left.dtype == torch.float32 else out.to(left.dtype)


def compute_volume(reference_embedding, target_embedding, maxdisp, side="left"):
    assert side in ("left", "right")
    return _pair_volume(reference_embedding, target_embedding, maxdisp, 1 if side == "left" else 2)


def build_sub_volume(feat_l, feat_r, maxdisp):
    return _pair_volume(feat_l, feat_r, maxdisp, 3)


class CoExCostVolume(torch.nn.Module):

    def __init__(self, maxdisp, group=1):
        super().__init__()
        self.maxdisp, self.group = maxdisp + 1, group

    def forward(self, x, y):
        return _pair_volume(x, y, self.maxdisp, 0, self.group)


def build_cost_volume_cl(gwc_left, gwc_right, num_groups, cat_left=None, cat_right=None, maxdisp=48,
                         mask_left=True):
    lg = rg = None
    if gwc_left is not None:
        lg, rg = _f32c(_chk(gwc_left, "gwc_left", 4)), _f32c(_chk(gwc_right, "gwc_right", 4))
        assert lg.shape[1] % num_groups == 0
    else:
        num_groups = 0
    lc = rc = None
    Cc = 0
    if cat_left is not None:
        lc, rc = _f32c(_chk(cat_left, "cat_left", 4)), _f32c(_chk(cat_right, "cat_right", 4))
        Cc = lc.shape[1]
    nch = num_groups + 2 * Cc
    VC = (nch + 3) // 4 * 4
    return _build(lg, rg, num_groups, lc, rc, maxdisp, mask_left=mask_left, vol_channels=VC)


def build_cost_volume_from_cl(gwc_feat, num_groups, cat_feat, B, maxdisp, gwc_channels=None, cat_channels=None,
                              gwc_off=0, mask_left=True, out_split=False):
    assert is_cl(gwc_feat) and gwc_feat.shape[0] == 2 * B and gwc_feat.shape[2] == 1
    _, Gs, _, H, W = gwc_feat.shape
    C = Gs - gwc_off if gwc_channels is None else gwc_channels
    Cc = 0
    if cat_feat is not None:
        assert is_cl(cat_feat) and cat_feat.shape[0] == 2 * B and tuple(cat_feat.shape[3:]) == (H, W)
        Cc = cat_feat.shape[1] if cat_channels is None else cat_channels
    gm = getattr(gwc_feat, "_osa_meta", None) if C > 0 else None
    cm = getattr(cat_feat, "_osa_meta", None) if (cat_feat is not None and Cc > 0) else None
    om = new_meta(gwc_feat.device)
    with timing.span("build_volume", C, num_groups, Cc, NDHWC, maxdisp, H, W):
        out, split = _ext.load().cost_volume_cl(gwc_feat, cat_feat, B, num_groups, maxdisp, C, Cc, gwc_off, bool(mask_left), bool(out_split), gm, cm, om)
    out._osa_meta = om
    if split:
        out._osa_split = True
    return out


# ... 155 lines not shown
```

Measured before the change: 203.3 stereo-pairs/s.

## Fuse left/right image concat and NHWC4 conversion; skip unused classifier depth taps

Result: no change. 204.8 stereo-pairs/s, median of 6 (+0.8%).

```diff
diff --git a/include/openstereo_amd.h b/include/openstereo_amd.h
--- a/include/openstereo_amd.h
+++ b/include/openstereo_amd.h
@@ -7,7 +7,7 @@
 extern "C" {
 #endif
 
-#define OSA_ABI_VERSION 17
+#define OSA_ABI_VERSION 18
 #define OSA_META_FLOATS 128
 
 enum { OSA_NCDHW = 0, OSA_NDHWC = 1 };
@@ -41,6 +41,8 @@
 
 int osa_ncdhw_to_ndhwc_f32(const float* x, float* y, int B, int C, long long S,
                            int yCs, int c_off, void* stream);
+int osa_pair_to_nhwc4_f32(const float* left, const float* right, float* y, int B, int C, long long S,
+                          float* meta, void* stream);
 int osa_ndhwc_to_ncdhw_f32(const float* x, float* y, int B, int C, long long S,
                            int xCs, int c_off, void* stream);
 
@@ -242,6 +244,7 @@
                                             int B, int D, int H, int W, int Ci, int xCs, int Co, int yCs,
                                             int kd, int kh, int kw, int pad_d, int pad_h, int pad_w,
                                             void* stream);
+int osa_classifier_march_segment_planes(int planes);
 
 int osa_softargmin_f32(const float* prob, float* out, int B, int D, int H, int W, void* stream);
 int osa_softmax_softargmin_f32(const float* cost, float* prob, float* out,
diff --git a/openstereo_amd/_lib.py b/openstereo_amd/_lib.py
--- a/openstereo_amd/_lib.py
+++ b/openstereo_amd/_lib.py
@@ -62,6 +62,7 @@
     **dict.fromkeys(("osa_softmax_softargmin_bwd_f32", "osa_softmax_softargmin_f32", "osa_softmax_softargmin_var_f32"), (c_i, [c_fp, c_fp, c_fp, c_i, c_i, c_i, c_i, c_st])),
     **dict.fromkeys(("osa_upsample_softargmin_bwd_f32", "osa_upsample_softargmin_var_f32"), (c_i, [c_fp, c_fp, c_fp, c_i, c_i, c_i, c_i, c_i, c_i, c_i, c_i, c_st])),
     "osa_amax_f32": (c_i, [c_fp, C.c_longlong, c_fp, c_st]),
+    "osa_pair_to_nhwc4_f32": (c_i, [c_fp, c_fp, c_fp, c_i, c_i, c_ll, c_fp, c_st]),
     **dict.fromkeys(("osa_upsample_softargmin_bwd_workspace_bytes", "osa_mr_volume_bwd_workspace_bytes", "osa_interlaced_volume_packed_floats", "osa_disparity_attention_packed_floats"), (C.c_size_t, [c_i] * 4)),
     "osa_upsample_softargmin_bwd_ws_f32": (c_i, [c_fp, c_fp, c_fp, c_i, c_i, c_i, c_i, c_i, c_i, c_i, c_i, c_fp, C.c_size_t, c_st]),
     "osa_deconv3d_redir_ndhwc_f32": (c_i, [c_fp] * 5 + [c_i] * 11 + [c_fp, c_i, c_i, c_fp, c_fp, c_fp, c_i, c_f, c_st]),
@@ -100,7 +101,7 @@
     "osa_channel_sums_multi": (c_i, [c_fp, c_i, c_i, c_i, c_ll, c_i, c_fp, c_fp, C.c_size_t, c_st]),
     "osa_channel_sums": (c_i, [c_fp, c_i, c_i, c_fp, c_i, c_i, c_fp, c_fp, c_fp, c_i, c_ll, c_i, c_fp, c_fp, C.c_size_t, c_st]),
     **dict.fromkeys(("osa_conv3d_march_launches", "osa_conv3d_march_s2_launches", "osa_deconv3d_walk_launches", "osa_conv_b_ring_launches", "osa_volume_walk_launches"), (c_ll, [])),
-    **dict.fromkeys(("osa_deconv_walk", "osa_deconv_walk_segment_planes", "osa_conv_march_s2_segment_planes", "osa_conv_b_ring_mask", "osa_volume_walk_step"), (c_i, [c_i])),
+    **dict.fromkeys(("osa_deconv_walk", "osa_deconv_walk_segment_planes", "osa_conv_march_s2_segment_planes", "osa_classifier_march_segment_planes", "osa_conv_b_ring_mask", "osa_volume_walk_step"), (c_i, [c_i])),
     "osa_build_volume_nhwc_split_eligible": (c_i, [c_fp, c_fp, c_fp, c_i, c_i, c_i, c_i, c_i, c_i, c_i, c_i, c_i]),
     "osa_build_volume_nhwc_split_f16x3": (c_i, [c_fp, c_fp, c_i, c_i, c_i, c_fp, c_fp, c_i, c_i, c_fp] + [c_i] * 7 + [c_fp, c_fp, c_fp, c_st]),
     "osa_upsample_softargmin_f32": (c_i, [c_fp, c_fp, c_i, c_i, c_i, c_i, c_i, c_i, c_i, c_i, c_st]),
diff --git a/openstereo_amd/csrc/conv3d.hip b/openstereo_amd/csrc/conv3d.hip
--- a/openstereo_amd/csrc/conv3d.hip
+++ b/openstereo_amd/csrc/conv3d.hip
@@ -1,3 +1,4 @@
+#include <type_traits>
 #include "conv_kernel.h"
 #include "conv_inst.h"
 
@@ -427,6 +428,21 @@
     const float4* xt = smem + th_ * CM_ROWQ + tw_ * CM_PXQ;
     const float4* w4 = reinterpret_cast<const float4*>(wpk);
     float a0 = 0.f, a1 = 0.f, a2 = 0.f;
+    auto taps = [&](auto sums) {
+        constexpr int SUMS = decltype(sums)::value;
+#pragma unroll
+        for (int kh = 0; kh < 3; ++kh)
+#pragma unroll
+            for (int kw = 0; kw < 3; ++kw)
+#pragma unroll
+                for (int q = 0; q < 8; ++q) {
+                    const float4 xv = xt[kh * CM_ROWQ + kw * CM_PXQ + q];
+                    const int wi = ((q >> 2) * 27 + kh * 3 + kw) * 4 + (q & 3);
+                    if (SUMS & 1) { const float4 wk2 = w4[wi + 18 * 4]; a0 = fmaf(xv.x, wk2.x, a0); a0 = fmaf(xv.y, wk2.y, a0); a0 = fmaf(xv.z, wk2.z, a0); a0 = fmaf(xv.w, wk2.w, a0); }
+                    if (SUMS & 2) { const float4 wk1 = w4[wi + 9 * 4]; a1 = fmaf(xv.x, wk1.x, a1); a1 = fmaf(xv.y, wk1.y, a1); a1 = fmaf(xv.z, wk1.z, a1); a1 = fmaf(xv.w, wk1.w, a1); }
+                    if (SUMS & 4) { const float4 wk0 = w4[wi]; a2 = fmaf(xv.x, wk0.x, a2); a2 = fmaf(xv.y, wk0.y, a2); a2 = fmaf(xv.z, wk0.z, a2); a2 = fmaf(xv.w, wk0.w, a2); }
+                }
+    };
     issue(d0 > 0 ? d0 - 1 : 0);
     for (int pd = d0 - 1; pd <= d1; ++pd) {
         if (pd >= 0 && pd < p.Di) {
@@ -436,19 +452,15 @@
                 if (loff[j] >= 0) smem[loff[j]] = pre[j];
             __syncthreads();
             if (pd + 1 <= d1 && pd + 1 < p.Di) issue(pd + 1);
-#pragma unroll
-            for (int kh = 0; kh < 3; ++kh)
-#pragma unroll
-                for (int kw = 0; kw < 3; ++kw)
-#pragma unroll
-                    for (int q = 0; q < 8; ++q) {
-                        const float4 xv = xt[kh * CM_ROWQ + kw * CM_PXQ + q];
-                        const int wi = ((q >> 2) * 27 + kh * 3 + kw) * 4 + (q & 3);
-                        const float4 wk0 = w4[wi], wk1 = w4[wi + 9 * 4], wk2 = w4[wi + 18 * 4];
-                        a0 = fmaf(xv.x, wk2.x, a0); a0 = fmaf(xv.y, wk2.y, a0); a0 = fmaf(xv.z, wk2.z, a0); a0 = fmaf(xv.w, wk2.w, a0);
-                        a1 = fmaf(xv.x, wk1.x, a1); a1 = fmaf(xv.y, wk1.y, a1); a1 = fmaf(xv.z, wk1.z, a1); a1 = fmaf(xv.w, wk1.w, a1);
-                        a2 = fmaf(xv.x, wk0.x, a2); a2 = fmaf(xv.y, wk0.y, a2); a2 = fmaf(xv.z, wk0.z, a2); a2 = fmaf(xv.w, wk0.w, a2);
-                    }
+            const int sums = (pd - 1 >= d0 ? 1 : 0) | (pd >= d0 && pd < d1 ? 2 : 0) | (pd + 1 < d1 ? 4 : 0);
+            switch (sums) {
+                case 1: taps(std::integral_constant<int, 1>{}); break;
+                case 4: taps(std::integral_constant<int, 4>{}); break;
+                case 3: taps(std::integral_constant<int, 3>{}); break;
+                case 6: taps(std::integral_constant<int, 6>{}); break;
+                case 2: taps(std::integral_constant<int, 2>{}); break;
+                default: taps(std::integral_constant<int, 7>{}); break;
+            }
         }
         const int od = pd - 1, oh = h0 + th_, ow = w0 + tw_;
         if (od >= d0 && od < d1 && oh < p.Hi && ow < p.Wi) {
@@ -918,6 +930,9 @@
                          int kd, int kh, int kw, int pad_d, int pad_h, int pad_w,
                          void* stream);
 
+static int g_classifier_march_planes = 0;
+extern "C" int osa_classifier_march_segment_planes(int planes) { const int prev = g_classifier_march_planes; g_classifier_march_planes = planes > 0 ? planes : 0; return prev; }
+
 extern "C" int osa_conv3d_small_co_ndhwc_f32(const float* x, const float* w_ref, const float* bias,
                                              const float* residual, float* y,
                                              int B, int D, int H, int W, int Ci, int xCs, int Co, int yCs,
@@ -968,10 +983,10 @@
         a.tilesH = cdiv(H, CM_TH); a.tilesW = cdiv(W, CM_TW);
         const long long cols = (long long)B * a.tilesH * a.tilesW;
         int nseg = (int)((2048 + cols - 1) / cols);
-        { const int o = exp_int("OSA_MARCH_NSEG", 0); if (o) nseg = o; }
         if (nseg > D / 8) nseg = D / 8;
         if (nseg < 1) nseg = 1;
-        const int dseg = cdiv(D, nseg);
+        int dseg = cdiv(D, nseg);
+        if (g_classifier_march_planes > 0) dseg = g_classifier_march_planes < D ? g_classifier_march_planes : D;
         nseg = cdiv(D, dseg);
         OSA_REQUIRE(cols * nseg < (1ll << 31), "conv3d_small_co: grid too large");
         OSA_REQUIRE((long long)H * W * xCs < (1ll << 31), "conv3d_small_co: plane too large");
diff --git a/openstereo_amd/csrc/layout.hip b/openstereo_amd/csrc/layout.hip
--- a/openstereo_amd/csrc/layout.hip
+++ b/openstereo_amd/csrc/layout.hip
@@ -55,9 +55,67 @@
     publish_amax(meta, am, 0u, red);
 }
 
+constexpr int PAIR_PX = 1024, PAIR_RUNS = 4;
+template <bool VEC>
+__global__ __launch_bounds__(256) void pair_to_nhwc4_kernel(const float* __restrict__ left, const float* __restrict__ right, float* __restrict__ y,
+                                                            int B, int C, long long S, int chunks, float* meta) {
+    __shared__ __attribute__((aligned(16))) float pl[4][PAIR_PX];
+    __shared__ float red[4];
+    const int tid = threadIdx.x;
+    const int img = blockIdx.x / chunks;
+    const long long s_first = (long long)(blockIdx.x % chunks) * (PAIR_PX * PAIR_RUNS);
+    const float* x = img < B ? left + (size_t)img * C * S : right + (size_t)(img - B) * C * S;
+    float* yo = y + (size_t)img * S * 4;
+    const unsigned seen = meta ? amax_peek(meta) : 0u;
+    float am = 0.f;
+    for (int r = 0; r < PAIR_RUNS; ++r) {
+        const long long s0 = s_first + (long long)r * PAIR_PX;
+        if (s0 >= S) break;
+        if (r) __syncthreads();
+        const long long s = s0 + tid * 4;
+        for (int c = 0; c < C; ++c) {
+            const float* xc = x + (size_t)c * S;
+            float4 v = make_float4(0.f, 0.f, 0.f, 0.f);
+            if (VEC) {
+                if (s < S) v = *reinterpret_cast<const float4*>(xc + s);
+            } else {
+                if (s < S) v.x = xc[s];
+                if (s + 1 < S) v.y = xc[s + 1];
+                if (s + 2 < S) v.z = xc[s + 2];
+                if (s + 3 < S) v.w = xc[s + 3];
+            }
+            am = fmaxf(am, fmaxf(fmaxf(fabsf(v.x), fabsf(v.y)), fmaxf(fabsf(v.z), fabsf(v.w))));
+            *reinterpret_cast<float4*>(&pl[c][tid * 4]) = v;
+        }
+        __syncthreads();
+#pragma unroll
+        for (int k = 0; k < PAIR_PX / 256; ++k) {
+            const int px = k * 256 + tid;
+            if (s0 + px < S)
+                store16(yo + (size_t)(s0 + px) * 4, make_float4(pl[0][px], C > 1 ? pl[1][px] : 0.f, C > 2 ? pl[2][px] : 0.f, C > 3 ? pl[3][px] : 0.f));
+        }
+    }
+    if (meta) publish_amax(meta, am, seen, red);
+}
+
 }
 
 using namespace osa;
+
+extern "C" int osa_pair_to_nhwc4_f32(const float* left, const float* right, float* y, int B, int C, long long S, float* meta, void* stream) {
+    OSA_REQUIRE(left && right && y, "pair_to_nhwc4: NULL pointer");
+    OSA_REQUIRE(B > 0 && C >= 1 && C <= 4 && S > 0, "pair_to_nhwc4: B = %d, C = %d (1..4), S = %lld", B, C, S);
+    OSA_REQUIRE(((size_t)y & 15) == 0, "pair_to_nhwc4: y must be 16-byte aligned");
+    const long long chunks = (S + PAIR_PX * PAIR_RUNS - 1) / (PAIR_PX * PAIR_RUNS);
+    OSA_REQUIRE(2ll * B * chunks < (1ll << 31), "pair_to_nhwc4: grid too large");
+    const dim3 grid((unsigned)(2ll * B * chunks));
+    if ((S & 3) == 0 && (((size_t)left | (size_t)right) & 15) == 0)
+        hipLaunchKernelGGL(pair_to_nhwc4_kernel<true>, grid, dim3(256), 0, (hipStream_t)stream, left, right, y, B, C, S, (int)chunks, meta);
+    else
+        hipLaunchKernelGGL(pair_to_nhwc4_kernel<false>, grid, dim3(256), 0, (hipStream_t)stream, left, right, y, B, C, S, (int)chunks, meta);
+    OSA_LAUNCH_CHECK("pair_to_nhwc4");
+    return 0;
+}
 
 extern "C" int osa_amax_f32(const float* x, long long n, float* meta, void* stream) {
     OSA_REQUIRE(x && meta && n > 0, "amax: NULL pointer or empty tensor");
diff --git a/openstereo_amd/csrc/torch_ext.cpp b/openstereo_amd/csrc/torch_ext.cpp
--- a/openstereo_amd/csrc/torch_ext.cpp
+++ b/openstereo_amd/csrc/torch_ext.cpp
@@ -609,6 +609,24 @@
     gpu_f32(x, "x"); gpu_f32(y, "y");
     TORCH_CHECK(y.is_contiguous() && x.dim() == 5 && x.stride(1) == 1, "to_ncdhw: x NDHWC, y contiguous NCDHW");
     OSA_CALL(osa_ndhwc_to_ncdhw_f32(fp(x), y.data_ptr<float>(), (int)x.size(0), (int)C, (long long)S, (int)x.size(1), (int)c_off, cur_stream()));
+}
+static void pair_to_cl_check(const at::Tensor& left, const at::Tensor& right) {
+    TORCH_CHECK(left.dim() == 4 && left.size(1) >= 1 && left.size(1) <= 4 && left.sizes() == right.sizes() && left.is_contiguous() && right.is_contiguous() && left.numel() > 0,
+                "pair_to_cl: two contiguous [B, C <= 4, H, W] images of one shape");
+}
+at::Tensor pair_to_cl(const at::Tensor& left, const at::Tensor& right, at::Tensor out_meta) {
+    gpu_f32(left, "left"); gpu_f32(right, "right"); gpu_f32(out_meta, "out_meta");
+    pair_to_cl_check(left, right);
+    TORCH_CHECK(out_meta.is_contiguous() && out_meta.numel() >= OSA_META_FLOATS, "pair_to_cl: out_meta is a range block of ", OSA_META_FLOATS, " floats");
+    const int64_t B = left.size(0), H = left.size(2), W = left.size(3);
+    auto out = at::empty({2 * B, 1, H, W, 4}, left.options());
+    OSA_CALL(osa_pair_to_nhwc4_f32(fp(left), fp(right), out.data_ptr<float>(), (int)B, (int)left.size(1), (long long)(H * W), out_meta.data_ptr<float>(), cur_stream()));
+    return out.permute({0, 4, 1, 2, 3});
+}
+at::Tensor pair_to_cl_meta(const at::Tensor& left, const at::Tensor& right, at::Tensor out_meta) {
+    pair_to_cl_check(left, right);
+    (void)out_meta;
+    return at::empty({2 * left.size(0), 1, left.size(2), left.size(3), 4}, left.options()).permute({0, 4, 1, 2, 3});
 }
 
 void conv_pack(const at::Tensor& w, at::Tensor packed, at::IntArrayRef geom, int64_t prec, const c10::optional<at::Tensor>& w_amax, const c10::optional<at::Tensor>& scale_out) {
@@ -1344,6 +1362,7 @@
     m.def("conv_wgrad_multi(Tensor[] xs, Tensor[] dys, Tensor(a!) dw, int[] dims, int prec, Tensor? x_meta, Tensor? dy_meta) -> bool");
     m.def("to_cl(Tensor x, Tensor(a!) y, int C, int S, int c_off) -> ()");
     m.def("to_ncdhw(Tensor x, Tensor(a!) y, int C, int S, int c_off) -> ()");
+    m.def("pair_to_cl(Tensor left, Tensor right, Tensor(a!) out_meta) -> Tensor");
     m.def("conv_pack(Tensor w, Tensor(a!) packed, int[] geom, int prec, Tensor? w_amax, Tensor(b!)? scale_out) -> ()");
     m.def("deconv_pack(Tensor w, Tensor(a!) packed, int[] geom, int prec, Tensor? w_amax, Tensor(b!)? scale_out) -> ()");
     m.def("gru_gates_rz_fwd(Tensor pre, Tensor? bias_z, Tensor? bias_r, Tensor cz, Tensor cr, Tensor h, Tensor(a!) z, Tensor(b!) rh) -> ()");
@@ -1418,6 +1437,7 @@
     m.impl("conv_wgrad_multi", &conv_wgrad_multi);
     m.impl("to_cl", &to_cl);
     m.impl("to_ncdhw", &to_ncdhw);
+    m.impl("pair_to_cl", &pair_to_cl);
     m.impl("conv_pack", &conv_pack);
     m.impl("deconv_pack", &deconv_pack);
     m.impl("gru_gates_rz_fwd", &gru_gates_rz_fwd);
@@ -1484,6 +1504,7 @@
     m.impl("softmax_softargmin_var_bwd", &softmax_softargmin_var_bwd_meta);
     m.impl("upsample_softargmin_var_bwd", &upsample_softargmin_var_bwd_meta);
     m.impl("cost_volume_cl", &cost_volume_cl_meta);
+    m.impl("pair_to_cl", &pair_to_cl_meta);
     m.impl("conv_wgrad", &conv_wgrad_meta);
     m.impl("conv_wgrad_multi", &conv_wgrad_multi_meta);
     m.impl("channel_sums", &channel_sums_meta);
diff --git a/openstereo_amd/models/gwcnet.py b/openstereo_amd/models/gwcnet.py
--- a/openstereo_amd/models/gwcnet.py
+++ b/openstereo_amd/models/gwcnet.py
@@ -62,9 +62,7 @@
         self.layer3 = self._stage(128, 3, 1, 1, 1)
         self.layer4 = self._stage(128, 3, 1, 1, 2)
         if concat_feature:
-            self.lastconv = nn.Sequential(
-                _cb2(320, 128, 3, 1, 1, 1), nn.ReLU(inplace=True),
-                nn.Conv2d(128, concat_feature_channel, 1, 1, 0, bias=False))
+            self.lastconv = nn.Sequential(_cb2(320, 128, 3, 1, 1, 1), nn.ReLU(inplace=True), nn.Conv2d(128, concat_feature_channel, 1, 1, 0, bias=False))
 
     def _stage(self, cout, n, stride, pad, dil):
         shortcut = None
@@ -88,10 +86,10 @@
             return pk
         return cached_pack(self, "_pk", build)
 
-    def forward_cl(self, img):
+    def forward_cl(self, img, right=None):
         pk = self._pack()
         sp = _SPLIT_ACT and chains(pk["first"][0].precision)
-        x = ops.to_cl(img.unsqueeze(2))
+        x = ops.to_cl(img.unsqueeze(2)) if right is None else ops.pair_to_cl(img, right)
         for conv in pk["first"]:
             x = conv(x, out_split=sp)
         xoff, cat, slices = 0, None, {1: 0, 2: 64, 3: 192}
@@ -160,7 +158,7 @@
 
     def forward_cl(self, left, right):
         with timing.span("backbone2d_engine", left.shape[2], left.shape[3]):
-            return self.feature_extraction.forward_cl(torch.cat((left, right), 0))
+            return self.feature_extraction.forward_cl(left, right)
 
 
 class GwcVolumeCostProcessor(nn.Module):
@@ -178,18 +176,15 @@
 
     @amp.contract("volume")
     def forward(self, inputs):
-        l, r = inputs["ref_feature"], inputs["tgt_feature"]
-        cat = self.use_concat_volume
+        l, r, cat = inputs["ref_feature"], inputs["tgt_feature"], self.use_concat_volume
         if self.training or (torch.is_grad_enabled() and l["gwc_feature"].requires_grad):
             D4 = self.maxdisp // self.downsample
             vol = AG.build_gwc_volume(l["gwc_feature"], r["gwc_feature"], D4, self.num_groups)
             if cat:
                 vol = torch.cat((vol, AG.build_concat_volume(l["concat_feature"], r["concat_feature"], D4)), 1)
             return {"cost_volume": vol}
-        vol = ops.build_cost_volume_cl(
-            l["gwc_feature"], r["gwc_feature"], self.num_groups,
-            l["concat_feature"] if cat else None, r["concat_feature"] if cat else None,
-            maxdisp=self.maxdisp // self.downsample)
+        vol = ops.build_cost_volume_cl(l["gwc_feature"], r["gwc_feature"], self.num_groups, l["concat_feature"] if cat else None,
+                                       r["concat_feature"] if cat else None, maxdisp=self.maxdisp // self.downsample)
         return {"cost_volume": vol}
 
     def input_output(self):
@@ -355,8 +350,7 @@
     def __init__(self, cfgs=GWCNET_G_SCENEFLOW):
         super().__init__()
         self.maxdisp = cfgs.MAX_DISP
-        kw = dict(maxdisp=self.maxdisp, downsample=cfgs.DOWNSAMPLE, num_groups=cfgs.NUM_GROUPS,
-                  use_concat_volume=cfgs.USE_CONCAT_VOLUME)
+        kw = dict(maxdisp=self.maxdisp, downsample=cfgs.DOWNSAMPLE, num_groups=cfgs.NUM_GROUPS, use_concat_volume=cfgs.USE_CONCAT_VOLUME)
         self.Backbone = GwcBackbone(use_concat_volume=cfgs.USE_CONCAT_VOLUME, concat_channels=cfgs.CONCAT_CHANNELS)
         self.CostProcessor = GwcVolumeCostProcessor(**kw)
         self.DispProcessor = GwcDispProcessor(concat_channels=cfgs.CONCAT_CHANNELS, **kw)
@@ -374,17 +368,13 @@
                 if catf is not None:
                     STAGE_STASH.append(("backbone concat", catf.clone()))
             cp = self.CostProcessor
-            vol = ops.build_cost_volume_from_cl(gwc, cp.num_groups, catf if cp.use_concat_volume else None, B,
-                                                cp.maxdisp // cp.downsample,
-                                                cat_channels=self.Backbone.concat_channels or None,
-                                                out_split=_SPLIT_ACT and _VOL_SPLIT and self.DispProcessor._pack()["d00"].precision == "f16x3")
+            vol = ops.build_cost_volume_from_cl(gwc, cp.num_groups, catf if cp.use_concat_volume else None, B, cp.maxdisp // cp.downsample,
+                                                cat_channels=self.Backbone.concat_channels or None, out_split=_SPLIT_ACT and _VOL_SPLIT and self.DispProcessor._pack()["d00"].precision == "f16x3")
             if getattr(vol, "_osa_split", False):
-                dp = self.DispProcessor
-                h, w = inputs["left"].shape[2:]
-                if getattr(self, "return_variance", False):
-                    pred, var = ops.upsample_softargmin(dp.aggregate_cl(vol), dp.maxdisp, h, w, align_corners=False, return_variance=True)
-                    return {"disp_pred": pred, "disp_var": var}
-                return {"disp_pred": ops.upsample_softargmin(dp.aggregate_cl(vol), dp.maxdisp, h, w, align_corners=False)}
+                dp, (h, w) = self.DispProcessor, inputs["left"].shape[2:]
+                var = bool(getattr(self, "return_variance", False))
+                out = ops.upsample_softargmin(dp.aggregate_cl(vol), dp.maxdisp, h, w, align_corners=False, return_variance=var)
+                return {"disp_pred": out[0], "disp_var": out[1]} if var else {"disp_pred": out}
             inputs["cost_volume"] = vol
         else:
             inputs.update(self.Backbone(inputs))
diff --git a/openstereo_amd/ops.py b/openstereo_amd/ops.py
--- a/openstereo_amd/ops.py
+++ b/openstereo_amd/ops.py
@@ -57,9 +57,16 @@
     B, Cn, D, H, W = xs.shape
     Cp = (Cn + pad_to - 1) // pad_to * pad_to
     y = empty_cl(B, Cp, D, H, W, x.device)
-    if Cp != Cn:
-        y.zero_()
-    _ext.load().to_cl(xs, y, Cn, D * H * W, 0)
+    _ext.load().to_cl(xs, y.zero_() if Cp != Cn else y, Cn, D * H * W, 0)
+    return y
+
+
+def pair_to_cl(left: torch.Tensor, right: torch.Tensor) -> torch.Tensor:
+    if not (left.is_cuda and left.dtype == right.dtype == torch.float32 and left.dim() == 4 and left.shape[1] <= 4 and left.shape == right.shape and left.is_contiguous() and right.is_contiguous()):
+        return to_cl(torch.cat((left, right), 0).unsqueeze(2))
+    m = new_meta(left.device)
+    y = _ext.load().pair_to_cl(left, right, m)
+    y._osa_meta = m
     return y
 
 
```
